# Litianyu141/Gen-FVGN-steady

Hardware: AMD Instinct MI355X
Metric: training iters/sec, 50k-cell cylinder mesh (fwd + loss + bwd + Adam, batch resident in HBM) (higher is better)
Workload: dtype f32

## Files before the change

### gen-fvgn-steady_amd/csrc/cfwd.hip

```cpp
#include <cstdlib>

#include "tchain_kernel.h"

#include "gfv_limits.h"
int* gfv_internal_status_ptr();

namespace {

constexpr float CF_SH = 16.0f;
constexpr float CF_SH_INV = 1.0f / 16.0f;
constexpr float CF_SH_LIMIT = 2048.0f;

__device__ __forceinline__ void cf_barrier() {
  asm volatile("s_waitcnt lgkmcnt(0)\n\ts_barrier" ::: "memory");
}

template <int KT0, int TG, int NW>
struct CfLds {
  static constexpr int KTB = KT0 > 4 ? KT0 : 4;
  static constexpr int B0 = 0;
  static constexpr int B1 = TG * KTB * 2048;
  static constexpr int SINV = B1 + TG * 8192;
  static constexpr int LNP = SINV + TG * 64;
  static constexpr int TOTAL = LNP + TG * 16 * NW * 8;
// ... 132 lines not shown
        if (!LOWP) wl[n][T] = im[T * 1024 + n * 128 + 64];
      }
  };
  auto hidden = [&](int layer, char* xout, float* save) {
#pragma unroll
    for (int q = 0; q < TG; ++q) {
      const int row = row0 + 16 * q + j;
      const bool live = q < ngt && row < A.M;
      const float si = layer == 0 ? sinv[q * 16 + j] : CF_SH_INV;
      float a[4 * NT];
#pragma unroll
      for (int n = 0; n < NT; ++n) {
        const float4 b = bias[layer][n];
        float v[4] = {(acc[q][n][0] * si) * invw + b.x, (acc[q][n][1] * si) * invw + b.y, (acc[q][n][2] * si) * invw + b.z,
                      (acc[q][n][3] * si) * invw + b.w};
        if (PADD && layer == 0) {
          v[0] += ps[PADD ? q : 0][n].x + pr[PADD ? q : 0][n].x; v[1] += ps[PADD ? q : 0][n].y + pr[PADD ? q : 0][n].y;
          v[2] += ps[PADD ? q : 0][n].z + pr[PADD ? q : 0][n].z; v[3] += ps[PADD ? q : 0][n].w + pr[PADD ? q : 0][n].w;
        }
        if (save && live) st4(save + (size_t)row * 128 + c0 + 16 * n, v);
        const gfv_f2 g01 = gfv_gelu2(gfv_f2{v[0], v[1]}), g23 = gfv_gelu2(gfv_f2{v[2], v[3]});
        a[4 * n + 0] = g01.x; a[4 * n + 1] = g01.y; a[4 * n + 2] = g23.x; a[4 * n + 3] = g23.y;
      }
      float m = 0.f;
#pragma unroll
      for (int e = 0; e < 4 * NT; e += 2) m = max3_abs(m, a[e], a[e + 1]);
      mabs = fmaxf(mabs, live ? m : 0.f);
      if constexpr (NT == 2) {
        float e8[8];
#pragma unroll
        for (int e = 0; e < 8; ++e) e8[e] = a[e] * CF_SH;
        gfv_uint4 hi, lo;
        gfv_split8_t<BF>(e8, hi, lo);
        gfv_uint4* dst = reinterpret_cast<gfv_uint4*>(xout + (size_t)(q * 4 + w) * 2048) + lane;
        dst[0] = hi;
        if (!LOWP) dst[64] = lo;
      } else {
        unsigned h0, h1, l0, l1;
        gfv_split_pair_t<BF>(a[0] * CF_SH, a[1] * CF_SH, h0, l0);
        gfv_split_pair_t<BF>(a[2] * CF_SH, a[3] * CF_SH, h1, l1);
        char* dst = xout + (size_t)(q * 4 + (w >> 1)) * 2048 + lane * 16 + (w & 1) * 8;
        *reinterpret_cast<uint2*>(dst) = make_uint2(h0, h1);
        if (!LOWP) *reinterpret_cast<uint2*>(dst + 1024) = make_uint2(l0, l1);
      }
    }
  };

  mma(b0, std::integral_constant<int, KT0>{});
  load_w(A.layer[1].Wh);
  hidden(0, b1, A.layer[0].save);
  cf_barrier();
  mma(b1, std::integral_constant<int, 4>{});
  load_w(A.layer[2].Wh);
  hidden(1, b0, A.layer[1].save);
  float4 gam[NT], bet[NT];
  if constexpr (FINLN) {
#pragma unroll
    for (int n = 0; n < NT; ++n) { gam[n] = ld4(A.fin_gamma + c0 + 16 * n); bet[n] = ld4(A.fin_beta + c0 + 16 * n); }
  }
  float4 rres[TG][NT];
  if (A.res[0]) {
#pragma unroll
    for (int q = 0; q < TG; ++q) {
      const float* rp = A.res[0] + (size_t)min(row0 + 16 * q + j, A.M - 1) * A.res_ld[0] + c0;
#pragma unroll
      for (int n = 0; n < NT; ++n) rres[q][n] = ld4(rp + 16 * n);
    }
  }
  cf_barrier();
  if constexpr (!FINLN) {
    if (w == 0) {
      mma(b0, std::integral_constant<int, 4>{});
      const int ncol = A.layer[2].N;
      const float* bp = A.layer[2].bias;
#pragma unroll
      for (int q = 0; q < TG; ++q) {
        const int row = row0 + 16 * q + j;
        if (q < ngt && row < A.M) {
#pragma unroll
          for (int r = 0; r < 4; ++r) {
            const int col = 4 * g + r;
            if (col < ncol) A.out[0][(size_t)row * A.out_ld[0] + col] = (acc[q][0][r] * CF_SH_INV) * invw + (bp ? bp[col] : 0.f);
          }
        }
      }
    }
    if (mabs > CF_SH_LIMIT) atomicOr(status, 2);
    return;
  }
  mma(b0, std::integral_constant<int, 4>{});
  const int hcols = (A.hidden > 0 && A.hidden < 128) ? A.hidden : 128;
  float y[TG][4 * NT];
#pragma unroll
  for (int q = 0; q < TG; ++q) {
    const int row = row0 + 16 * q + j;
    const bool live = q < ngt && row < A.M;
    float s = 0.f;
#pragma unroll
    for (int n = 0; n < NT; ++n) {
      const float4 b = bias[2][n];
      float v[4] = {(acc[q][n][0] * CF_SH_INV) * invw + b.x, (acc[q][n][1] * CF_SH_INV) * invw + b.y,
                    (acc[q][n][2] * CF_SH_INV) * invw + b.z, (acc[q][n][3] * CF_SH_INV) * invw + b.w};
      if (A.fin_presave && live) st4(A.fin_presave + (size_t)row * 128 + c0 + 16 * n, v);
#pragma unroll
      for (int r = 0; r < 4; ++r) {
        y[q][4 * n + r] = v[r];
        s += v[r];
      }
    }
    const float mw = row_sum(s) * (1.0f / (16.0f * NT));
    float m2 = 0.f;
#pragma unroll
    for (int e = 0; e < 4 * NT; ++e) {
      const float d = y[q][e] - mw;
      m2 += d * d;
    }
    m2 = row_sum(m2);
    if (g == 0) *reinterpret_cast<float2*>(lnp + ((q * 16 + j) * NW + w) * 2) = make_float2(mw, m2);
  }
  cf_barrier();
  {
    const float inv_h = 1.0f / (float)hcols, npad = (float)(128 - hcols);
#pragma unroll
    for (int q = 0; q < TG; ++q) {
      const int row = row0 + 16 * q + j;
      const bool live = q < ngt && row < A.M;
      const float4* pp = reinterpret_cast<const float4*>(lnp + (q * 16 + j) * 2 * NW);
      float m128, m2a;
      if constexpr (NW == 4) {
        const float4 p0 = pp[0], p1 = pp[1];
        m128 = ((p0.x + p0.z) + (p1.x + p1.z)) * 0.25f;
        const float e0 = p0.x - m128, e1 = p0.z - m128, e2 = p1.x - m128, e3 = p1.z - m128;
        m2a = ((p0.y + p0.w) + (p1.y + p1.w)) + 32.0f * ((e0 * e0 + e1 * e1) + (e2 * e2 + e3 * e3));
      } else {
        const float4 p0 = pp[0], p1 = pp[1], p2 = pp[2], p3 = pp[3];
        m128 = (((p0.x + p0.z) + (p1.x + p1.z)) + ((p2.x + p2.z) + (p3.x + p3.z))) * 0.125f;
        const float e0 = p0.x - m128, e1 = p0.z - m128, e2 = p1.x - m128, e3 = p1.z - m128, e4 = p2.x - m128, e5 = p2.z - m128,
                    e6 = p3.x - m128, e7 = p3.z - m128;
        m2a = (((p0.y + p0.w) + (p1.y + p1.w)) + ((p2.y + p2.w) + (p3.y + p3.w))) +
              16.0f * (((e0 * e0 + e1 * e1) + (e2 * e2 + e3 * e3)) + ((e4 * e4 + e5 * e5) + (e6 * e6 + e7 * e7)));
      }
      const float mean = hcols == 128 ? m128 : (m128 * 128.0f) * inv_h;
      const float dm = m128 - mean;
      const float m2 = hcols == 128 ? m2a : (m2a + 128.0f * dm * dm) - npad * (mean * mean);
      const float rstd = rsqrtf(m2 * inv_h + 1e-5f);
      if (A.fin_stats && live && w == 0 && g == 0) *reinterpret_cast<float2*>(A.fin_stats + 2 * (size_t)row) = make_float2(mean, rstd);
#pragma unroll
      for (int n = 0; n < NT; ++n) {
        const float4 ga = gam[n], be = bet[n];
        float o[4] = {(y[q][4 * n + 0] - mean) * rstd * ga.x + be.x, (y[q][4 * n + 1] - mean) * rstd * ga.y + be.y,
                      (y[q][4 * n + 2] - mean) * rstd * ga.z + be.z, (y[q][4 * n + 3] - mean) * rstd * ga.w + be.w};
        if (live) {
          if (A.out_nores) st4(A.out_nores + (size_t)row * 128 + c0 + 16 * n, o);
          if (A.res[0]) { o[0] += rres[q][n].x; o[1] += rres[q][n].y; o[2] += rres[q][n].z; o[3] += rres[q][n].w; }
          st4(A.out[0] + (size_t)row * A.out_ld[0] + c0 + 16 * n, o);
        }
      }
    }
  }
  if (mabs > CF_SH_LIMIT) atomicOr(status, 2);
}

inline bool cf_al16(const void* p) { return (reinterpret_cast<size_t>(p) & 15) == 0; }

template <int KT0, int N0, bool PADD, bool RAGIN, bool FINLN = true>
void cf_launch(const gfv_rowtile_args_t& a, int lowp, hipStream_t stream) {
  int* st = gfv_internal_status_ptr();
  constexpr int tg = 2;
  const int tiles = (a.M + 16 * tg - 1) / (16 * tg);
  const dim3 grid(PADD ? gfv_xcd_grid(tiles) : tiles), blk(512);
  if (lowp == 2) GFV_LAUNCH((cfwd_kernel<KT0, N0, 2, PADD, 2, RAGIN, 8, FINLN>), grid, blk, 0, stream, a, st);
  else if (lowp) GFV_LAUNCH((cfwd_kernel<KT0, N0, 2, PADD, 1, RAGIN, 8, FINLN>), grid, blk, 0, stream, a, st);
  else GFV_LAUNCH((cfwd_kernel<KT0, N0, 2, PADD, 0, RAGIN, 8, FINLN>), grid, blk, 0, stream, a, st);
}

}

int gfv_internal_cfwd_try(const gfv_rowtile_args_t* a, int lowp, hipStream_t stream, int dry) {
  if (!gfv_internal_status_ptr()) return 0;
  const int on = gfv_internal_limit(GFV_LIM_CFWD_ON);
  const int max_m = gfv_internal_limit(GFV_LIM_CFWD_MAX_M);
  if (!on || a->nlayers != 3 || a->M > max_m || a->M < 1 || (a->flags & (GFV_CHAIN_ROW_OWNER | GFV_CHAIN_COLUMN_OWNER))) return 0;
  const bool dec = a->fin_op == GFV_FIN_PLAIN && a->layer[2].N >= 1 && a->layer[2].N <= 16 && !a->res[0] && !a->out_nores && !a->fin_presave &&
                   !a->fin_stats && !a->padd && a->nseg == 1 && a->layer[0].K == 128;
  if (a->in_op != GFV_IN_NONE || !a->wmax) return 0;
  if (!dec && (a->fin_op != GFV_FIN_LN || !a->fin_gamma || !a->fin_beta)) return 0;
  if (a->in_add || a->gadd || a->in_save || a->in_aux || a->ln_partial || a->gscale || a->dw_partial || a->in_stats || a->fin_aux) return 0;
  for (int l = 0; l < 3; ++l) {
    const gfv_layer_t& L = a->layer[l];
    if (!L.Wh || (L.N != 128 && !(dec && l == 2)) || L.aux || L.bias2 || (L.bias && !cf_al16(L.bias) && !(dec && l == 2))) return 0;
    if (L.op != (l < 2 ? GFV_OP_BIAS_GELU : GFV_OP_NONE)) return 0;
    if (l > 0 && L.K != 128) return 0;
    if (L.save && !cf_al16(L.save)) return 0;
  }
  if (a->layer[2].save) return 0;
  if (!a->out[0] || a->out[1] || a->out[2] || (!dec && ((a->out_ld[0] & 3) || !cf_al16(a->out[0]))) || a->res[1] || a->res[2]) return 0;
  if (a->res[0] && ((a->res_ld[0] & 3) || !cf_al16(a->res[0]))) return 0;
  if ((a->out_nores && !cf_al16(a->out_nores)) || (a->fin_presave && !cf_al16(a->fin_presave)) ||
      (!dec && (!cf_al16(a->fin_gamma) || !cf_al16(a->fin_beta))))
    return 0;
  if (a->fin_stats && (reinterpret_cast<size_t>(a->fin_stats) & 7)) return 0;
  for (int i = 0; i < a->nseg; ++i)
    if (a->seg[i].idx || a->seg[i].csr_rowptr || a->seg[i].csr_scale || a->seg[i].save) return 0;
  const int K0 = a->layer[0].K;
  int shape = -1;
  auto plain = [&](int i, int width) {
    const gfv_seg_t& s = a->seg[i];
    return s.width == width && (s.ld & 3) == 0 && cf_al16(s.ptr);
  };
  if (a->padd) {
    if (a->nseg == 1 && K0 == 128 && plain(0, 128) && a->padd_s && a->padd_r && a->padd_ld >= 256 && (a->padd_ld & 3) == 0 && cf_al16(a->padd))
      shape = 1;
  } else if (a->nseg == 2 && K0 == 192 && plain(0, 64) && plain(1, 128)) {
    shape = 0;
  } else if (dec) {
    if (plain(0, 128)) shape = 4;
  } else if (a->nseg == 1 && K0 == 128 && plain(0, 128)) {
    shape = 2;
  } else if (a->nseg == 1 && K0 <= 32 && a->seg[0].width == K0) {
    shape = 3;
  }
  if (shape < 0) return 0;
  if (dry) return 1;
  if (shape == 0) cf_launch<6, 4, false, false>(*a, lowp, stream);
  else if (shape == 1) cf_launch<4, 8, true, false>(*a, lowp, stream);
  else if (shape == 2) cf_launch<4, 8, false, false>(*a, lowp, stream);
  else if (shape == 4) cf_launch<4, 8, false, false, false>(*a, lowp, stream);
  else cf_launch<1, 2, false, true>(*a, lowp, stream);
  return 1;
}
```

### gen-fvgn-steady_amd/csrc/colchain.hip

```cpp
#include "colchain_kernel.h"

int* gfv_internal_status_ptr();

static int cc_env(const char* name, int dflt) {
  const char* e = getenv(name);
  return e ? atoi(e) : dflt;
}
static bool al16(const void* p) { return (reinterpret_cast<size_t>(p) & 15) == 0; }

static int cc_cus() {
  static int n = 0;
  if (!n) {
    int dev = 0;
    hipDeviceProp_t pr;
    if (hipGetDevice(&dev) == hipSuccess && hipGetDeviceProperties(&pr, dev) == hipSuccess) n = pr.multiProcessorCount;
    if (n <= 0) n = 256;
    const int want = cc_env("GFV_COLCHAIN_WGS", 0);
    if (want > 0 && want <= n) n = want;
  }
  return n;
}

static bool cc_bwd_ok(const gfv_rowtile_args_t* a) {
  static const int on = cc_env("GFV_COLCHAIN_BWD", 1);
  static const int min_m = cc_env("GFV_COLCHAIN_BWD_MIN_M", 2048);
  if (a->flags & GFV_CHAIN_ROW_OWNER) return false;
  if (!(a->flags & GFV_CHAIN_COLUMN_OWNER) && (!on || a->M < min_m)) return false;
  if (!a->dw_partial || a->dw_partial_stride < GFV_DW_FUSED_FLOATS || !a->in_stats || !a->wmax) return false;
  if (a->dw_in) return false;
  const bool noout = a->nlayers == 2;
  const bool rc = a->rc_Wh[0] != nullptr;
  if (rc && (!a->rc_Wh[1] || a->dw_in || !al16(a->rc_Wh[0]) || !al16(a->rc_Wh[1]) || (a->rc_bias[0] && !al16(a->rc_bias[0])) ||
             (a->rc_bias[1] && !al16(a->rc_bias[1]))))
    return false;
  if (!rc && a->rc_Wh[1]) return false;
  if ((a->nlayers != 3 && !noout) || a->in_op != GFV_IN_LNBWD || a->fin_op != GFV_FIN_PLAIN || a->nseg != 1) return false;
  if (noout && (a->layer[1].op != GFV_OP_MUL_DGELU || a->layer[1].save || a->res[0] || a->gadd || a->dw_in || !a->out[0])) return false;
  if (a->seg[0].width != 128 || a->seg[0].idx || a->seg[0].csr_rowptr || a->seg[0].save || a->seg[0].ld != 128 || !al16(a->seg[0].ptr)) return false;
  if (a->M > (1 << 22) || a->out_ld[0] != 128 || (a->res[0] && a->res_ld[0] != 128) || (a->dw_in && a->dw_in_ld != 128)) return false;
  if (a->layer[0].op != GFV_OP_MUL_DGELU || a->layer[1].op != GFV_OP_MUL_DGELU || (!noout && a->layer[2].op != GFV_OP_NONE)) return false;
  for (int l = 0; l < a->nlayers; ++l) {
    const gfv_layer_t& L = a->layer[l];
    if (!L.Wh || (L.N != 128 && !(l == 2 && L.N == 192)) || L.K != 128 || L.bias || L.bias2) return false;
    if (l < 2 && !(rc && l == 0) && (!L.aux || !al16(L.aux))) return false;
    if (L.save && !al16(L.save)) return false;
  }
  if ((!rc && (!a->in_aux || !al16(a->in_aux))) || !a->in_gamma || !al16(a->in_gamma) || a->ln_partial || a->padd) return false;
  const bool out2 = !noout && a->layer[2].N == 192;
  if (!a->out[0] || (out2 ? (!a->out[1] || a->out_ld[1] != 64 || !al16(a->out[1]) || a->dw_in) : a->out[1] != nullptr) || a->out[2] ||
      a->res[1] || a->res[2] || a->out_nores)
    return false;
  if ((a->out_ld[0] & 3) || !al16(a->out[0]) || (a->res[0] && ((a->res_ld[0] & 3) || !al16(a->res[0])))) return false;
  if (a->in_add && !al16(a->in_add)) return false;
  if (a->gadd && (!al16(a->gadd) || !a->gadd_s || !a->gadd_r)) return false;
  if (a->in_save && !al16(a->in_save)) return false;
  if ((reinterpret_cast<size_t>(a->in_stats) & 7) || !al16(a->dw_partial) || (a->dw_partial_stride & 3)) return false;
  return true;
}
extern "C" int gfv_hidden_size(void);
extern "C" int gfv_f16split_enabled(void);
extern "C" int gfv_rowtile_dw_partials(void) { return cc_cus(); }
extern "C" int gfv_rowtile_dw_partials_m(int32_t M) {
  const int tiles = (M + 63) / 64;
  return tiles < cc_cus() ? (tiles > 0 ? tiles : 1) : cc_cus();
}
extern "C" int gfv_rowtile_fuses_dw(const gfv_rowtile_args_t* a) {
  if (!a || gfv_hidden_size() != 128 || gfv_f16split_enabled() == 0) return 0;
  gfv_rowtile_args_t t = *a;
  t.hidden = 128;
  return cc_bwd_ok(&t) ? 1 : 0;
}

int gfv_internal_colchain_try(const gfv_rowtile_args_t* a, hipStream_t stream) {
  if (a->hidden == 128 && cc_bwd_ok(a)) {
    int* st = gfv_internal_status_ptr();
    if (!st) return 0;
    const dim3 grid(gfv_rowtile_dw_partials_m(a->M)), blk(64 * CC_W);
#define CB_K(...) GFV_LAUNCH((colchain_bwd_kernel<__VA_ARGS__>), grid, blk, 0, stream, *a, st)
#define CB_LAUNCH(LOWP, RC)                                                                                                      \
  do {                                                                                                                           \
    if (a->nlayers == 2) CB_K(LOWP, false, false, true, RC);                                                                     \
    else if (a->layer[2].N == 192 && a->gadd) CB_K(LOWP, true, true, false, RC);                                                 \
    else if (a->layer[2].N == 192) CB_K(LOWP, false, true, false, RC);                                                           \
    else if (a->gadd) CB_K(LOWP, true, false, false, RC);                                                                        \
    else CB_K(LOWP, false, false, false, RC);                                                                                    \
  } while (0)
    const bool rc = a->rc_Wh[0] != nullptr;
    if (a->product_form == 2) { if (rc) CB_LAUNCH(2, true); else CB_LAUNCH(2, false); }
    else if (a->product_form != 0) { if (rc) CB_LAUNCH(1, true); else CB_LAUNCH(1, false); }
    else { if (rc) CB_LAUNCH(0, true); else CB_LAUNCH(0, false); }
#undef CB_K
#undef CB_LAUNCH
    return 2;
  }
  return 0;
}
```

### gen-fvgn-steady_amd/csrc/colchain_kernel.h

```cpp
#pragma once
#include "tchain_kernel.h"

namespace {

constexpr int CC_W = 8;
constexpr float CC_SH = 16.0f;
constexpr float CC_SH_INV = 1.0f / 16.0f;
constexpr float CC_SH_LIMIT = 2048.0f;
#ifdef GFV_CC_TIMING
#define CT_DECL long long ct_[16] = {0, 0, 0, 0, 0, 0, 0, 0, 0, 0, 0, 0, 0, 0, 0, 0}; long long ct_prev_ = clock64();
#define CT(k) do { __builtin_amdgcn_s_waitcnt(0xc07f); const long long now_ = clock64(); ct_[k] += now_ - ct_prev_; ct_prev_ = now_; } while (0)
#else
#define CT_DECL
#define CT(k)
#endif
__device__ __forceinline__ void cc_barrier() {
  asm volatile("s_waitcnt lgkmcnt(0)\n\ts_barrier" ::: "memory");
}

struct CcCtx {
  int w, lane, j, g, col0;
  int M;
  int row0;
  int ngt;
  float invw;
  float mabs;
};

template <int KT, int LOWP, bool FENCE = false>
__device__ __forceinline__ void cc_mma_pair(const char* xbuf, int pair, const gfv_f16x8 (&wh)[KT], const gfv_f16x8 (&wl)[KT],
                                            int lane, floatx4& a0, floatx4& a1) {
  const gfv_f16x8* f0 = reinterpret_cast<const gfv_f16x8*>(xbuf + (size_t)(2 * pair) * KT * 2048) + lane;
  const gfv_f16x8* f1 = f0 + KT * 128;
  a0 = floatx4{0.f, 0.f, 0.f, 0.f};
  a1 = floatx4{0.f, 0.f, 0.f, 0.f};
#pragma unroll
  for (int T = 0; T < KT; ++T) {
    const gfv_f16x8 xh0 = f0[(2 * T) * 64], xh1 = f1[(2 * T) * 64];
    if (!LOWP) {
      const gfv_f16x8 xl0 = f0[(2 * T + 1) * 64], xl1 = f1[(2 * T + 1) * 64];
      a0 = __builtin_amdgcn_mfma_f32_16x16x32_f16(wl[T], xh0, a0, 0, 0, 0);
      a1 = __builtin_amdgcn_mfma_f32_16x16x32_f16(wl[T], xh1, a1, 0, 0, 0);
      a0 = __builtin_amdgcn_mfma_f32_16x16x32_f16(wh[T], xl0, a0, 0, 0, 0);
      a1 = __builtin_amdgcn_mfma_f32_16x16x32_f16(wh[T], xl1, a1, 0, 0, 0);
    }
    a0 = gfv_mma_hh<LOWP == 2>(wh[T], xh0, a0);
    a1 = gfv_mma_hh<LOWP == 2>(wh[T], xh1, a1);
    if (FENCE) __builtin_amdgcn_sched_barrier(0);
  }
}

template <bool BF>
__device__ __forceinline__ void cc_put_frag(char* xbuf, int q, const CcCtx& c, const float (&a)[4], float scale) {
  unsigned h0, h1, l0, l1;
  const gfv_f2 s01 = gfv_f2{a[0], a[1]} * gfv_splat2(scale), s23 = gfv_f2{a[2], a[3]} * gfv_splat2(scale);
  gfv_split_pair_t<BF>(s01.x, s01.y, h0, l0);
  gfv_split_pair_t<BF>(s23.x, s23.y, h1, l1);
  char* dst = xbuf + (size_t)((q * 4 + (c.w >> 1)) * 2) * 1024 + c.lane * 16 + (c.w & 1) * 8;
  *reinterpret_cast<uint2*>(dst) = make_uint2(h0, h1);
  *reinterpret_cast<uint2*>(dst + 1024) = make_uint2(l0, l1);
}

constexpr int CB_TG = 4;
struct CbLds {
  static constexpr int BUF = CB_TG * 8192;
  static constexpr int B0 = 0, B1 = BUF, B2 = 2 * BUF;
  static constexpr int PART = 3 * BUF;
  static constexpr int SMAX = PART + CB_TG * 16 * 8 * 8;
  static constexpr int TOTAL = SMAX + 64;
};

__device__ __forceinline__ void cb_tr_operand(const char* xbuf, int q0, int ct, int lane, gfv_f16x8& hi, gfv_f16x8& lo) {
  typedef short s4 __attribute__((ext_vector_type(4)));
  typedef __attribute__((address_space(3))) s4* lds_s4;
  const int s = lane & 15, gp = lane >> 4;
  const int off = ((q0 * 4 + (ct >> 1)) * 2) * 1024 + (16 * (s & 3) + 4 * gp + (s >> 2)) * 16 + (ct & 1) * 8;
  const char* p = xbuf + off;
  const s4 h0 = __builtin_amdgcn_ds_read_tr16_b64_v4i16((lds_s4)(p));
  const s4 l0 = __builtin_amdgcn_ds_read_tr16_b64_v4i16((lds_s4)(p + 1024));
  const s4 h1 = __builtin_amdgcn_ds_read_tr16_b64_v4i16((lds_s4)(p + 8192));
  const s4 l1 = __builtin_amdgcn_ds_read_tr16_b64_v4i16((lds_s4)(p + 8192 + 1024));
  typedef short s8 __attribute__((ext_vector_type(8)));
  const s8 h = {h0[0], h0[1], h0[2], h0[3], h1[0], h1[1], h1[2], h1[3]};
  const s8 l = {l0[0], l0[1], l0[2], l0[3], l1[0], l1[1], l1[2], l1[3]};
  hi = __builtin_bit_cast(gfv_f16x8, h);
  lo = __builtin_bit_cast(gfv_f16x8, l);
}

__device__ __forceinline__ int cb_dw_ntile(int w, int i) { return 2 * (w >> 1) + (i >> 2); }
__device__ __forceinline__ int cb_dw_ktile(int w, int i) { return 4 * (w & 1) + (i & 3); }
__device__ __forceinline__ int cb_dw_btile(int w) { return 2 * (w >> 1) + (w & 1); }
template <int LOWP>
__device__ __forceinline__ void cb_dw_tile(const char* gbuf, const char* abuf, int npairs, int w, int lane, floatx4 (&acc)[8],
                                           floatx4& accb) {
  const gfv_f16x8 ones = gfv_frag_ones<LOWP == 2>();
  const int nt0 = 2 * (w >> 1), kt0 = 4 * (w & 1);
  for (int pr = 0; pr < npairs; ++pr) {
    gfv_f16x8 gh[2], gl[2];
    cb_tr_operand(gbuf, 2 * pr, nt0, lane, gh[0], gl[0]);
    cb_tr_operand(gbuf, 2 * pr, nt0 + 1, lane, gh[1], gl[1]);
    {
      const bool odd = (w & 1) != 0;
      const gfv_f16x8 bh = odd ? gh[1] : gh[0], bl = odd ? gl[1] : gl[0];
      if (!LOWP) accb = __builtin_amdgcn_mfma_f32_16x16x32_f16(bl, ones, accb, 0, 0, 0);
      accb = gfv_mma_hh<LOWP == 2>(bh, ones, accb);
    }
#pragma unroll
    for (int kk = 0; kk < 4; ++kk) {
      gfv_f16x8 ah, al;
      cb_tr_operand(abuf, 2 * pr, kt0 + kk, lane, ah, al);
#pragma unroll
      for (int nn = 0; nn < 2; ++nn) {
        if (!LOWP) {
          acc[4 * nn + kk] = __builtin_amdgcn_mfma_f32_16x16x32_f16(gl[nn], ah, acc[4 * nn + kk], 0, 0, 0);
          acc[4 * nn + kk] = __builtin_amdgcn_mfma_f32_16x16x32_f16(gh[nn], al, acc[4 * nn + kk], 0, 0, 0);
        }
        acc[4 * nn + kk] = gfv_mma_hh<LOWP == 2>(gh[nn], ah, acc[4 * nn + kk]);
      }
    }
    __builtin_amdgcn_sched_barrier(0);
  }
}

template <bool BF>
__device__ __forceinline__ void cb_hidden_bwd(CcCtx& c, int q, const floatx4& acc, float inv_in, const float4& z, float sg,
                                              char* gout, char* aout, float (&v)[4]) {
  const gfv_f2 z01 = {z.x, z.y}, z23 = {z.z, z.w};
  gfv_f2 a01, a23, d01, d23;
  gfv_gelu_dgelu2(z01, a01, d01);
  gfv_gelu_dgelu2(z23, a23, d23);
  const gfv_f2 ki = gfv_splat2(inv_in), kw = gfv_splat2(c.invw);
  const gfv_f2 v01 = ((gfv_f2{acc[0], acc[1]} * ki) * kw) * d01, v23 = ((gfv_f2{acc[2], acc[3]} * ki) * kw) * d23;
  v[0] = v01.x; v[1] = v01.y; v[2] = v23.x; v[3] = v23.y;
  const float a[4] = {a01.x, a01.y, a23.x, a23.y};
  const float mq = max3_abs(max3_abs(0.f, v[0], v[1]), v[2], v[3]) * sg;
  const float ma = max3_abs(max3_abs(0.f, a[0], a[1]), a[2], a[3]) * (60000.0f / CC_SH_LIMIT);
  c.mabs = fmaxf(c.mabs, q < c.ngt ? fmaxf(mq, ma) : 0.f);
  cc_put_frag<BF>(gout, q, c, v, sg);
  cc_put_frag<BF>(aout, q, c, a, CC_SH);
}

__device__ __forceinline__ char* cb_own_slot(char* xbuf, int q, const CcCtx& c) {
  return xbuf + (size_t)((q * 4 + (c.w >> 1)) * 2) * 1024 + c.lane * 16 + (c.w & 1) * 8;
}
__device__ __forceinline__ void cb_park4(char* xbuf, int q, const CcCtx& c, const float (&v)[4]) {
  char* d = cb_own_slot(xbuf, q, c);
  *reinterpret_cast<float2*>(d) = make_float2(v[0], v[1]);
  *reinterpret_cast<float2*>(d + 1024) = make_float2(v[2], v[3]);
}
__device__ __forceinline__ void cb_unpark4(char* xbuf, int q, const CcCtx& c, float (&v)[4]) {
  const char* d = cb_own_slot(xbuf, q, c);
  const float2 a = *reinterpret_cast<const float2*>(d), b = *reinterpret_cast<const float2*>(d + 1024);
  v[0] = a.x; v[1] = a.y; v[2] = b.x; v[3] = b.y;
}

template <bool BF>
__device__ __forceinline__ void cb_hidden_bwd_dg(CcCtx& c, int q, const floatx4& acc, float inv_in, const float (&dg)[4], float sg,
                                                 char* gout, float (&v)[4]) {
#pragma unroll
  for (int r = 0; r < 4; ++r) v[r] = ((acc[r] * inv_in) * c.invw) * dg[r];
  const float mq = max3_abs(max3_abs(0.f, v[0], v[1]), v[2], v[3]) * sg;
  c.mabs = fmaxf(c.mabs, q < c.ngt ? mq : 0.f);
  cc_put_frag<BF>(gout, q, c, v, sg);
}

typedef int cb_i32x4 __attribute__((ext_vector_type(4)));
typedef int cb_i32x2 __attribute__((ext_vector_type(2)));
typedef __amdgpu_buffer_rsrc_t cb_rsrc;
constexpr int CB_OFF_DEAD = 0x7ffffff0;
__device__ __forceinline__ cb_rsrc cb_buf(const void* p, size_t bytes) {
  const size_t n = p ? (bytes < 0x7fffffe0ull ? bytes : 0x7fffffe0ull) : 0;
  return __builtin_amdgcn_make_buffer_rsrc(const_cast<void*>(p), 0, (int)n, 0x00020000);
}
typedef float cb_f32x2 __attribute__((ext_vector_type(2)));
__device__ __forceinline__ float4 cb_ld4(cb_rsrc r, int off) {
  const floatx4 f = __builtin_bit_cast(floatx4, __builtin_amdgcn_raw_buffer_load_b128(r, off, 0, 0));
  return make_float4(f[0], f[1], f[2], f[3]);
}
__device__ __forceinline__ float2 cb_ld2(cb_rsrc r, int off) {
  const cb_f32x2 f = __builtin_bit_cast(cb_f32x2, __builtin_amdgcn_raw_buffer_load_b64(r, off, 0, 0));
  return make_float2(f[0], f[1]);
}
__device__ __forceinline__ void cb_st4v(cb_rsrc r, int off, const floatx4& f) {
  __builtin_amdgcn_raw_buffer_store_b128(__builtin_bit_cast(cb_i32x4, f), r, off, 0, 0);
}
__device__ __forceinline__ void cb_st4(cb_rsrc r, int off, const float (&v)[4]) {
  const floatx4 f = {v[0], v[1], v[2], v[3]};
  __builtin_amdgcn_raw_buffer_store_b128(__builtin_bit_cast(cb_i32x4, f), r, off, 0, 0);
}

struct CbIn {
  float4 dy[CB_TG], yv[CB_TG], ga[CB_TG];
  float2 st[CB_TG];
};
struct CbBufs {
  cb_rsrc dy, y3, stats, z2, z1, gadd, gidx, save1, res, out;
};
__device__ __forceinline__ int cb_off(const CcCtx& c, int row0, int q) { return min(row0 + 16 * q + c.j, c.M - 1) * 512 + c.col0 * 4; }

template <bool GADD>
__device__ __forceinline__ void cb_load_gidx(const CbBufs& B, const CcCtx& c, int row0, int (&gidx)[CB_TG]) {
  if (GADD) {
#pragma unroll
    for (int q = 0; q < CB_TG; ++q) gidx[q] = __builtin_amdgcn_raw_buffer_load_b32(B.gidx, min(row0 + 16 * q + c.j, c.M - 1) * 4, 0, 0);
  }
}
__device__ __forceinline__ void cb_load_inputs(const CbBufs& B, const CcCtx& c, int row0, CbIn& in) {
#pragma unroll
  for (int q = 0; q < CB_TG; ++q) {
    const int off = cb_off(c, row0, q);
    in.dy[q] = cb_ld4(B.dy, off);
    in.yv[q] = cb_ld4(B.y3, off);
    in.st[q] = cb_ld2(B.stats, min(row0 + 16 * q + c.j, c.M - 1) * 8);
  }
}
__device__ __forceinline__ void cb_load_dy_stats(const CbBufs& B, const CcCtx& c, int row0, CbIn& in) {
#pragma unroll
  for (int q = 0; q < CB_TG; ++q) {
    in.dy[q] = cb_ld4(B.dy, cb_off(c, row0, q));
    in.st[q] = cb_ld2(B.stats, min(row0 + 16 * q + c.j, c.M - 1) * 8);
  }
}
__device__ __forceinline__ void cb_load_rows(cb_rsrc r, const CcCtx& c, int row0, float4 (&v)[CB_TG]) {
#pragma unroll
  for (int q = 0; q < CB_TG; ++q) v[q] = cb_ld4(r, cb_off(c, row0, q));
}
template <bool GADD>
__device__ __forceinline__ void cb_load_gathers(const CbBufs& B, const CcCtx& c, const int (&gidx)[CB_TG], CbIn& in) {
  if (GADD) {
#pragma unroll
    for (int q = 0; q < CB_TG; ++q) in.ga[q] = cb_ld4(B.gadd, gidx[q] * 256 + (c.col0 & 63) * 4);
  }
}

template <int LOWP, bool GADD, bool OUT2 = false, bool NOOUT = false, bool RC = false>
__global__ __launch_bounds__(64 * CC_W, 2) void colchain_bwd_kernel(const gfv_rowtile_args_t A, int* status) {
  constexpr int TG = CB_TG;
  __shared__ __attribute__((aligned(16))) char lds[CbLds::TOTAL + (RC ? CbLds::BUF : 0)];
  char* b0 = lds + CbLds::B0;
  char* b1 = lds + CbLds::B1;
  char* b2 = lds + CbLds::B2;
  char* b3 = lds + CbLds::TOTAL;
  float* part = reinterpret_cast<float*>(lds + CbLds::PART);
  float* smax = reinterpret_cast<float*>(lds + CbLds::SMAX);

  CcCtx c;
  c.w = __builtin_amdgcn_readfirstlane(threadIdx.x >> 6);
  c.lane = threadIdx.x & 63;
  c.j = c.lane & 15;
  c.g = c.lane >> 4;
  c.col0 = 16 * c.w + 4 * c.g;
  c.M = A.M;
  c.mabs = 0.f;
  c.invw = 1.0f / gfv_pow2_scale(*A.wmax);

  const int nwg = gridDim.x;
  const int wg = (nwg & 7) == 0 ? (int)(blockIdx.x & 7) * (nwg >> 3) + (int)(blockIdx.x >> 3) : (int)blockIdx.x;
  const int NG = (A.M + 15) >> 4;
  const int g_beg = (int)((long)NG * wg / nwg), g_end = (int)((long)NG * (wg + 1) / nwg);

  const size_t rows128 = (size_t)A.M * 512;
  CbBufs B;
  B.dy = cb_buf(A.seg[0].ptr, rows128);
  B.y3 = cb_buf(RC ? nullptr : A.in_aux, rows128);
  B.stats = cb_buf(A.in_stats, (size_t)A.M * 8);
  B.z2 = cb_buf(RC ? nullptr : A.layer[0].aux, rows128);
  B.z1 = cb_buf(A.layer[1].aux, rows128);
  B.gadd = cb_buf(A.gadd, 0x7fffffe0ull);
  B.gidx = cb_buf(c.w < 4 ? A.gadd_s : A.gadd_r, (size_t)A.M * 4);
  B.save1 = cb_buf(NOOUT ? A.out[0] : A.layer[1].save, rows128);
  B.res = cb_buf(NOOUT ? nullptr : A.res[0], rows128);
  B.out = cb_buf(NOOUT ? nullptr : A.out[0], rows128);
  const cb_rsrc out2 = cb_buf(OUT2 ? A.out[1] : nullptr, (size_t)A.M * 256);

  const cb_rsrc w0 = cb_buf(A.layer[0].Wh, 65536), w1 = cb_buf(A.layer[1].Wh, 65536),
                w2 = cb_buf(NOOUT ? nullptr : A.layer[2].Wh, OUT2 ? 131072 : 65536);
  const cb_rsrc rw2 = cb_buf(RC ? A.rc_Wh[0] : nullptr, 65536), rw3 = cb_buf(RC ? A.rc_Wh[1] : nullptr, 65536);
  const int woff = (c.w * 128 + c.lane) * 16;
  floatx4 dw3[8], dw2[8], db3 = floatx4{0.f, 0.f, 0.f, 0.f}, db2 = db3;
#pragma unroll
  for (int kt = 0; kt < 8; ++kt) dw3[kt] = dw2[kt] = floatx4{0.f, 0.f, 0.f, 0.f};
  float dgam[4] = {0.f, 0.f, 0.f, 0.f}, dbet[4] = {0.f, 0.f, 0.f, 0.f};
  float sacc = 0.f;
  float scap = 3.0e38f;

  float step1, step2;
  {
    float l1[2];
#pragma unroll
    for (int l = 0; l < 2; ++l) {
      const cb_rsrc wb = l == 0 ? w0 : w1;
      float acc = 0.f;
#pragma unroll
      for (int T = 0; T < 4; ++T) {
        const gfv_f16x8 h = __builtin_bit_cast(gfv_f16x8, __builtin_amdgcn_raw_buffer_load_b128(wb, woff + T * 16384, 0, 0));
        const gfv_f16x8 lo = __builtin_bit_cast(gfv_f16x8, __builtin_amdgcn_raw_buffer_load_b128(wb, woff + T * 16384 + 1024, 0, 0));
        if (LOWP == 2) {
          const gfv_bf16x8 hb = __builtin_bit_cast(gfv_bf16x8, h);
#pragma unroll
          for (int e = 0; e < 8; ++e) acc += fabsf((float)hb[e]);
        } else {
#pragma unroll
          for (int e = 0; e < 8; ++e) acc += fabsf((float)h[e] + (float)lo[e]);
        }
      }
      l1[l] = gfv_wave_max(row_sum(acc));
    }
    if (c.lane == 0) { smax[c.w] = l1[0]; part[c.w] = l1[1]; }
    cc_barrier();
    float m0 = 0.f, m1 = 0.f;
#pragma unroll
    for (int k = 0; k < 8; ++k) { m0 = fmaxf(m0, smax[k]); m1 = fmaxf(m1, part[k]); }
    cc_barrier();
    const float g0 = 1.13f * m0 * c.invw, g1 = 1.13f * m1 * c.invw;
    step1 = 1.0f / gfv_pow2_ceil(g0);
    step2 = 1.0f / gfv_pow2_ceil(g1);
  }

  constexpr bool PRE = true;
  int gidx[TG] = {0, 0, 0, 0};
  CbIn in;
  float4 zn[RC ? TG : 1];
  if (g_beg < g_end) {
    cb_load_gidx<GADD>(B, c, 16 * g_beg, gidx);
    if constexpr (RC) {
      cb_load_rows(B.z1, c, 16 * g_beg, zn);
      cb_load_dy_stats(B, c, 16 * g_beg, in);
      cb_load_gathers<GADD>(B, c, gidx, in);
    } else if (PRE) {
      cb_load_inputs(B, c, 16 * g_beg, in);
      cb_load_gathers<GADD>(B, c, gidx, in);
    }
  }
  const bool CB_LATE = c.w >= 4;
  CT_DECL
  for (int t0 = g_beg; t0 < g_end; t0 += TG) {
    c.row0 = 16 * t0;
    c.ngt = min(TG, g_end - t0);
    const int np = (c.ngt + 1) >> 1;
    const int next_row0 = t0 + TG < g_end ? 16 * (t0 + TG) : c.M;
    int offL[TG], offS[TG];
#pragma unroll
    for (int q = 0; q < TG; ++q) {
      const int row = c.row0 + 16 * q + c.j;
      offL[q] = cb_off(c, c.row0, q);
      offS[q] = (q < c.ngt && row < c.M) ? row * 512 + c.col0 * 4 : CB_OFF_DEAD;
    }
    if constexpr (RC) {
      gfv_f16x8 rh[4], rl[4];
#pragma unroll
      for (int T = 0; T < 4; ++T) {
        rh[T] = __builtin_bit_cast(gfv_f16x8, __builtin_amdgcn_raw_buffer_load_b128(rw2, woff + T * 16384, 0, 0));
        rl[T] = __builtin_bit_cast(gfv_f16x8, __builtin_amdgcn_raw_buffer_load_b128(rw2, woff + T * 16384 + 1024, 0, 0));
      }
      const float4 zero4 = make_float4(0.f, 0.f, 0.f, 0.f);
#pragma unroll
      for (int q = 0; q < TG; ++q) {
        const float z4[4] = {zn[q].x, zn[q].y, zn[q].z, zn[q].w};
        float a[4];
#pragma unroll
        for (int r = 0; r < 4; ++r) a[r] = gfv_gelu(z4[r]);
        const float ma = max3_abs(max3_abs(0.f, a[0], a[1]), a[2], a[3]) * (60000.0f / CC_SH_LIMIT);
        c.mabs = fmaxf(c.mabs, q < c.ngt ? ma : 0.f);
        cc_put_frag<LOWP == 2>(b3, q, c, a, CC_SH);
      }
      CT(12);
      cc_barrier();
      CT(13);
#pragma unroll
      for (int q = 0; q < TG; ++q) in.yv[q] = zero4;
      {
        int tvar = 0;
        asm volatile("" : "+v"(tvar));
        const float4 bi2 = cb_ld4(cb_buf(A.rc_bias[0], 512), c.col0 * 4 + tvar);
        floatx4 a0, a1;
        cc_mma_pair<4, LOWP, true>(b3, 0, rh, rl, c.lane, a0, a1);
#pragma unroll
        for (int p = 0; p < TG / 2; ++p) {
          if (p >= np) break;
          floatx4 n0 = a0, n1 = a1;
          if (p + 1 < TG / 2) cc_mma_pair<4, LOWP, true>(b3, p + 1, rh, rl, c.lane, n0, n1);
#pragma unroll
          for (int h = 0; h < 2; ++h) {
            const int q = 2 * p + h;
            const floatx4& acc = h ? a1 : a0;
            const float bb[4] = {bi2.x, bi2.y, bi2.z, bi2.w};
            float a[4], dg[4];
#pragma unroll
            for (int r = 0; r < 4; ++r) {
              const float z = (acc[r] * CC_SH_INV) * c.invw + bb[r];
              const gfv_erfc_t e = gfv_erfc_half(z);
              const float cdf = z >= 0.0f ? 1.0f - e.y : e.y;
              dg[r] = fmaf(z * 0.39894228040143267794f, e.e, cdf);
              a[r] = fmaf(-fabsf(z), e.y, fmaxf(z, 0.0f));
            }
            cb_park4(b1, q, c, dg);
            const float ma = max3_abs(max3_abs(0.f, a[0], a[1]), a[2], a[3]) * (60000.0f / CC_SH_LIMIT);
            c.mabs = fmaxf(c.mabs, q < c.ngt ? ma : 0.f);
            cc_put_frag<LOWP == 2>(b2, q, c, a, CC_SH);
          }
          a0 = n0; a1 = n1;
        }
      }
#pragma unroll
      for (int T = 0; T < 4; ++T) {
        rh[T] = __builtin_bit_cast(gfv_f16x8, __builtin_amdgcn_raw_buffer_load_b128(rw3, woff + T * 16384, 0, 0));
        rl[T] = __builtin_bit_cast(gfv_f16x8, __builtin_amdgcn_raw_buffer_load_b128(rw3, woff + T * 16384 + 1024, 0, 0));
      }
      CT(14);
      cc_barrier();
      CT(15);
      {
        int tvar = 0;
        asm volatile("" : "+v"(tvar));
        const float4 bi3 = cb_ld4(cb_buf(A.rc_bias[1], 512), c.col0 * 4 + tvar);
        floatx4 a0, a1;
        cc_mma_pair<4, LOWP, true>(b2, 0, rh, rl, c.lane, a0, a1);
#pragma unroll
        for (int p = 0; p < TG / 2; ++p) {
          if (p >= np) break;
          floatx4 n0 = a0, n1 = a1;
          if (p + 1 < TG / 2) cc_mma_pair<4, LOWP, true>(b2, p + 1, rh, rl, c.lane, n0, n1);
          in.yv[2 * p] = make_float4((a0[0] * CC_SH_INV) * c.invw + bi3.x, (a0[1] * CC_SH_INV) * c.invw + bi3.y,
                                     (a0[2] * CC_SH_INV) * c.invw + bi3.z, (a0[3] * CC_SH_INV) * c.invw + bi3.w);
          in.yv[2 * p + 1] = make_float4((a1[0] * CC_SH_INV) * c.invw + bi3.x, (a1[1] * CC_SH_INV) * c.invw + bi3.y,
                                         (a1[2] * CC_SH_INV) * c.invw + bi3.z, (a1[3] * CC_SH_INV) * c.invw + bi3.w);
          a0 = n0; a1 = n1;
        }
      }
    }
    float gg[TG][4], xh[TG][4], rs[TG];
    {
      float bmax = 0.f;
      if (!PRE) {
        cb_load_inputs(B, c, c.row0, in);
        cb_load_gathers<GADD>(B, c, gidx, in);
      }
      if (A.in_add) {
        const cb_rsrc ia = cb_buf(A.in_add, rows128);
#pragma unroll
        for (int q = 0; q < TG; ++q) {
          const float4 t = cb_ld4(ia, offL[q]);
          in.dy[q].x += t.x; in.dy[q].y += t.y; in.dy[q].z += t.z; in.dy[q].w += t.w;
        }
      }
      float* part_j = part + (c.j * 8 + c.w) * 2;
      const float4 gam = RC ? cb_ld4(cb_buf(A.in_gamma, 512), c.col0 * 4) : ld4(A.in_gamma + c.col0);
#pragma unroll
      for (int q = 0; q < TG; ++q) {
        const float lf = offS[q] != CB_OFF_DEAD ? 1.0f : 0.0f;
        float d[4] = {in.dy[q].x, in.dy[q].y, in.dy[q].z, in.dy[q].w};
        if (GADD) { d[0] += in.ga[q].x; d[1] += in.ga[q].y; d[2] += in.ga[q].z; d[3] += in.ga[q].w; }
        const float y[4] = {in.yv[q].x, in.yv[q].y, in.yv[q].z, in.yv[q].w};
        const float gm[4] = {gam.x, gam.y, gam.z, gam.w};
        const float mean = in.st[q].x, rstd = in.st[q].y;
        rs[q] = rstd;
        float s1 = 0.f, s2 = 0.f, am = 0.f;
#pragma unroll
        for (int h = 0; h < 2; ++h) {
          const int r = 2 * h;
          const gfv_f2 dd = gfv_f2{d[r], d[r + 1]} * gfv_splat2(lf);
          const gfv_f2 xx = (gfv_f2{y[r], y[r + 1]} - gfv_splat2(mean)) * gfv_splat2(rstd);
          const gfv_f2 dx = dd * xx;
          const gfv_f2 g2 = dd * gfv_f2{gm[r], gm[r + 1]};
          const gfv_f2 gx = g2 * xx;
          const gfv_f2 ng = gfv_f2{dgam[r], dgam[r + 1]} + dx, nb = gfv_f2{dbet[r], dbet[r + 1]} + dd;
          dgam[r] = ng.x; dgam[r + 1] = ng.y;
          dbet[r] = nb.x; dbet[r + 1] = nb.y;
          xh[q][r] = xx.x; xh[q][r + 1] = xx.y;
          gg[q][r] = g2.x; gg[q][r + 1] = g2.y;
          s1 += g2.x; s1 += g2.y;
          s2 += gx.x; s2 += gx.y;
          am = max3_abs(am, g2.x, g2.y);
        }
        s1 = row_sum(s1);
        s2 = row_sum(s2);
        if (c.g == 0) *reinterpret_cast<float2*>(part_j + q * 256) = make_float2(s1, s2);
        bmax = fmaxf(bmax, am * fabsf(rstd) * lf);
      }
      bmax = gfv_wave_max(bmax);
      if (c.lane == 0) smax[c.w] = bmax;
    }
    gfv_f16x8 wh[4], wl[4];
#pragma unroll
    for (int T = 0; T < 4; ++T) {
      wh[T] = __builtin_bit_cast(gfv_f16x8, __builtin_amdgcn_raw_buffer_load_b128(w0, woff + T * 16384, 0, 0));
      wl[T] = __builtin_bit_cast(gfv_f16x8, __builtin_amdgcn_raw_buffer_load_b128(w0, woff + T * 16384 + 1024, 0, 0));
    }
    float4 zq[TG];
    if constexpr (!RC) {
#pragma unroll
      for (int q = 0; q < TG; ++q) zq[q] = cb_ld4(B.z2, offL[q]);
    }
    CT(0);
    cc_barrier();
    CT(1);
    float s3;
    {
      const float4 ma = *reinterpret_cast<const float4*>(smax), mb = *reinterpret_cast<const float4*>(smax + 4);
      const float mx = fmaxf(fmaxf(fmaxf(ma.x, ma.y), fmaxf(ma.z, ma.w)), fmaxf(fmaxf(mb.x, mb.y), fmaxf(mb.z, mb.w)));
      s3 = fminf(gfv_pow2_scale(mx * 13.5f) * 2.0f, scap);
      scap = fminf(scap, s3 * 1048576.0f);
#pragma unroll
      for (int q = 0; q < TG; ++q) {
        const float4* pp = reinterpret_cast<const float4*>(part + (q * 16 + c.j) * 16);
        const float4 p0 = pp[0], p1 = pp[1], p2 = pp[2], p3 = pp[3];
        const float m1 = (((p0.x + p0.z) + (p1.x + p1.z)) + ((p2.x + p2.z) + (p3.x + p3.z))) * 0.0078125f;
        const float m2 = (((p0.y + p0.w) + (p1.y + p1.w)) + ((p2.y + p2.w) + (p3.y + p3.w))) * 0.0078125f;
        float g3[4];
#pragma unroll
        for (int h = 0; h < 2; ++h) {
          const int r = 2 * h;
          const gfv_f2 t = gfv_splat2(rs[q]) * ((gfv_f2{gg[q][r], gg[q][r + 1]} - gfv_splat2(m1)) - gfv_f2{xh[q][r], xh[q][r + 1]} * gfv_splat2(m2));
          g3[r] = t.x; g3[r + 1] = t.y;
        }
        if (A.in_save) cb_st4(cb_buf(A.in_save, rows128), offS[q], g3);
        cc_put_frag<LOWP == 2>(b0, q, c, g3, s3);
      }
    }
    if (sacc != 0.f && sacc != s3) {
      const float ratio = s3 / sacc;
#pragma unroll
      for (int kt = 0; kt < 8; ++kt) { dw3[kt] *= ratio; dw2[kt] *= ratio; }
      db3 *= ratio;
      db2 *= ratio;
    }
    sacc = s3;
    const float s2s = s3 * step1, s1s = s2s * step2;
    if (A.gscale && c.w == 0 && c.lane < c.ngt) {
      const size_t grp = (size_t)(c.row0 >> 4) + c.lane;
      A.gscale[grp] = s3 * 0.25f;
      A.gscale[(size_t)A.gscale_ld + grp] = s2s * 0.25f;
      A.gscale[2 * (size_t)A.gscale_ld + grp] = s1s * 0.25f;
    }
    CT(2);
    cc_barrier();
    CT(3);
    cb_load_gidx<GADD>(B, c, next_row0, gidx);
    {
      const float inv_in = 1.0f / s3;
      floatx4 a0, a1;
      cc_mma_pair<4, LOWP, true>(b0, 0, wh, wl, c.lane, a0, a1);
#pragma unroll
      for (int p = 0; p < TG / 2; ++p) {
        if (p >= np) break;
        floatx4 n0 = a0, n1 = a1;
        float v0[4], v1[4];
        if (!CB_LATE && p + 1 < TG / 2) cc_mma_pair<4, LOWP, true>(b0, p + 1, wh, wl, c.lane, n0, n1);
        if constexpr (RC) {
          float d0[4], d1[4];
          cb_unpark4(b1, 2 * p, c, d0);
          cb_unpark4(b1, 2 * p + 1, c, d1);
          cb_hidden_bwd_dg<LOWP == 2>(c, 2 * p, a0, inv_in, d0, s2s, b1, v0);
          cb_hidden_bwd_dg<LOWP == 2>(c, 2 * p + 1, a1, inv_in, d1, s2s, b1, v1);
        } else {
          cb_hidden_bwd<LOWP == 2>(c, 2 * p, a0, inv_in, zq[2 * p], s2s, b1, b2, v0);
          cb_hidden_bwd<LOWP == 2>(c, 2 * p + 1, a1, inv_in, zq[2 * p + 1], s2s, b1, b2, v1);
        }
        if (A.layer[0].save) {
          const cb_rsrc s0 = cb_buf(A.layer[0].save, rows128);
          cb_st4(s0, offS[2 * p], v0);
          cb_st4(s0, offS[2 * p + 1], v1);
        }
        if (CB_LATE && p + 1 < TG / 2) cc_mma_pair<4, LOWP, true>(b0, p + 1, wh, wl, c.lane, n0, n1);
        a0 = n0; a1 = n1;
      }
    }
#pragma unroll
    for (int T = 0; T < 4; ++T) {
      wh[T] = __builtin_bit_cast(gfv_f16x8, __builtin_amdgcn_raw_buffer_load_b128(w1, woff + T * 16384, 0, 0));
      wl[T] = __builtin_bit_cast(gfv_f16x8, __builtin_amdgcn_raw_buffer_load_b128(w1, woff + T * 16384 + 1024, 0, 0));
    }
#pragma unroll
    for (int q = 0; q < TG; ++q) zq[q] = cb_ld4(B.z1, offL[q]);
    CT(4);
    cc_barrier();
    CT(5);
    if constexpr (RC) cb_load_rows(B.z1, c, next_row0, zn);
    cb_dw_tile<LOWP>(b0, b2, np, c.w, c.lane, dw3, db3);
    if constexpr (RC) cb_dw_tile<LOWP>(b1, b3, np, c.w, c.lane, dw2, db2);
    CT(6);
    cc_barrier();
    CT(7);
    {
      const float inv_in = 1.0f / s2s;
      floatx4 a0, a1;
      cc_mma_pair<4, LOWP, true>(b1, 0, wh, wl, c.lane, a0, a1);
#pragma unroll
      for (int p = 0; p < TG / 2; ++p) {
        if (p >= np) break;
        floatx4 n0 = a0, n1 = a1;
        float v0[4], v1[4];
        if (!CB_LATE && p + 1 < TG / 2) cc_mma_pair<4, LOWP, true>(b1, p + 1, wh, wl, c.lane, n0, n1);
        if constexpr (RC) {
          const float d0[4] = {gfv_dgelu(zq[2 * p].x), gfv_dgelu(zq[2 * p].y), gfv_dgelu(zq[2 * p].z), gfv_dgelu(zq[2 * p].w)};
          const float d1[4] = {gfv_dgelu(zq[2 * p + 1].x), gfv_dgelu(zq[2 * p + 1].y), gfv_dgelu(zq[2 * p + 1].z),
                               gfv_dgelu(zq[2 * p + 1].w)};
          cb_hidden_bwd_dg<LOWP == 2>(c, 2 * p, a0, inv_in, d0, s1s, b0, v0);
          cb_hidden_bwd_dg<LOWP == 2>(c, 2 * p + 1, a1, inv_in, d1, s1s, b0, v1);
        } else {
          cb_hidden_bwd<LOWP == 2>(c, 2 * p, a0, inv_in, zq[2 * p], s1s, b0, b2, v0);
          cb_hidden_bwd<LOWP == 2>(c, 2 * p + 1, a1, inv_in, zq[2 * p + 1], s1s, b0, b2, v1);
        }
        cb_st4(B.save1, offS[2 * p], v0);
        cb_st4(B.save1, offS[2 * p + 1], v1);
        if (CB_LATE && p + 1 < TG / 2) cc_mma_pair<4, LOWP, true>(b1, p + 1, wh, wl, c.lane, n0, n1);
        a0 = n0; a1 = n1;
      }
    }
    if constexpr (!NOOUT) {
#pragma unroll
      for (int T = 0; T < 4; ++T) {
        wh[T] = __builtin_bit_cast(gfv_f16x8, __builtin_amdgcn_raw_buffer_load_b128(w2, woff + T * 16384, 0, 0));
        wl[T] = __builtin_bit_cast(gfv_f16x8, __builtin_amdgcn_raw_buffer_load_b128(w2, woff + T * 16384 + 1024, 0, 0));
      }
    }
    float4 rr[NOOUT ? 1 : TG];
    if constexpr (!NOOUT) {
#pragma unroll
      for (int q = 0; q < TG; ++q) rr[q] = cb_ld4(B.res, offL[q]);
    }
    CT(8);
    cc_barrier();
    CT(9);
    if constexpr (!NOOUT) {
      const float inv_in = 1.0f / s1s;
      floatx4 a0, a1;
      cc_mma_pair<4, LOWP, true>(b0, 0, wh, wl, c.lane, a0, a1);
#pragma unroll
      for (int p = 0; p < TG / 2; ++p) {
        if (p >= np) break;
        floatx4 n0 = a0, n1 = a1;
        if (!CB_LATE && p + 1 < TG / 2) cc_mma_pair<4, LOWP, true>(b0, p + 1, wh, wl, c.lane, n0, n1);
        const floatx4 o0 = (a0 * inv_in) * c.invw + floatx4{rr[2 * p].x, rr[2 * p].y, rr[2 * p].z, rr[2 * p].w};
        const floatx4 o1 = (a1 * inv_in) * c.invw + floatx4{rr[2 * p + 1].x, rr[2 * p + 1].y, rr[2 * p + 1].z, rr[2 * p + 1].w};
        cb_st4v(B.out, offS[2 * p], o0);
        cb_st4v(B.out, offS[2 * p + 1], o1);
        if (CB_LATE && p + 1 < TG / 2) cc_mma_pair<4, LOWP, true>(b0, p + 1, wh, wl, c.lane, n0, n1);
        a0 = n0; a1 = n1;
      }
      if constexpr (OUT2) {
        if (c.w < 4) {
          gfv_f16x8 xh2[4], xl2[4];
#pragma unroll
          for (int T = 0; T < 4; ++T) {
            xh2[T] = __builtin_bit_cast(gfv_f16x8, __builtin_amdgcn_raw_buffer_load_b128(w2, 65536 + woff + T * 16384, 0, 0));
            xl2[T] = __builtin_bit_cast(gfv_f16x8, __builtin_amdgcn_raw_buffer_load_b128(w2, 65536 + woff + T * 16384 + 1024, 0, 0));
          }
#pragma unroll
          for (int p = 0; p < TG / 2; ++p) {
            if (p >= np) break;
            floatx4 e0, e1;
            cc_mma_pair<4, LOWP, true>(b0, p, xh2, xl2, c.lane, e0, e1);
            const floatx4 o0 = (e0 * inv_in) * c.invw, o1 = (e1 * inv_in) * c.invw;
            const int ra = c.row0 + 32 * p + c.j, rb = ra + 16;
            cb_st4v(out2, (2 * p < c.ngt && ra < c.M) ? ra * 256 + c.col0 * 4 : CB_OFF_DEAD, o0);
            cb_st4v(out2, (2 * p + 1 < c.ngt && rb < c.M) ? rb * 256 + c.col0 * 4 : CB_OFF_DEAD, o1);
          }
        }
      }
    }
    CT(10);
    if constexpr (RC) {
      cb_load_dy_stats(B, c, next_row0, in);
      cb_load_gathers<GADD>(B, c, gidx, in);
    } else {
      if (PRE) {
        cb_load_inputs(B, c, next_row0, in);
        cb_load_gathers<GADD>(B, c, gidx, in);
      }
      cb_dw_tile<LOWP>(b1, b2, np, c.w, c.lane, dw2, db2);
    }
    CT(11);
  }

#ifdef GFV_CC_TIMING
  if (c.lane == 0 && A.fin_aux) {
    long long* dbg = reinterpret_cast<long long*>(const_cast<float*>(A.fin_aux)) + ((size_t)blockIdx.x * CC_W + c.w) * 16;
    for (int kk = 0; kk < 16; ++kk) dbg[kk] = ct_[kk];
  }
#endif
  if (A.dw_partial) {
    float* blk = A.dw_partial + (size_t)blockIdx.x * A.dw_partial_stride;
    const float is = sacc != 0.f ? 1.0f / sacc : 0.f;
    const float r2 = 1.0f / step1, r1 = r2 / step2;
    const float u3 = is * CC_SH_INV, u2 = (is * r2) * CC_SH_INV;
#pragma unroll
    for (int kt = 0; kt < 8; ++kt)
#pragma unroll
      for (int r = 0; r < 4; ++r) {
        const int n = 16 * cb_dw_ntile(c.w, kt) + 4 * c.g + r, k = 16 * cb_dw_ktile(c.w, kt) + c.j;
        blk[n * 128 + k] = dw3[kt][r] * u3;
        blk[16384 + 128 + n * 128 + k] = dw2[kt][r] * u2;
      }
    if (c.j == 0) {
#pragma unroll
      for (int r = 0; r < 4; ++r) {
        const int nb = 16 * cb_dw_btile(c.w) + 4 * c.g + r;
        blk[16384 + nb] = db3[r] * is;
        blk[2 * 16384 + 128 + nb] = db2[r] * (is * r2);
      }
    }
#pragma unroll
    for (int r = 0; r < 4; ++r) {
      const float dg = gfv_row16_sum(dgam[r]), db = gfv_row16_sum(dbet[r]);
      if (c.j == 0) {
        blk[2 * 16384 + 256 + c.col0 + r] = dg;
        blk[2 * 16384 + 384 + c.col0 + r] = db;
      }
    }
  }
  if (c.mabs > 60000.0f) atomicOr(status, 2);
}


}
```

### gen-fvgn-steady_amd/csrc/gfv_limits.h

```cpp
#pragma once
enum {
  GFV_LIM_CBWD_ON = 0,
  GFV_LIM_CBWD_MAX_M,
  GFV_LIM_CFWD_ON,
  GFV_LIM_CFWD_MAX_M,
  GFV_LIM_CTRANS_ON,
  GFV_LIM_CTRANS_MAX_M,
  GFV_LIM_LIN1S_ON,
  GFV_LIM_LIN1S_MAX_M,
  GFV_LIM_COUNT
};
int gfv_internal_limit(int which);
```

### gen-fvgn-steady_amd/csrc/rowtile.hip

```cpp
#include <atomic>
#include <stdio.h>
#include <stdlib.h>
#include <mutex>
#include "gfv_common.h"
#include "gfv_limits.h"
#include "gfv_prof.h"
#include "../../include/gfv.h"

namespace {
constexpr int BM = 64;
}

int gfv_internal_tchain_launch(const gfv_rowtile_args_t* args, int ragged, int f16, hipStream_t stream);

static std::atomic<int> g_f16_default{-1};
static thread_local int g_f16split = -1;
static int f16_default() {
  int d = g_f16_default.load(std::memory_order_relaxed);
  if (d < 0) {
    const char* e = getenv("GFV_F16SPLIT");
    d = e ? ((atoi(e) == 2 || atoi(e) == 3) ? atoi(e) : (atoi(e) != 0)) : 1;
    int expect = -1;
    if (!g_f16_default.compare_exchange_strong(expect, d)) d = expect;
  }
  return d;
}
extern "C" int gfv_f16split_enabled(void) { return g_f16split >= 0 ? g_f16split : f16_default(); }
extern "C" int gfv_set_f16split(int32_t on) {
  g_f16_default.store((on == 2 || on == 3) ? on : (on ? 1 : 0));
  g_f16split = -1;
  return GFV_OK;
}
extern "C" int gfv_set_f16split_thread(int32_t on) {
  if (on < -1 || on > 3) return GFV_ERR_ARG;
  g_f16split = on;
  return GFV_OK;
}
static int f16_mode() { return gfv_f16split_enabled(); }

static thread_local int g_hidden = 128;
extern "C" int gfv_hidden_size(void) { return g_hidden; }
extern "C" int gfv_set_hidden_size(int32_t h) {
  if (h < 16 || h > 128 || (h & 15)) return GFV_ERR_ARG;
  g_hidden = h;
  return GFV_OK;
}

static thread_local int g_last_path = -1;
extern "C" int gfv_rowtile_last_path(void) { return g_last_path; }
namespace {
struct LimitDef { const char* env; int dflt; };
const LimitDef k_limits[GFV_LIM_COUNT] = {
    {"GFV_CBWD", 1},        {"GFV_CBWD_MAX_M", 25000},      {"GFV_CFWD", 1},          {"GFV_CFWD_MAX_M", 250000},
    {"GFV_CTRANS", 1},         {"GFV_CTRANS_MAX_M", 16384},
    {"GFV_LIN1S", 1},       {"GFV_LIN1S_MAX_M", 16384}};
int g_limit[GFV_LIM_COUNT];
bool g_limit_set[GFV_LIM_COUNT];
std::once_flag g_limit_once;
void limits_init() {
  for (int i = 0; i < GFV_LIM_COUNT; ++i) {
    const char* e = getenv(k_limits[i].env);
    g_limit[i] = e ? atoi(e) : k_limits[i].dflt;
    g_limit_set[i] = false;
  }
}
}
int gfv_internal_limit(int which) {
  std::call_once(g_limit_once, limits_init);
  return (which >= 0 && which < GFV_LIM_COUNT) ? g_limit[which] : 0;
}
extern "C" int gfv_get_limit(int32_t which) { return (which >= 0 && which < GFV_LIM_COUNT) ? gfv_internal_limit(which) : -1; }
extern "C" int gfv_set_limit(int32_t which, int32_t value) {
  if (which < 0 || which >= GFV_LIM_COUNT) return GFV_ERR_ARG;
  std::call_once(g_limit_once, limits_init);
  if (value < 0) {
    const char* e = getenv(k_limits[which].env);
    g_limit[which] = e ? atoi(e) : k_limits[which].dflt;
  } else {
    g_limit[which] = value;
  }
  return GFV_OK;
}
extern "C" const char* gfv_limit_name(int32_t which) { return (which >= 0 && which < GFV_LIM_COUNT) ? k_limits[which].env : nullptr; }

static thread_local int g_last_ln_rows = 0;
extern "C" int gfv_rowtile_last_ln_rows(void) { return g_last_ln_rows; }

extern "C" int gfv_rowtile_tiles(int32_t M) { return (M + BM - 1) / BM; }

static int rowtile_chain_impl(const gfv_rowtile_args_t* args, void* stream);
extern "C" int gfv_rowtile_chain(const gfv_rowtile_args_t* args, void* stream) {
  if (!args) return GFV_ERR_ARG;
  if (args->product_form < 0 || args->product_form > 4 || (args->hidden != 0 && (args->hidden < 16 || args->hidden > 128 || (args->hidden & 15))))
    return GFV_ERR_ARG;
  if (args->product_form == 0 && args->hidden == 0) return rowtile_chain_impl(args, stream);
  const int f0 = g_f16split, h0 = g_hidden;
  if (args->product_form) g_f16split = args->product_form - 1;
  if (args->hidden) g_hidden = args->hidden;
  const int rc = rowtile_chain_impl(args, stream);
  g_f16split = f0;
  g_hidden = h0;
  return rc;
}
int gfv_internal_lin1_try(const gfv_rowtile_args_t* a, int lowp, hipStream_t stream, int dry);
int gfv_internal_cfwd_try(const gfv_rowtile_args_t* a, int lowp, hipStream_t stream, int dry);
bool gfv_internal_wimg_form_ok(const float* wmax);
int gfv_internal_cbwd_try(const gfv_rowtile_args_t* a, int lowp, hipStream_t stream, int dry);
static int cfwd_try(const gfv_rowtile_args_t* args, int lowp, hipStream_t stream, int dry) {
  if (args->nlayers != 3 || (args->fin_op != GFV_FIN_LN && args->fin_op != GFV_FIN_PLAIN)) return 0;
  gfv_rowtile_args_t local = *args;
  local.hidden = g_hidden;
  return gfv_internal_cfwd_try(&local, lowp, stream, dry);
}
static int cbwd_try(const gfv_rowtile_args_t* args, int lowp, hipStream_t stream, int dry) {
  if (args->in_op != GFV_IN_LNBWD || args->dw_partial || !args->in_stats) return 0;
  gfv_rowtile_args_t local = *args;
  local.hidden = g_hidden;
  return gfv_internal_cbwd_try(&local, lowp, stream, dry);
}
static int rowtile_chain_impl(const gfv_rowtile_args_t* args, void* stream) {
  if (!args || args->M < 0 || args->nlayers < 1 || args->nlayers > 3 || args->nseg < 1 || args->nseg > 3) return GFV_ERR_ARG;
  if (args->M == 0) {
    g_last_ln_rows = 0;
    return GFV_OK;
  }
  for (int i = 0; i < args->nseg; ++i)
    if (args->seg[i].width < 1 || args->seg[i].width > 128) return GFV_ERR_ARG;
  for (int l = 0; l + 1 < args->nlayers; ++l)
    if (args->layer[l].N != 128 || args->layer[l + 1].K != 128) return GFV_ERR_ARG;
  int k0 = 0;
  for (int i = 0; i < args->nseg; ++i) k0 += args->seg[i].width;
  if (k0 != args->layer[0].K) return GFV_ERR_ARG;
  const gfv_layer_t& last = args->layer[args->nlayers - 1];
  if (last.N > 384 || last.N < 1) return GFV_ERR_ARG;
  if ((args->rc_Wh[0] || args->rc_Wh[1]) && !args->dw_partial) return GFV_ERR_ARG;
  if (args->padd && (args->nlayers < 2 || args->padd_ld < 256 || (args->padd_ld & 3) || !args->padd_s || !args->padd_r)) return GFV_ERR_ARG;
  for (int l = 0; l < args->nlayers; ++l)
    if (args->layer[l].ldw != 0 && args->layer[l].ldw < args->layer[l].K) return GFV_ERR_ARG;
  if (last.N > 128 && (last.N & 15)) return GFV_ERR_ARG;
  if ((args->fin_op != GFV_FIN_PLAIN || args->in_op == GFV_IN_LN || args->in_op == GFV_IN_LNBWD) &&
      (args->fin_op != GFV_FIN_PLAIN ? last.N != 128 : false))
    return GFV_ERR_ARG;
  if ((args->in_op == GFV_IN_LN || args->in_op == GFV_IN_LNBWD) && (args->nseg != 1 || args->seg[0].width != 128))
    return GFV_ERR_ARG;
  bool fast_t = true;
  for (int i = 0; i < args->nseg; ++i) fast_t = fast_t && (args->seg[i].width % 32 == 0) && (args->seg[i].ld % 4 == 0);
  for (int l = 0; l < args->nlayers; ++l) {
    const bool lastl = (l == args->nlayers - 1);
    fast_t = fast_t && (args->layer[l].K % 4 == 0) && (args->layer[l].ldw % 4 == 0) && (args->layer[l].N % (lastl ? 64 : 128) == 0);
  }
  if (args->fin_op != GFV_FIN_PLAIN) fast_t = fast_t && last.N == 128;
  for (int c = 0; c < 3; ++c) {
    if (args->out[c]) fast_t = fast_t && (args->out_ld[c] % 4 == 0);
    if (args->res[c]) fast_t = fast_t && (args->res_ld[c] % 4 == 0);
  }
  bool rag_t = !fast_t && args->in_op != GFV_IN_LNBWD && args->fin_op != GFV_FIN_LNBWD;
  for (int l = 0; l + 1 < args->nlayers; ++l) rag_t = rag_t && args->layer[l].N == 128;
  if (last.N > 128) rag_t = rag_t && (last.N % 64 == 0);
  if (last.N % 16) rag_t = rag_t && last.op != GFV_OP_MUL_DGELU && args->fin_op == GFV_FIN_PLAIN && !args->out_nores;
  if (args->in_op == GFV_IN_LN) rag_t = rag_t && args->seg[0].width == 128 && (args->seg[0].ld % 4 == 0);
  if (args->gadd) rag_t = rag_t && args->seg[0].width == 128 && (args->seg[0].ld % 4 == 0);
  for (int l = 1; l < args->nlayers; ++l) rag_t = rag_t && (args->layer[l].K == 128);
  {
    bool csr = false;
    for (int i = 0; i < args->nseg; ++i) {
      const gfv_seg_t& sg = args->seg[i];
      csr = csr || sg.csr_rowptr != nullptr || sg.save != nullptr;
      if (sg.csr_rowptr && (!sg.idx || (i == 0 && args->in_add))) return GFV_ERR_ARG;
    }
    if (csr && (!fast_t || args->in_op == GFV_IN_LNBWD || args->fin_op == GFV_FIN_LNBWD))
      return GFV_ERR_ARG;
  }
  bool f16 = (fast_t || rag_t) && f16_mode() != 0 && args->wmax != nullptr;
  for (int l = 0; l < args->nlayers; ++l) f16 = f16 && args->layer[l].Wh != nullptr;
  for (int i = 0; i + 1 < args->nseg; ++i) f16 = f16 && (args->seg[i].width % 32 == 0);
  if (f16 && !gfv_internal_wimg_form_ok(args->wmax)) return GFV_ERR_ARG;
  for (int l = 0; l < args->nlayers; ++l)
    if ((!args->layer[l].W || args->layer[l].bias2) && !f16) return GFV_ERR_ARG;
  if (!fast_t && !rag_t) {
    static const bool dbg = getenv("GFV_ROWTILE_DEBUG") != nullptr;
    if (dbg)
      fprintf(stderr, "[gfv] gfv_rowtile_chain: unsupported shape M=%d nseg=%d widths=%d,%d,%d ld0=%d nlayers=%d K0=%d Nlast=%d out_ld=%d in_op=%d fin_op=%d\n",
              args->M, args->nseg, args->seg[0].width, args->nseg > 1 ? args->seg[1].width : 0,
              args->nseg > 2 ? args->seg[2].width : 0, args->seg[0].ld, args->nlayers, args->layer[0].K, last.N,
              args->out_ld[0], args->in_op, args->fin_op);
    return GFV_ERR_ARG;
  }
  void* tok = nullptr;
  if (gfv_prof_enabled()) {
    double fl = 0, by = 0;
    for (int l = 0; l < args->nlayers; ++l) {
      fl += 2.0 * args->M * (double)args->layer[l].K * args->layer[l].N;
      by += 4.0 * ((double)args->layer[l].K * args->layer[l].N + args->layer[l].N);
      if (args->layer[l].save) by += 4.0 * args->M * args->layer[l].N;
      if (args->layer[l].aux) by += 4.0 * args->M * args->layer[l].N;
    }
    by += 4.0 * args->M * (double)args->layer[0].K + 4.0 * args->M * (double)last.N;
    for (int i = 0; i < args->nseg; ++i) if (args->seg[i].idx) by += 4.0 * args->M;
    if (args->in_aux || args->fin_aux) by += 4.0 * args->M * 128.0;
    if (args->in_save) by += 4.0 * args->M * 128.0;
    if (args->fin_presave) by += 4.0 * args->M * 128.0;
    if (args->out_nores) by += 4.0 * args->M * 128.0;
    if (args->padd) by += 4.0 * args->M * 258.0;
    for (int c = 0; c < 3; ++c) if (args->res[c]) by += 4.0 * args->M * 128.0;
    const int lnm = args->in_op == GFV_IN_LNBWD ? 1 : (args->fin_op == GFV_FIN_LNBWD ? 2 : 0);
    int kind = fast_t ? GFV_K_TCHAIN0 + lnm : GFV_K_TCHAIN_RAG;
    for (int i = 0; i < args->nseg; ++i)
      if (args->seg[i].csr_rowptr || args->seg[i].save) kind = GFV_K_TCHAIN_CSR;
    if (fast_t && f16 && args->nlayers == 1 && gfv_internal_lin1_try(args, f16_mode() >= 2 ? f16_mode() - 1 : 0, (hipStream_t)stream, 1))
      kind = GFV_K_LIN1;
    if (f16 && cfwd_try(args, f16_mode() >= 2 ? f16_mode() - 1 : 0, (hipStream_t)stream, 1))
      kind = GFV_K_COLCHAIN_FWD;
    if (args->dw_partial) {
      kind = GFV_K_COLCHAIN_BWD;
      const int nfused = 2 + (args->rc_Wh[0] ? 2 : 0);
      fl += nfused * 2.0 * args->M * 128.0 * 128.0;
      by += 8.0 * args->M + 4.0 * (double)gfv_rowtile_dw_partials_m(args->M) * (double)args->dw_partial_stride;
    }
    tok = gfv_prof_begin(kind, fl, by, (hipStream_t)stream);
  }
  g_last_path = (fast_t ? 1 : 2) + (f16 ? 4 : 0);
  g_last_ln_rows = (args->M + BM - 1) / BM;
  if (args->dw_partial && !(fast_t && f16)) return GFV_ERR_ARG;
  if (fast_t && f16 && args->nlayers == 1 && gfv_internal_lin1_try(args, f16_mode() >= 2 ? f16_mode() - 1 : 0, (hipStream_t)stream, 0)) {
    g_last_path += 32;
  } else if (f16 && !args->dw_partial && cfwd_try(args, f16_mode() >= 2 ? f16_mode() - 1 : 0, (hipStream_t)stream, 0)) {
    g_last_path += 64;
  } else if (fast_t && f16 && cbwd_try(args, f16_mode() >= 2 ? f16_mode() - 1 : 0, (hipStream_t)stream, 0)) {
    g_last_path += 128;
    g_last_ln_rows = (args->M + 31) / 32;
  } else if (fast_t) {
    const int took = gfv_internal_tchain_launch(args, 0, f16 ? 1 : 0, (hipStream_t)stream);
    if (args->dw_partial && took != 2) return GFV_ERR_ARG;
    g_last_path += 8 * took;
  }
  else
    gfv_internal_tchain_launch(args, 1, f16 ? 1 : 0, (hipStream_t)stream);
  gfv_prof_end(tok, (hipStream_t)stream);
  GFV_CHECK_LAUNCH();
  return GFV_OK;
}
```

### gen-fvgn-steady_amd/gfv/cmdlist.py

```python
from __future__ import annotations

import torch

import os

NATIVE = os.environ.get("GFV_CMDLIST_NATIVE", "1") != "0"

_QUERIES = frozenset((
    "gfv_abi_version", "gfv_struct_size", "gfv_rowtile_tiles", "gfv_rowtile_last_path", "gfv_dw_chunks", "gfv_dw_slabs",
    "gfv_linear_dw_workspace_floats", "gfv_dw_multi_workspace_floats", "gfv_f16split_enabled", "gfv_set_f16split", "gfv_set_f16split_thread", "gfv_hidden_size",
    "gfv_weight_image_bytes", "gfv_normalizer_blocks", "gfv_slice_softmax_bwd_blocks", "gfv_profile_enable",
    "gfv_profile_collect", "gfv_profile_reset", "gfv_profile_set_sizes", "gfv_status_flags", "gfv_status_mirror", "gfv_prep_workspace_bytes", "gfv_get_limit", "gfv_set_limit", "gfv_limit_name", "gfv_rowtile_dw_partials", "gfv_rowtile_dw_partials_m",
    "gfv_rowtile_fuses_dw", "gfv_graph_norm_workspace_bytes", "gfv_plan_create", "gfv_plan_destroy", "gfv_plan_table", "gfv_plan_sizes",
    "gfv_record_begin", "gfv_record_count", "gfv_record_end", "gfv_record_length", "gfv_record_replay", "gfv_record_free",
    "gfv_record_delay_side", "gfv_pool_args_bytes", "gfv_pool_table_bytes", "gfv_pool_table_check"))


class CommandList:
    def __init__(self):
        self.cmds = []
        self.pool = None
        self.main = None
        self.keep = []
        self.native = 0
        self.n_native = 0

    def __len__(self):
        return len(self.cmds) + self.n_native

    def __del__(self):
        if self.native:
            try:
                from . import lib as L
                L.load(raw=True).gfv_record_free(self.native)
            except Exception:
                pass

    def replay(self):
        cur = torch.cuda.current_stream()
        if cur != self.main:
            raise RuntimeError("a command list replays on the stream it was recorded on")
        if self.native:
            from . import lib as L
            lib, h, pos = L.load(raw=True), self.native, 0
            for fn, args, st, idx in self.cmds:
                if idx > pos:
                    L.check(lib.gfv_record_replay(h, pos, idx), "gfv_record_replay")
                    pos = idx
                if st is None or st == cur:
                    fn(*args)
                else:
                    with torch.cuda.stream(st):
                        fn(*args)
            if self.n_native > pos:
                L.check(lib.gfv_record_replay(h, pos, self.n_native), "gfv_record_replay")
            return
        for fn, args, st in self.cmds:
            if st is None or st == cur:
                fn(*args)
            else:
                with torch.cuda.stream(st):
                    fn(*args)


_ACTIVE = None


def active():
    return _ACTIVE


_IN_CALL = 0


def call(fn, *args):
    global _IN_CALL
    _IN_CALL += 1
    try:
        r = fn(*args)
    finally:
        _IN_CALL -= 1
    if _ACTIVE is not None:
        if _ACTIVE.native:
            from . import lib as L
            _ACTIVE.cmds.append((fn, args, torch.cuda.current_stream(), L.load(raw=True).gfv_record_count()))
        else:
            _ACTIVE.cmds.append((fn, args, torch.cuda.current_stream()))
    return r


_NO_KERNEL = frozenset((
    "aten::empty.memory_format", "aten::empty_strided", "aten::empty_like", "aten::new_empty", "aten::new_empty_strided",
    "aten::detach", "aten::alias", "aten::lift_fresh", "aten::_unsafe_view", "aten::is_pinned", "aten::resize_",
    "aten::set_.source_Storage", "aten::set_.source_Storage_storage_offset", "aten::set_.source_Tensor", "aten::_local_scalar_dense",
    "aten::is_same_size", "aten::stride", "aten::sym_size", "aten::sym_stride", "aten::sym_numel", "aten::sym_storage_offset"))


def _guard_mode():
    from torch.utils._python_dispatch import TorchDispatchMode
    from torch.utils._pytree import tree_leaves

    class Guard(TorchDispatchMode):
        def __torch_dispatch__(self, func, types, args=(), kwargs=None):
            out = func(*args, **(kwargs or {}))
            if _IN_CALL == 0:
                name = func._schema.name + ("." + func._overloadname if func._overloadname and func._overloadname != "default" else "")
                if name not in _NO_KERNEL and not getattr(func, "is_view", False):
                    leaves = tree_leaves((args, kwargs, out))
                    if any(isinstance(t, torch.Tensor) and t.is_cuda for t in leaves):
                        raise RuntimeError(
                            f"cmdlist: torch op {name} enqueued device work outside cmdlist.call while a step was being "
                            "recorded; it would be dropped on replay (wrap it in cmdlist.call, move it to set-up, or run the "
                            "step with use_graph=False)")
            return out
    return Guard()


class _RecordingLib:

    def __init__(self, cdll, target):
        self._cdll, self._target, self._cache = cdll, target, {}

    def __getattr__(self, name):
        hit = self._cache.get(name)
        if hit is not None:
            return hit
        f = getattr(self._cdll, name)
        if name in _QUERIES:
            self._cache[name] = f
            return f
        cmds = self._target.cmds
        if self._target.native:
            self._cache[name] = f
            return f

        def launch(*args):
            rc = f(*args)
            cmds.append((f, args, None))
            return rc
        self._cache[name] = launch
        return launch


class record:

    def __init__(self):
        self.cl = CommandList()

    def __enter__(self):
        global _ACTIVE
        from . import lib as L
        if _ACTIVE is not None:
            raise RuntimeError("nested recording")
        self.cl.main = torch.cuda.current_stream()
        self.cl.pool = torch.cuda.MemPool()
        self._ctx = torch.cuda.use_mem_pool(self.cl.pool)
        self._ctx.__enter__()
        _ACTIVE = self.cl
        if NATIVE:
            rc = L.load(raw=True).gfv_record_begin()
            if rc != 0:
                _ACTIVE = None
                self._ctx.__exit__(None, None, None)
                L.check(rc, "gfv_record_begin")
            self.cl.native = -1
        L._recording = _RecordingLib(L.load(raw=True), self.cl)
# ... 26 lines not shown
```

### gen-fvgn-steady_amd/gfv/engine.py

```python
from __future__ import annotations

import contextlib
import os

import torch

from . import cmdlist
from . import lib as L
from . import ops
from .ops import LayerSpec, Seg

_MODE = {"explicit": 0, "implicit": 1, "imex": 2}


def _empty(dev, *shape):
    return torch.empty(shape, dtype=torch.float32, device=dev)


def pick_concurrent_stream(priority=0, candidates=8):
    if torch.cuda.is_current_stream_capturing():
        return torch.cuda.Stream(priority=priority)
    main = torch.cuda.current_stream()
    cycles = 400_000

# ... 169 lines not shown
            return
        pend, self._pending = self._pending, []
        if split and len(pend) > 1:
            k = 1 if split == 1 else len(pend) - 1
            main_part, side_part = (pend[:k], pend[k:]) if split == 1 else (pend[k:], pend[:k])
            self._pending = side_part
            self.flush()
            self._pending = main_part
            self.flush(on_main=True)
            return
        if on_main:
            ws, self._dw_ws = self._dw_ws, self._dw_ws_main
            try:
                for fn, _ in pend:
                    fn()
            finally:
                self._dw_ws_main, self._dw_ws = self._dw_ws, ws
            return
        with self.fork(*[t for _, keep in pend for t in keep]):
            for fn, _ in pend:
                fn()

    def join(self):
        self.flush()
        if self.overlap and self._side is not None:
            for sd in self._sides:
                L.stream_wait(torch.cuda.current_stream(), sd)
        self._keep.clear()

    def _pkey(self, P, fresh=False):
        hit = self._pkey_cache
        if fresh or hit is None or hit[0] is not P:
            self._pkey_cache = hit = (P, tuple(t.data_ptr() for t in P.values()))
        return hit[1]

    def _wi_enter(self, phase, P):
        if not self.f16split:
            return None
        key = self._pkey(P, fresh=(phase == "fwd"))
        if self._wi_key != key:
            dev = next(iter(P.values())).device
            self._retired.append((self._wi, self._wmax, self._wi_abs))
            self._wmax = torch.zeros((1,), dtype=torch.float32, device=dev)
            self._wi = {ph: ops.WeightImages(dev, self._wmax) for ph in ("fwd", "bwd")}
            self._wi["fwd"].add_static(P.values())
            mats = [t for t in P.values() if t.dim() == 2 and t.stride(1) == 1]
            self._wi_abs = ops.WeightImages._upload([((t.data_ptr(), t.stride(0), t.shape[0], t.shape[1]), t) for t in mats], dev)
            self._wi_key = key
        wi = self._wi[phase]
        if phase == "fwd":
            L.check(L.load().gfv_weight_absmax(self._wi_abs[0].data_ptr(), self._wi_abs[1], self._wmax.data_ptr(),
                                               L.stream_ptr()), "gfv_weight_absmax")
        elif not wi.static and self._wt:
            wi.add_static(self._wt.values())
            if self.recompute:
                wi.add_static(P.values())
        wi.build()
        return ops.set_weight_images(wi)

    def build_static_images(self, P):
        if not self.f16split:
            return
        prev = self._wi_enter("fwd", P)
        ops.set_weight_images(prev)

    def _wi_static_enter(self, P):
        if not self.f16split:
            return None
        if self._wi is None or self._wi_key != self._pkey(P, fresh=True):
            raise RuntimeError("static weight images belong to another parameter set: call build_static_images(P) first")
        wi = self._wi["fwd"]
        if len(wi.valid) != len(wi.images) and cmdlist.active() is None:
            L.check(L.load().gfv_weight_absmax(self._wi_abs[0].data_ptr(), self._wi_abs[1], self._wmax.data_ptr(),
                                               L.stream_ptr()), "gfv_weight_absmax")
            wi.build()
        return ops.set_weight_images(wi)

    def capture_signature(self):
        wi = self._wi or {}
        return (self._wi_key, self._wt_key, L.load().gfv_f16split_enabled(),
                tuple((ph, len(w.images), None if w._desc is None else w._desc.data_ptr()) for ph, w in sorted(wi.items())))

    def _wi_exit(self, phase, prev):
        if not self.f16split:
            return
        self._wi[phase].invalidate()
        ops.set_weight_images(prev)

    def _T(self, W, perm=False):
        hit = self._wt.get((W.data_ptr(), perm)) if self._wt_live else None
        if hit is not None:
            return hit
        if not perm:
            return ops.transpose(W)
        if perm == "c":
            return ops.transpose(W, col0=256, ncols=128)
        if perm == "ab":
            return torch.cat((ops.transpose(W, col0=0, ncols=128), ops.transpose(W, col0=128, ncols=128)), 1).contiguous()
        out = _empty(W.device, 192, 128)
        ops.transpose(W, out=out[0:128], col0=64, ncols=128)
        ops.transpose(W, out=out[128:192], col0=0, ncols=64)
        return out

    def prepare_transposes(self, P):
        lib = L.load()
        key = self._pkey(P)
        if self._wt_key != key:
            import ctypes as C
            rows = []
            self._retired.append((self._wt, getattr(self, "_wt_desc", None)))
            self._wt = {}
            dev = next(iter(P.values())).device
            for n, W in P.items():
                if not n.endswith(".weight") or W.dim() != 2:
                    continue
                if any(t in n for t in (".to_q.", ".to_k.", ".to_v.", ".in_project_slice.")):
                    continue
                if ".encoder." in n and n.endswith(".0.0.weight"):
                    continue
                r, c = W.shape
                if ".nb_module.net.0.0.weight" in n:
                    out = _empty(dev, 192, 128)
                    rows.append((W.data_ptr() + 4 * 64, out.data_ptr(), r, 128, c, 0))
                    rows.append((W.data_ptr(), out.data_ptr() + 4 * 128 * 128, r, 64, c, 0))
                    self._wt[(W.data_ptr(), True)] = out
                elif self.factor and ".eb_module.net.0.0.weight" in n:
                    oc, oab = _empty(dev, 128, 128), _empty(dev, 128, 256)
                    rows.append((W.data_ptr() + 4 * 256, oc.data_ptr(), r, 128, c, 0))
                    rows.append((W.data_ptr(), oab.data_ptr(), r, 128, c, 256))
                    rows.append((W.data_ptr() + 4 * 128, oab.data_ptr() + 4 * 128, r, 128, c, 256))
                    self._wt[(W.data_ptr(), "c")] = oc
                    self._wt[(W.data_ptr(), "ab")] = oab
                else:
                    out = _empty(dev, c, r)
                    rows.append((W.data_ptr(), out.data_ptr(), r, c, c, 0))
                    self._wt[(W.data_ptr(), False)] = out
            import struct
            blob = b"".join(struct.pack("<QQiiii", a, b, r, c, ld, ldo) for a, b, r, c, ld, ldo in rows)
            self._wt_desc = torch.frombuffer(bytearray(blob), dtype=torch.uint8).to(dev)
            self._wt_n = len(rows)
            self._wt_max = (max(r[2] for r in rows), max(r[3] for r in rows))
            self._wt_key = key
        L.check(lib.gfv_transpose_batch(self._wt_desc.data_ptr(), self._wt_n, self._wt_max[0], self._wt_max[1],
                                        L.stream_ptr()), "gfv_transpose_batch")
        self._wt_live = True

    @staticmethod
    def _mlp_names(prefix, ln):
        lin = prefix + ".0" if ln else prefix
        return [f"{lin}.0.weight", f"{lin}.0.bias", f"{lin}.2.weight", f"{lin}.2.bias", f"{lin}.4.weight",
                f"{lin}.4.bias"] + ([f"{prefix}.1.weight", f"{prefix}.1.bias"] if ln else [])

    def mlp3_fwd(self, P, prefix, M, segs, *, ln=True, res=None, in_add=None, want_nores=False, keep=True, w1=None,
                 padd=None, saved_segs=None, nores_from_saved=False):
        names = self._mlp_names(prefix, ln)
        W1, b1, W2, b2, W3, b3 = (P[n] for n in names[:6])
        if w1 is not None:
            W1 = w1
        dev = W1.device
        nout = W3.shape[0]
        would_fuse = (ln and self.fuse_dw and self.f16split and self.hidden == 128 and nout == 128
                      and M >= self._fuse_dw_min and M > self._cbwd_max
                      and (self._fuse_noout or all(sg.width % 32 == 0 for sg in segs)))
        fused_bwd = keep and would_fuse
        would_stats = would_fuse or (ln and self.f16split and nout == 128 and M <= self._cbwd_max)
        lean = fused_bwd and self.recompute
        if keep:
            stats = _empty(dev, M, 2) if would_stats else None
            z1 = _empty(dev, M, 128)
            z2 = _empty(dev, M, 128) if not lean else None
            y3 = _empty(dev, M, 128) if (ln and not lean) else None
        else:
            from_saved = (want_nores and nores_from_saved and would_stats and ln and nout == 128
                          and not (would_fuse and self.recompute))
            z1 = z2 = None
            y3 = _empty(dev, M, 128) if from_saved else None
            stats = _empty(dev, M, 2) if from_saved else None
        out = _empty(dev, M, nout)
        if want_nores and nores_from_saved and y3 is not None and stats is not None and nout == 128:
            want_nores = False
        nores = _empty(dev, M, 128) if want_nores else None
        ops.rowtile_chain(
            M, segs,
            [LayerSpec(W1, b1, L.OP_BIAS_GELU, save=z1), LayerSpec(W2, b2, L.OP_BIAS_GELU, save=z2), LayerSpec(W3, b3)],
            [out], in_add=in_add, fin_op=L.FIN_LN if ln else L.FIN_PLAIN,
            fin_gamma=P[names[6]] if ln else None, fin_beta=P[names[7]] if ln else None, fin_presave=y3,
            res=[res] if res is not None else None, out_nores=nores, fin_stats=stats,
            **(dict(padd=padd[0], padd_s=padd[1], padd_r=padd[2]) if padd is not None else {}))
        if not keep:
            return out, nores, dict(y3=y3, stats=stats)
        saved = dict(z1=z1, z2=z2, y3=y3, segs=segs if saved_segs is None else saved_segs, in_add=in_add, M=M, ln=ln,
                     prefix=prefix, stats=stats, lean=lean, fused=fused_bwd)
        return out, nores, saved

    def _rematerialize(self, P, sv):
        if not sv.get("lean") or sv["z2"] is not None:
            return
        names = self._mlp_names(sv["prefix"], sv["ln"])
        M, dev = sv["M"], sv["z1"].device
        sv["z2"], sv["y3"] = _empty(dev, M, 128), _empty(dev, M, 128)
        ops.rowtile_chain(M, [Seg(sv["z1"])], [LayerSpec(P[names[2]], P[names[3]], L.OP_BIAS_GELU, save=sv["z2"]),
                                              LayerSpec(P[names[4]], P[names[5]])], [sv["y3"]], in_op=L.IN_GELU)

    def mlp3_bwd(self, P, sv, G, grads, *, outs=None, res=None, gadd=None, W1t=None, g_ld=None, g_add=None):
        prefix, M, ln = sv["prefix"], sv["M"], sv["ln"]
        names = self._mlp_names(prefix, ln)
        W1, W2, W3 = P[names[0]], P[names[2]], P[names[4]]
        dev = W1.device
        nout = W3.shape[0]
        W3t, W2t = self._T(W3), self._T(W2)
        if (self.fuse_dw and ln and sv.get("fused", sv.get("stats") is not None) and G.stride(0) == 128 and g_ld is None and gadd is None
                and (outs is not None or (res is None and self._fuse_noout))
                and self._mlp3_bwd_fused(P, sv, G, grads, names, W3t, W2t,
                                         None if outs is None else (W1t if W1t is not None else self._T(W1)), outs, res, g_add)):
            return
        self._rematerialize(P, sv)
        gz2, gz1 = _empty(dev, M, 128), _empty(dev, M, 128)
        part = _empty(dev, ops.ln_rows(M), 2, 128) if ln else None
        g3 = _empty(dev, M, 128) if ln else G
        gseg = Seg(G, width=nout, ld=G.stride(0) if g_ld is None else g_ld)
        kw = dict(in_op=L.IN_LNBWD, in_gamma=P[names[6]], in_aux=sv["y3"], in_save=g3, ln_partial=part,
                  in_stats=sv.get("stats")) if ln else {}
        if gadd is not None:
            kw.update(gadd=gadd[0], gadd_s=gadd[1], gadd_r=gadd[2])
        if g_add is not None:
            assert ln, "the addend is folded into the LayerNorm-backward prologue"
            kw.update(in_add=g_add)
        gs = _empty(dev, 3, ops.gscale_ld(M))
        if outs is not None:
            if W1t is None:
                W1t = self._T(W1)
            have = ops.rowtile_chain(M, [gseg],
                                     [LayerSpec(W3t, None, L.OP_MUL_DGELU, save=gz2, aux=sv["z2"]),
                                      LayerSpec(W2t, None, L.OP_MUL_DGELU, save=gz1, aux=sv["z1"]), LayerSpec(W1t)],
                                     outs, res=res, gscale=gs, **kw)
        else:
            have = ops.rowtile_chain(M, [gseg],
                                     [LayerSpec(W3t, None, L.OP_MUL_DGELU, save=gz2, aux=sv["z2"]),
                                      LayerSpec(W2t, None, L.OP_MUL_DGELU, aux=sv["z1"])], [gz1], gscale=gs, **kw)
        tiles_n = ops.last_ln_rows()
        s0, s1, s2 = (gs[0], gs[1], gs[2]) if have else (None, None, None)
        if not ln and (gadd is not None or g_add is not None):
            s0 = None
        tiles = [self._tile(gz1, 128, sg, in_add=sv["in_add"] if i == 0 else None, gscale=s2,
                            a_op=L.DW_COLSCALE if sg.width <= 16 else 0) for i, sg in enumerate(sv["segs"])]
        tiles.append(self._tile(gz2, 128, Seg(sv["z1"]), a_op=1, gscale=s1))
        tiles.append(self._tile(g3, nout, Seg(sv["z2"]), a_op=1, ldg=(G.stride(0) if g_ld is None else g_ld) if not ln else None,
                                gscale=s0))
        def side():
            wptr, slabs, blen, _ = self._dw_block(
                grads, [(names[0], names[1], len(sv["segs"])), (names[2], names[3], 1), (names[4], names[5], 1)], tiles, M,
                reduce=False)
            off0, _ = grads.block(names[0], names[5])
            pieces = [dict(partial=wptr, out=grads.flat.data_ptr() + 4 * off0, n_chunks=slabs, chunk_stride=blen, rows=1, cols=blen)]
            if ln:
                pieces.append(dict(partial=part, out=self._gview2(grads, names[6], names[7]), n_chunks=tiles_n, chunk_stride=256,
                                   rows=1, cols=256))
            ops.reduce_multi(pieces)
        self.defer(side, gz1, gz2, g3, G, part, gs, sv["z1"], sv["z2"], sv["in_add"], *[sg.t for sg in sv["segs"]],
                   *[sg.idx for sg in sv["segs"]])

    def _mlp3_bwd_fused(self, P, sv, G, grads, names, W3t, W2t, W1t, outs, res, g_add):
        M = sv["M"]
        dev = G.device
        lib = L.load()
        nwg = lib.gfv_rowtile_dw_partials_m(M)
        FL = L.DW_FUSED_FLOATS
        dwp = _empty(dev, nwg, FL)
        gz1 = _empty(dev, M, 128)
        gs = _empty(dev, 3, ops.gscale_ld(M))
        if outs is None:
            layers = [LayerSpec(W3t, None, L.OP_MUL_DGELU, aux=sv["z2"]), LayerSpec(W2t, None, L.OP_MUL_DGELU, aux=sv["z1"])]
            outs = [gz1]
        else:
            layers = [LayerSpec(W3t, None, L.OP_MUL_DGELU, aux=sv["z2"]),
                      LayerSpec(W2t, None, L.OP_MUL_DGELU, save=gz1, aux=sv["z1"]), LayerSpec(W1t)]
        kw = dict(res=res, in_op=L.IN_LNBWD, in_gamma=P[names[6]], in_aux=sv["y3"], in_stats=sv["stats"], dw_partial=dwp, gscale=gs,
                  in_add=g_add, rc=(P[names[2]], P[names[3]], P[names[4]], P[names[5]]) if sv["z2"] is None else None)
        if not ops.rowtile_chain(M, [Seg(G)], layers, outs, query_fused=True, **kw):
            return False
        ops.rowtile_chain(M, [Seg(G)], layers, outs, **kw)
        segs = sv["segs"]

        base = dwp.data_ptr()
        piece = lambda off, out, cols: dict(partial=base + 4 * off, out=out, n_chunks=nwg, chunk_stride=FL, rows=1, cols=cols)
        fused_pieces = [piece(16384 + 128, self._gview2(grads, names[2], names[3]), 16384 + 128),
                        piece(0, self._gview2(grads, names[4], names[5]), 16384 + 128),
                        piece(2 * 16384 + 256, self._gview2(grads, names[6], names[7]), 256)]
        keep = (dwp, gz1, gs, sv["in_add"], *[sg.t for sg in segs], *[sg.idx for sg in segs])

        def side():
            lay = [(names[0], names[1], len(segs))]
            tiles = [self._tile(gz1, 128, sg, in_add=sv["in_add"] if i == 0 else None, gscale=gs[2],
                                a_op=L.DW_COLSCALE if sg.width <= 16 else 0) for i, sg in enumerate(segs)]
            w1, slabs1, blen1, _ = self._dw_block(grads, lay, tiles, M, reduce=False)
            off0, _ = grads.block(names[0], names[1])
            ops.reduce_multi([dict(partial=w1, out=grads.flat.data_ptr() + 4 * off0, n_chunks=slabs1, chunk_stride=blen1, rows=1,
                                   cols=blen1)] + fused_pieces)
        self.defer(side, *keep)
        return True

    @staticmethod
    def _gview2(grads, n0, n1):
        off, length = grads.block(n0, n1)
        return grads.flat[off:off + length]

    @staticmethod
    def _tile(G, n_out, seg, *, a_op=0, a_gamma=None, a_beta=None, in_add=None, ldg=None, g_offset=0, gscale=None):
        return dict(G=G, n_out=n_out, seg=seg, a_op=a_op, a_gamma=a_gamma, a_beta=a_beta, in_add=in_add,
                    ldg=G.stride(0) if ldg is None else ldg, g_offset=g_offset, gscale=gscale)

    def _workspace(self, n_floats, dev):
        if self._dw_ws is None or self._dw_ws.numel() < n_floats or self._dw_ws.device != dev:
            self._dw_ws = torch.zeros(int(n_floats * 1.25) + 1024, dtype=torch.float32, device=dev)
        return self._dw_ws

    def _dw_block(self, grads, layers, tiles, M, row0s=None, reduce=True, ws_offset=0):
        lib = L.load()
        first = layers[0][0]
        last = layers[-1][1] if layers[-1][1] is not None else layers[-1][0]
        off0, blen = grads.block(first, last)
        ct = (L.DwTile * 6)()
        ti = 0
        for li, (wname, bname, nt) in enumerate(layers):
            K = grads.shape[wname][1]
            koff = 0
            for j in range(nt):
                t, c = tiles[ti], ct[ti]
                sg = t["seg"]
                row0 = 0 if row0s is None else row0s[ti]
                c.G = t["G"].data_ptr() + 4 * t["g_offset"]
                c.A = sg.t.data_ptr() + 4 * sg.offset
                c.idx = None if sg.idx is None else sg.idx.data_ptr()
                c.in_add = None if t["in_add"] is None else t["in_add"].data_ptr()
                c.a_gamma = None if t["a_gamma"] is None else t["a_gamma"].data_ptr()
                c.a_beta = None if t["a_beta"] is None else t["a_beta"].data_ptr()
                c.gscale = None if t.get("gscale") is None else t["gscale"].data_ptr()
                c.ldg, c.n_out, c.width, c.ld = t["ldg"], t["n_out"], sg.width, sg.ld
                c.a_op, c.ld_out = t["a_op"], K
                if row0s is None:
                    c.out_off = grads.off[wname] - off0 + koff
                    c.db_off = (grads.off[bname] - off0) if (bname is not None and j == 0) else -1
                    koff += sg.width
                else:
                    c.out_off = grads.off[wname] - off0 + row0 * K
                    c.db_off = (grads.off[bname] - off0 + row0) if bname is not None else -1
                ti += 1
        need = lib.gfv_dw_multi_workspace_floats(M, ti, blen)
        dev = grads.flat.device
        ws = self._workspace(ws_offset + need, dev)
        wptr = ws.data_ptr() + 4 * ws_offset
        L.check(lib.gfv_dw_multi(ct, ti, M, blen, wptr, (grads.flat.data_ptr() + 4 * off0) if reduce else None, 0,
                                 L.stream_ptr()), "gfv_dw_multi")
        if not reduce:
            return wptr, lib.gfv_dw_slabs(M, ti, None), blen, (need + 3) // 4 * 4

    def _dw_jobs(self, grads, jobs, pieces=()):
        lib = L.load()
        dev = grads.flat.device
        needs = []
        for j in jobs:
            first = j["layers"][0][0]
            last = j["layers"][-1][1] if j["layers"][-1][1] is not None else j["layers"][-1][0]
            blen = grads.block(first, last)[1]
            needs.append((lib.gfv_dw_multi_workspace_floats(j["M"], len(j["tiles"]), blen) + 3) // 4 * 4)
        self._workspace(sum(needs) + 8, dev)
        out, off = [], 0
        for j, need in zip(jobs, needs):
            first = j["layers"][0][0]
            last = j["layers"][-1][1] if j["layers"][-1][1] is not None else j["layers"][-1][0]
            wptr, slabs, blen, used = self._dw_block(grads, j["layers"], j["tiles"], j["M"], row0s=j.get("row0s"), reduce=False,
                                                     ws_offset=off)
            assert used <= need
            off0, _ = grads.block(first, last)
            out.append(dict(partial=wptr, out=grads.flat.data_ptr() + 4 * off0, n_chunks=slabs, chunk_stride=blen, rows=1, cols=blen))
            off += need
        out += list(pieces)
        for k in range(0, len(out), 12):
            ops.reduce_multi(out[k:k + 12])

    @staticmethod
    def _put(grads, name, value):
        cmdlist.call(grads.view(name).copy_, value.reshape(grads.shape[name]))

    def gn_fwd(self, P, prefix, x, e, pl, keep=True):
        N, E = pl.N, pl.E
        fuse = self.csr_fuse
        if self.factor:
            W1 = P[f"{prefix}.eb_module.net.0.0.weight"]
            pab = _empty(x.device, N, 256)
            if fuse and ((self._fuse_mask & 1) or N <= self._csr1_max) and ops.stack_ready(W1[:, 0:128], W1[:, 128:256], rows=True):
                nb = _empty(x.device, N, 128) if keep else None
                ops.rowtile_chain(N, [Seg(x, csr=(pl.n_rowptr, pl.n_col_node), save=nb)],
                                  [LayerSpec(W1[:, 0:128], stack=W1[:, 128:256])], [(pab, 256), (pab.data_ptr() + 512, 256)])
            else:
                nb = ops.seg_gather_sum(x, pl.n_rowptr, pl.n_col_node, N)
                ops.rowtile_chain(N, [Seg(nb)], [LayerSpec(W1[:, 0:128], stack=W1[:, 128:256])],
                                  [(pab, 256), (pab.data_ptr() + 512, 256)])
            e_out, e_new, sv_e = self.mlp3_fwd(P, f"{prefix}.eb_module.net", E, [Seg(e)], res=e, want_nores=True,
                                               w1=W1[:, 256:384], padd=(pab, pl.es, pl.er), nores_from_saved=self._agg_ln, keep=keep)
            sv_e["nb"] = nb
        else:
            nb = ops.seg_gather_sum(x, pl.n_rowptr, pl.n_col_node, N)
            e_out, e_new, sv_e = self.mlp3_fwd(P, f"{prefix}.eb_module.net", E, [Seg(nb, pl.es), Seg(nb, pl.er), Seg(e)],
                                               res=e, want_nores=True, nores_from_saved=self._agg_ln, keep=keep)
        if e_new is None:
            ln_names = self._mlp_names(f"{prefix}.eb_module.net", True)
            agg = ops.seg_gather_sum_ln(sv_e["y3"], sv_e["stats"], P[ln_names[6]], P[ln_names[7]], pl.n_rowptr, pl.n_col_edge2, N)
        else:
            agg = ops.seg_gather_sum(e_new.view(2 * E, 64), pl.n_rowptr, pl.n_col_edge2, N)
        if fuse and (self._fuse_mask & 2):
            nbm = _empty(x.device, N, 128) if keep else None
            x_out, _, sv_n = self.mlp3_fwd(P, f"{prefix}.nb_module.net", N,
                                           [Seg(agg, csr=(pl.n_rowptr, pl.n_col_node), scale=pl.inv_deg, save=nbm), Seg(x)],
                                           res=x, saved_segs=[Seg(nbm, width=64, ld=128), Seg(x)] if keep else None, keep=keep)
        else:
            nbm = ops.seg_gather_sum(agg, pl.n_rowptr, pl.n_col_node, N, scale=pl.inv_deg)
            x_out, _, sv_n = self.mlp3_fwd(P, f"{prefix}.nb_module.net", N, [Seg(nbm), Seg(x)], res=x, keep=keep)
        if not keep:
            return x_out, e_out, None
        return x_out, e_out, dict(sv_e=sv_e, sv_n=sv_n, prefix=prefix)

    def _edge_tmp(self, dev):
        if self._etmp is None or self._etmp[0].flat.device != dev:
            e = GradStore(["W1c", "b1", "W2", "b2", "W3", "b3"], [(128, 128), (128,), (128, 128), (128,), (128, 128), (128,)], dev)
            n = GradStore(["W1ab"], [(128, 256)], dev)
            self._etmp = (e, n)
        return self._etmp

    def edge_bwd_factored(self, P, sv, G, grads, pl, gadd):
        prefix, M, N = sv["prefix"], sv["M"], pl.N
        names = self._mlp_names(prefix, True)
        W1, W2, W3 = P[names[0]], P[names[2]], P[names[4]]
        dev = W1.device
        W3t, W2t, W1ct, Wabt = self._T(W3), self._T(W2), self._T(W1, perm="c"), self._T(W1, perm="ab")
        e = sv["segs"][0].t
        if self.fuse_dw and sv.get("fused", sv.get("stats") is not None) and e.stride(0) == 128 and G.stride(0) == 128:
            fused = self._edge_bwd_fused(P, sv, G, grads, pl, gadd, names, (W3t, W2t, W1ct, Wabt))
            if fused is not None:
                return fused
        self._rematerialize(P, sv)
        gz2, gz1, g3, g_e_in = (_empty(dev, M, 128) for _ in range(4))
        part = _empty(dev, ops.ln_rows(M), 2, 128)
        gs = _empty(dev, 3, ops.gscale_ld(M))
        have = ops.rowtile_chain(M, [Seg(G)],
                                 [LayerSpec(W3t, None, L.OP_MUL_DGELU, save=gz2, aux=sv["z2"]),
                                  LayerSpec(W2t, None, L.OP_MUL_DGELU, save=gz1, aux=sv["z1"]), LayerSpec(W1ct)],
                                 [g_e_in], res=[G], in_op=L.IN_LNBWD, in_gamma=P[names[6]], in_aux=sv["y3"], in_save=g3,
                                 ln_partial=part, gadd=gadd[0], gadd_s=gadd[1], gadd_r=gadd[2], gscale=gs, in_stats=sv.get("stats"))
        tiles_n = ops.last_ln_rows()
        s0, s1, s2 = (gs[0], gs[1], gs[2]) if have else (None, None, None)
        g_nb = _empty(dev, N, 128)
        if self.csr_fuse and (self._fuse_mask & 4):
            G_s, G_r = _empty(dev, N, 128), _empty(dev, N, 128)
            ops.rowtile_chain(N, [Seg(gz1, csr=(pl.s_rowptr, pl.s_col), save=G_s), Seg(gz1, csr=(pl.r_rowptr, pl.r_col), save=G_r)],
                              [LayerSpec(Wabt)], [g_nb])
        else:
            G_s = ops.seg_gather_sum(gz1, pl.s_rowptr, pl.s_col, N)
            G_r = ops.seg_gather_sum(gz1, pl.r_rowptr, pl.r_col, N)
            ops.rowtile_chain(N, [Seg(G_s), Seg(G_r)], [LayerSpec(Wabt)], [g_nb])
        nb = sv["nb"]
        def side():
            tmpE, tmpN = self._edge_tmp(dev)
            gW1 = grads.view(names[0])
            lib = L.load()
            self._workspace(lib.gfv_dw_multi_workspace_floats(M, 3, tmpE.block("W1c", "b3")[1])
                            + lib.gfv_dw_multi_workspace_floats(N, 2, tmpN.block("W1ab", "W1ab")[1]) + 8, dev)
            w1, slabs1, blen1, used = self._dw_block(tmpE, [("W1c", "b1", 1), ("W2", "b2", 1), ("W3", "b3", 1)],
                                                     [self._tile(gz1, 128, Seg(e), gscale=s2),
                                                      self._tile(gz2, 128, Seg(sv["z1"]), a_op=1, gscale=s1),
                                                      self._tile(g3, 128, Seg(sv["z2"]), a_op=1, gscale=s0)], M, reduce=False)
            w2, slabs2, blen2, _ = self._dw_block(tmpN, [("W1ab", None, 2)],
                                                  [self._tile(G_s, 128, Seg(nb)), self._tile(G_r, 128, Seg(nb))], N,
                                                  reduce=False, ws_offset=used)
            assert w2 == w1 + 4 * used
            off, length = grads.block(names[1], names[5])
            o2, l2 = tmpE.block("b1", "b3")
            assert l2 == length
            ops.reduce_multi([
                dict(partial=w1, out=gW1.data_ptr() + 4 * 256, n_chunks=slabs1, chunk_stride=blen1, rows=128, cols=128, ld_out=384),
                dict(partial=w1 + 4 * o2, out=grads.flat.data_ptr() + 4 * off, n_chunks=slabs1, chunk_stride=blen1, rows=1, cols=l2),
                dict(partial=w2, out=gW1.data_ptr(), n_chunks=slabs2, chunk_stride=blen2, rows=128, cols=256, ld_out=384),
                dict(partial=part, out=self._gview2(grads, names[6], names[7]), n_chunks=tiles_n, chunk_stride=256, rows=1,
                     cols=256)])
        self.defer(side, gz1, gz2, g3, G_s, G_r, nb, e, part, gs, sv["z1"], sv["z2"])
        return g_nb, g_e_in

    def _edge_bwd_fused(self, P, sv, G, grads, pl, gadd, names, Wt):
        M, N = sv["M"], pl.N
        W3t, W2t, W1ct, Wabt = Wt
        dev = G.device
        e = sv["segs"][0].t
        lib = L.load()
        nwg = lib.gfv_rowtile_dw_partials_m(M)
        lean = sv["z2"] is None
        FL = L.DW_FUSED_FLOATS
        dwp = _empty(dev, nwg, FL)
        gz1, g_e_in = _empty(dev, M, 128), _empty(dev, M, 128)
        layers = [LayerSpec(W3t, None, L.OP_MUL_DGELU, aux=sv["z2"]), LayerSpec(W2t, None, L.OP_MUL_DGELU, save=gz1, aux=sv["z1"]),
                  LayerSpec(W1ct)]
        gs = _empty(dev, 3, ops.gscale_ld(M))
        kw = dict(res=[G], in_op=L.IN_LNBWD, in_gamma=P[names[6]], in_aux=sv["y3"], in_stats=sv["stats"], gadd=gadd[0], gadd_s=gadd[1],
                  gadd_r=gadd[2], dw_partial=dwp, gscale=gs,
                  rc=(P[names[2]], P[names[3]], P[names[4]], P[names[5]]) if lean else None)
        if not ops.rowtile_chain(M, [Seg(G)], layers, [g_e_in], query_fused=True, **kw):
            return None
        ops.rowtile_chain(M, [Seg(G)], layers, [g_e_in], **kw)
        g_nb = _empty(dev, N, 128)
        if self.csr_fuse and (self._fuse_mask & 4):
            G_s, G_r = _empty(dev, N, 128), _empty(dev, N, 128)
            ops.rowtile_chain(N, [Seg(gz1, csr=(pl.s_rowptr, pl.s_col), save=G_s), Seg(gz1, csr=(pl.r_rowptr, pl.r_col), save=G_r)],
                              [LayerSpec(Wabt)], [g_nb])
        else:
            G_s = ops.seg_gather_sum(gz1, pl.s_rowptr, pl.s_col, N)
            G_r = ops.seg_gather_sum(gz1, pl.r_rowptr, pl.r_col, N)
            ops.rowtile_chain(N, [Seg(G_s), Seg(G_r)], [LayerSpec(Wabt)], [g_nb])
        nb = sv["nb"]

        def side():
            tmpE, tmpN = self._edge_tmp(dev)
            gW1 = grads.view(names[0])
            base = dwp.data_ptr()
            piece = lambda off, out, rows, cols, ld_out=None: dict(partial=base + 4 * off, out=out, n_chunks=nwg, chunk_stride=FL,
                                                                   rows=rows, cols=cols, ld_in=cols, ld_out=cols if ld_out is None else ld_out)
            pieces = [piece(16384 + 128, self._gview2(grads, names[2], names[3]), 1, 16384 + 128),
                      piece(0, self._gview2(grads, names[4], names[5]), 1, 16384 + 128),
                      piece(2 * 16384 + 256, self._gview2(grads, names[6], names[7]), 1, 256)]
            lay = [("W1c", "b1", 1)]
            self._workspace(lib.gfv_dw_multi_workspace_floats(M, 1, tmpE.block("W1c", "b1")[1])
                            + lib.gfv_dw_multi_workspace_floats(N, 2, tmpN.block("W1ab", "W1ab")[1]) + 8, dev)
            w1, slabs1, blen1, used = self._dw_block(tmpE, lay, [self._tile(gz1, 128, Seg(e), gscale=gs[2])], M, reduce=False)
            ob1, lb1 = tmpE.block("b1", "b1")
            pieces += [dict(partial=w1, out=gW1.data_ptr() + 4 * 256, n_chunks=slabs1, chunk_stride=blen1, rows=128, cols=128, ld_out=384),
                       dict(partial=w1 + 4 * ob1, out=grads.view(names[1]), n_chunks=slabs1, chunk_stride=blen1, rows=1, cols=128)]
            w2, slabs2, blen2, _ = self._dw_block(tmpN, [("W1ab", None, 2)],
                                                  [self._tile(G_s, 128, Seg(nb)), self._tile(G_r, 128, Seg(nb))], N, reduce=False,
                                                  ws_offset=used)
            pieces.append(dict(partial=w2, out=gW1.data_ptr(), n_chunks=slabs2, chunk_stride=blen2, rows=128, cols=256, ld_out=384))
            ops.reduce_multi(pieces)
        self.defer(side, dwp, gz1, e, G_s, G_r, nb, gs)
        return g_nb, g_e_in

    def gn_bwd(self, P, sv, g_x_out, g_e_out, grads, pl):
        N, E = pl.N, pl.E
        dev = g_x_out.device
        prefix = sv["prefix"]
        W1n = P[f"{prefix}.nb_module.net.0.0.weight"]
        W1t = self._T(W1n, perm=True)
        g_x_in, g_nbm = _empty(dev, N, 128), _empty(dev, N, 64)
        self.mlp3_bwd(P, sv["sv_n"], g_x_out, grads, outs=[g_x_in, (g_nbm, 64)], res=[g_x_out, None], W1t=W1t)
        g_agg = ops.seg_gather_sum(g_nbm, pl.n_rowptr, pl.n_col_node, N, src_scale=pl.inv_deg)
        if "nb" in sv["sv_e"]:
            g_nb, g_e_in = self.edge_bwd_factored(P, sv["sv_e"], g_e_out, grads, pl, (g_agg, pl.es, pl.er))
        else:
            gnb2, g_e_in = _empty(dev, E, 256), _empty(dev, E, 128)
            self.mlp3_bwd(P, sv["sv_e"], g_e_out, grads, outs=[(gnb2, 256), (gnb2.data_ptr() + 512, 256), g_e_in],
                          res=[None, None, g_e_out], gadd=(g_agg, pl.es, pl.er))
            g_nb = ops.seg_gather_sum(gnb2.view(2 * E, 128), pl.n_rowptr, pl.n_col_edge2, N)
        ops.seg_gather_sum(g_nb, pl.n_rowptr, pl.n_col_node, N, out=g_x_in, accumulate=True)
        last = self._defer_mode and getattr(self, "_last_gn", False)
        tail_main, tail_split = self._tail_cfg(pl)
        self.flush(on_main=last and tail_main >= 3, split=tail_split if last else 0)
        return g_x_in, g_e_in

    def trans_fwd(self, P, prefix, xg, emb, pl, keep=True):
        lib = L.load()
        st = L.stream_ptr()
        N, B = pl.N, pl.B
        dev = xg.device
        a = f"{prefix}.Attn"
        fx_in, fx_mid, x_mid = _empty(dev, N, 128), _empty(dev, N, 128), _empty(dev, N, 128)
        ops.rowtile_chain(N, [Seg(xg)],
                          [LayerSpec(P[f"{a}.in_project_fx.weight"], P[f"{a}.in_project_fx.bias"],
                                     stack=P[f"{a}.in_project_x.weight"], bias2=P[f"{a}.in_project_x.bias"])],
                          [fx_mid, x_mid], in_add=emb, in_save=fx_in)
        w = _empty(dev, N, 256)
        temp = P[f"{a}.graph_temperature"]
        partial = _empty(dev, pl.n_chunks, 256, 17)
        if self._slice_fuse:
            L.check(lib.gfv_slice_softmax_token(x_mid.data_ptr(), P[f"{a}.in_project_slice.weight"].data_ptr(),
                                                P[f"{a}.in_project_slice.bias"].data_ptr(), temp.data_ptr(), fx_mid.data_ptr(),
                                                pl.chunk_beg.data_ptr(), pl.chunk_end.data_ptr(), pl.n_chunks, w.data_ptr(),
                                                partial.data_ptr(), st), "slice_softmax_token")
        else:
            L.check(lib.gfv_slice_softmax_fwd(x_mid.data_ptr(), P[f"{a}.in_project_slice.weight"].data_ptr(),
                                              P[f"{a}.in_project_slice.bias"].data_ptr(), temp.data_ptr(), w.data_ptr(), N,
                                              st), "slice_softmax_fwd")
            L.check(lib.gfv_slice_token_partial(w.data_ptr(), fx_mid.data_ptr(), pl.chunk_beg.data_ptr(),
                                                pl.chunk_end.data_ptr(), pl.n_chunks, partial.data_ptr(), st), "token_partial")
        partial, gptr = self._graph_partials(partial, pl)
        token, norm = (_empty(dev, B, 8, 32, 16), _empty(dev, B, 8, 32)) if keep else (None, None)
        attn, out_token = _empty(dev, B, 8, 32, 32) if keep else None, _empty(dev, B, 8, 32, 16)
        L.check(lib.gfv_slice_attention_fwd(partial.data_ptr(), gptr.data_ptr(), B, P[f"{a}.to_q.weight"].data_ptr(),
                                            P[f"{a}.to_k.weight"].data_ptr(), P[f"{a}.to_v.weight"].data_ptr(),
                                            L.ptr(token), L.ptr(norm), L.ptr(attn), out_token.data_ptr(), st),
                "slice_attention_fwd")
        if not keep:
            del partial, fx_mid, x_mid
        out_x = _empty(dev, N, 128)
        L.check(lib.gfv_deslice(w.data_ptr(), out_token.data_ptr(), pl.batch.data_ptr(), out_x.data_ptr(), N,
                                4 if B == 1 else 0, st), "deslice")
        if not keep:
            del w
        fx1, z = (_empty(dev, N, 128), _empty(dev, N, 256)) if keep else (None, None)
        out = _empty(dev, N, 128)
        if not (self._trans_fuse and (N >= self._trans_fuse_min or self._trans_fuse_fwd_small) and ops.trans_mlp_fwd(
                out_x, fx_in, P[f"{a}.to_out.0.weight"], P[f"{a}.to_out.0.bias"], P[f"{prefix}.ln_2.weight"], P[f"{prefix}.ln_2.bias"],
                P[f"{prefix}.mlp.linear_pre.0.weight"], P[f"{prefix}.mlp.linear_pre.0.bias"], P[f"{prefix}.mlp.linear_post.weight"],
                P[f"{prefix}.mlp.linear_post.bias"], fx1, z, out)):
            if not keep:
                fx1, z = _empty(dev, N, 128), _empty(dev, N, 256)
            ops.rowtile_chain(N, [Seg(out_x)], [LayerSpec(P[f"{a}.to_out.0.weight"], P[f"{a}.to_out.0.bias"])], [fx1],
                              res=[fx_in])
            ops.rowtile_chain(N, [Seg(fx1)],
                              [LayerSpec(P[f"{prefix}.mlp.linear_pre.0.weight"], P[f"{prefix}.mlp.linear_pre.0.bias"])],
                              [(z, 256), (z.data_ptr() + 512, 256)], in_op=L.IN_LN, in_gamma=P[f"{prefix}.ln_2.weight"],
                              in_beta=P[f"{prefix}.ln_2.bias"])
            ops.rowtile_chain(N, [Seg(z, width=128, ld=256), Seg(z, width=128, ld=256, offset=128)],
                              [LayerSpec(P[f"{prefix}.mlp.linear_post.weight"], P[f"{prefix}.mlp.linear_post.bias"])], [out],
                              in_op=L.IN_GELU, res=[fx1])
        if not keep:
            return out, None
        sv = dict(prefix=prefix, fx_in=fx_in, fx_mid=fx_mid, x_mid=x_mid, w=w, token=token, norm=norm, attn=attn,
                  out_token=out_token, out_x=out_x, fx1=fx1, z=z)
        return out, sv

    def _graph_partials(self, partial, pl):
        out = _empty(partial.device, pl.B, 256, 17)
        L.check(L.load().gfv_reduce_partials_seg(partial.data_ptr(), pl.gchunk_ptr.data_ptr(), pl.B, 256 * 17,
                                                 out.data_ptr(), L.stream_ptr()), "reduce_partials_seg")
        return out, pl.gunit_ptr

    def trans_bwd(self, P, sv, g_out, grads, pl, g_add=None):
        lib = L.load()
        st = L.stream_ptr()
        N, B = pl.N, pl.B
        dev = g_out.device
        prefix = sv["prefix"]
        a = f"{prefix}.Attn"
        z, fx1, fx_in = sv["z"], sv["fx1"], sv["fx_in"]
        zsegs = [Seg(z, width=128, ld=256), Seg(z, width=128, ld=256, offset=128)]
        Wpost, Wpre = P[f"{prefix}.mlp.linear_post.weight"], P[f"{prefix}.mlp.linear_pre.0.weight"]
        g_z = _empty(dev, N, 256)
        g_sum = _empty(dev, N, 128) if g_add is not None else None
        gs = _empty(dev, 3, ops.gscale_ld(N))
        tiles = ops.rowtile_tiles(N)
        part = _empty(dev, ops.ln_rows(N), 2, 128)
        g_fx1, g_out_x = _empty(dev, N, 128), _empty(dev, N, 128)
        gam2, bet2 = P[f"{prefix}.ln_2.weight"], P[f"{prefix}.ln_2.bias"]
        fused = (self._trans_fuse and (N >= self._trans_fuse_min or self._trans_fuse_fwd_small) and
                 ops.trans_mlp_bwd(g_out, g_add, g_sum, z, fx1, self._T(Wpost), self._T(Wpre), self._T(P[f"{a}.to_out.0.weight"]),
                                   gam2, g_z, g_fx1, g_out_x, part, gs[0]))
        if fused:
            have = True
            tiles = lib.gfv_trans_mlp_ln_rows(N)
        else:
            have = ops.rowtile_chain(N, [Seg(g_out)], [LayerSpec(self._T(Wpost), None, L.OP_MUL_DGELU, aux=z)],
                                     [(g_z, 256), (g_z.data_ptr() + 512, 256)], in_add=g_add, in_save=g_sum, gscale=gs)
        s_post = gs[0] if have else None
        if g_add is not None:
# ... 190 lines not shown
                                       sums.data_ptr(), losses.data_ptr(), B, st), "graph_loss")
            if want_outputs:
                L.check(lib.gfv_cell_to_node(phic.data_ptr(), pl.nrow.data_ptr(), pl.ncell.data_ptr(), pl.pos.data_ptr(),
                                             pl.centroid.data_ptr(), pl.node_type.data_ptr(), pl.y.data_ptr(),
                                             pl.batch.data_ptr(), pl.uvp_dim.data_ptr(), pl.sigma.data_ptr(), phi.data_ptr(),
                                             self.smooth | (2 if raw_outputs else 0), uvp_node.data_ptr(), N, st), "cell_to_node")
            if train_loss is not None:
                L.check(lib.gfv_train_loss_dev(losses.data_ptr(), B, train_loss[0].data_ptr(), train_loss[1].data_ptr(),
                                               train_loss[2].data_ptr(), st), "train_loss")
        if want_outputs and raw_outputs:
            uvp_cell = phic[:, 0:3].clone()
        if not keep:
            return losses, uvp_node, uvp_cell, None
        sv = dict(Ff=Ff, cres=cres, sums=sums, phi=phi, grad=grad, phic=phic, gradc=gradc)
        return losses, uvp_node, uvp_cell, sv

    def fvm_bwd(self, sv, gloss, pl):
        lib = L.load()
        if self._fvm_fuse and not self.nc:
            dev = gloss.device
            gFf, gphi, grhs = _empty(dev, pl.E, 16), _empty(dev, pl.N, 8), _empty(dev, pl.N, 8, pl.M)
            gdec = _empty(dev, pl.N, 3)
            L.check(lib.gfv_fvm_bwd_fused(self._fvm_mesh(pl), sv["cres"].data_ptr(), sv["sums"].data_ptr(), gloss.data_ptr(),
                                          sv["Ff"].data_ptr(), sv["dec"].data_ptr(), gFf.data_ptr(), gphi.data_ptr(), grhs.data_ptr(),
                                          gdec.data_ptr(), L.stream_ptr()), "fvm_bwd_fused")
            return gdec
        gphi = self.fvm_core_bwd(sv, gloss, pl)
        gdec = _empty(gloss.device, pl.N, 3)
        L.check(lib.gfv_phi_bwd(gphi.data_ptr(), sv["dec"].data_ptr(), pl.node_type.data_ptr(), gdec.data_ptr(), pl.N,
                                self.mode, L.stream_ptr()), "phi_bwd")
        return gdec

    def fvm_core_bwd(self, sv, gloss, pl):
        lib = L.load()
        st = L.stream_ptr()
        N, E, C = pl.N, pl.E, pl.C
        dev = gloss.device
        gc, gFf = _empty(dev, C, 4), _empty(dev, E, 16)
        gphi, ggrad = _empty(dev, N, 8), _empty(dev, N, 16)
        L.check(lib.gfv_fvm_bwd_ex(sv["cres"].data_ptr(), sv["sums"].data_ptr(), gloss.data_ptr(), sv["Ff"].data_ptr(),
                                pl.cbatch.data_ptr(), pl.theta.data_ptr(), pl.sigma.data_ptr(), pl.dt.data_ptr(),
                                pl.frow.data_ptr(), pl.fk.data_ptr(), pl.kcell.data_ptr(), pl.kS.data_ptr(),
                                pl.ftype.data_ptr(), pl.n_rowptr.data_ptr(), pl.n_col_edge2.data_ptr(), pl.nrow.data_ptr(),
                                pl.ncell.data_ptr(), pl.crow.data_ptr(), pl.pos.data_ptr(), pl.fpos.data_ptr(),
                                pl.centroid.data_ptr(), pl.area.data_ptr(), gc.data_ptr(), gFf.data_ptr(), gphi.data_ptr(),
                                ggrad.data_ptr(), N, E, C, self.nc, None if not self.nc else sv["gradc"].data_ptr(),
                                None if not self.nc else sv["phic"].data_ptr(), st), "fvm_bwd")
        grhs = _empty(dev, N, 8, pl.M)
        L.check(lib.gfv_wlsq_bwd_ex(ggrad.data_ptr(), None, pl.An.data_ptr(), pl.rn.data_ptr(), pl.xo_rowptr.data_ptr(),
                                    pl.xo_in.data_ptr(), pl.xo_B.data_ptr(), pl.sumB.data_ptr(), grhs.data_ptr(),
                                    gphi.data_ptr(), N, pl.M, st), "wlsq_bwd")
        return gphi

    def prep_fwd(self, x, buffers, pl, norm_global, accumulate, want_edge_attr15=True, x_raw=None):
        lib = L.load()
        st = L.stream_ptr()
        N, E, B = pl.N, pl.E, pl.B
        dev = x.device
        assert x.is_contiguous() and x.shape[1] == 12
        if os.environ.get("GFV_PREP_FUSE", "1") == "0" or B > 1024:
            return self._prep_fwd_unfused(x, buffers, pl, norm_global, accumulate, want_edge_attr15, x_raw)
        stats = _empty(dev, B, 6)
        ws = self._prep_ws
        need = lib.gfv_prep_workspace_bytes(B) // 4
        if ws is None or ws.numel() < need or ws.device != dev:
            ws = self._prep_ws = torch.zeros(need, dtype=torch.float32, device=dev)
        mean_std = _empty(dev, 18)
        fused_norm = False
        if norm_global:
            sync = accumulate and (self.dist_world > 1 or self.dist_force)
            if accumulate:
                nb = lib.gfv_normalizer_blocks(N)
                pws = _empty(dev, nb, 18)
                src = x if x_raw is None else x_raw
                if sync:
                    from . import parallel
                    before = parallel.snapshot_normalizer(buffers)

                def update(acc):
                    L.check(lib.gfv_normalizer_update(src.data_ptr(), 12, N, 1 if acc else 0, buffers["acc_count"].data_ptr(),
                                                      buffers["num_accumulations"].data_ptr(), buffers["acc_sum"].data_ptr(),
                                                      buffers["acc_sum_squared"].data_ptr(), pws.data_ptr(),
                                                      mean_std.data_ptr(), L.stream_ptr()), "normalizer_update")
                update(True)
                if sync:
                    parallel.allreduce_normalizer(buffers, before, self.dist_world, self.dist_group, force=self.dist_force)
                    update(False)
            else:
                fused_norm = True
        own_raw = x_raw is None
        if own_raw:
            x_raw = _empty(dev, N, 12)
        L.check(lib.gfv_prep_stats((x if own_raw else x_raw).data_ptr(), 12, pl.gnode_ptr.data_ptr(), B, stats.data_ptr(), ws.data_ptr(),
                                   x_raw.data_ptr() if own_raw else None,
                                   buffers["acc_count"].data_ptr() if fused_norm else None,
                                   buffers["acc_sum"].data_ptr() if fused_norm else None,
                                   buffers["acc_sum_squared"].data_ptr() if fused_norm else None,
                                   mean_std.data_ptr() if fused_norm else None, st), "prep_stats")
        uv_old = _empty(dev, N, 2)
        ea16 = _empty(dev, E, 16)
        ea15 = _empty(dev, E, 15) if want_edge_attr15 else None
        L.check(lib.gfv_prep_apply(x_raw.data_ptr(), x.data_ptr(), pl.batch.data_ptr(), stats.data_ptr(), pl.uvp_dim.data_ptr(),
                                   mean_std.data_ptr(), 1 if norm_global else 0, uv_old.data_ptr(), N, pl.pos.data_ptr(),
                                   pl.es.data_ptr(), pl.er.data_ptr(), ea16.data_ptr(),
                                   None if ea15 is None else ea15.data_ptr(), E, st), "prep_apply")
        return uv_old, ea16, ea15

    def _prep_fwd_unfused(self, x, buffers, pl, norm_global, accumulate, want_edge_attr15=True, x_raw=None):
        lib = L.load()
        st = L.stream_ptr()
        N, E, B = pl.N, pl.E, pl.B
        dev = x.device
        if x_raw is not None:
            cmdlist.call(x.copy_, x_raw)
        stats = _empty(dev, B, 6)
        nws = _empty(dev, B, 64 * 12)
        L.check(lib.gfv_graph_norm_stats_ws(x.data_ptr(), 12, pl.gnode_ptr.data_ptr(), B, stats.data_ptr(), nws.data_ptr(), st),
                "norm_stats")
        mean_std = _empty(dev, 18)
        if norm_global:
            nb = lib.gfv_normalizer_blocks(N)
            pws = _empty(dev, nb, 18)
            sync = accumulate and (self.dist_world > 1 or self.dist_force)
            if sync:
                from . import parallel
                before = parallel.snapshot_normalizer(buffers)

            def update(acc):
                L.check(lib.gfv_normalizer_update(x.data_ptr(), 12, N, 1 if acc else 0, buffers["acc_count"].data_ptr(),
                                                  buffers["num_accumulations"].data_ptr(), buffers["acc_sum"].data_ptr(),
                                                  buffers["acc_sum_squared"].data_ptr(), pws.data_ptr(),
                                                  mean_std.data_ptr(), L.stream_ptr()), "normalizer_update")
            update(accumulate)
            if sync:
                parallel.allreduce_normalizer(buffers, before, self.dist_world, self.dist_group, force=self.dist_force)
                update(False)
        uv_old = _empty(dev, N, 2)
        L.check(lib.gfv_node_prep(x.data_ptr(), 12, pl.batch.data_ptr(), stats.data_ptr(), pl.uvp_dim.data_ptr(),
                                  mean_std.data_ptr(), 1 if norm_global else 0, uv_old.data_ptr(), N, st), "node_prep")
        ea16 = _empty(dev, E, 16)
        ea15 = _empty(dev, E, 15) if want_edge_attr15 else None
        L.check(lib.gfv_edge_attr(x.data_ptr(), 12, pl.pos.data_ptr(), pl.es.data_ptr(), pl.er.data_ptr(), ea16.data_ptr(),
                                  None if ea15 is None else ea15.data_ptr(), E, st), "edge_attr")
        return uv_old, ea16, ea15

    def simulator_fwd(self, P, x, ea16, pl, prefix="simulator", keep=True):
        N, E = pl.N, pl.E
        xn, _, sv_nenc = self.mlp3_fwd(P, f"{prefix}.encoder.nb_encoder", N, [Seg(x, width=12, ld=12)], keep=keep)
        en, _, sv_eenc = self.mlp3_fwd(P, f"{prefix}.encoder.eb_encoder", E, [Seg(ea16, width=15, ld=16)], keep=keep)
        procs = []
        if self.net == "EPD":
            blocks = []
            for ig in range(self.mp):
                xn, en, sv = self.gn_fwd(P, f"{prefix}.GN_block_list.{ig}", xn, en, pl, keep=keep)
                blocks.append(sv)
            procs.append(dict(blocks=blocks, trans=None))
        else:
            pps = [prefix] if self.net == "TransFVGN_v1" else [f"{prefix}.processpr_list.{ip}" for ip in range(self.n_proc)]
            for pp in pps:
                emb = xn
                blocks = []
                for ig in range(self.mp):
                    xn, en, sv = self.gn_fwd(P, f"{pp}.GN_block_list.{ig}", xn, en, pl, keep=keep)
                    blocks.append(sv)
                xn, svt = self.trans_fwd(P, f"{pp}.TransBlock", xn, emb, pl, keep=keep)
                procs.append(dict(blocks=blocks, trans=svt))
        dec, _, sv_dec = self.mlp3_fwd(P, f"{prefix}.decoder.node_decode_module", N, [Seg(xn)], ln=False, keep=keep)
        if not keep:
            return dec, None
        return dec, dict(sv_nenc=sv_nenc, sv_eenc=sv_eenc, procs=procs, sv_dec=sv_dec)

    def simulator_bwd(self, P, sv, g_dec, grads, pl):
        N, E = pl.N, pl.E
        dev = g_dec.device
        g_x = _empty(dev, N, 128)
        self.mlp3_bwd(P, sv["sv_dec"], g_dec, grads, outs=[g_x])
        self.flush()
        g_e = None
        pending = None
        for proc in reversed(sv["procs"]):
            g_emb = None
            if proc["trans"] is not None:
                g_x = self.trans_bwd(P, proc["trans"], g_x, grads, pl, g_add=pending)
                pending = None
                g_emb = g_x
            elif pending is not None:
                g_x, pending = g_x + pending, None
            for blk in reversed(proc["blocks"]):
                if g_e is None:
                    if self._zero_e is None or self._zero_e.shape[0] != E or self._zero_e.device != dev:
                        self._zero_e = torch.zeros((E, 128), dtype=torch.float32, device=dev)
                    g_e = self._zero_e
                self._last_gn = proc is sv["procs"][0] and blk is proc["blocks"][0]
                g_x, g_e = self.gn_bwd(P, blk, g_x, g_e, grads, pl)
            if g_emb is not None:
                pending = g_emb
            if self.bucket_hook is not None and proc is sv["procs"][-1] and len(sv["procs"]) > 1:
                self.flush()
                self.bucket_hook()
        tail = self._tail_cfg(pl)[0] if self._defer_mode else 0
        self.mlp3_bwd(P, sv["sv_eenc"], g_e, grads)
        self.flush(on_main=tail >= 2)
        self.mlp3_bwd(P, sv["sv_nenc"], g_x, grads, g_add=pending)
        self.flush(on_main=tail >= 1)

    def forward(self, P, buffers, x, pl, *, norm_global=True, accumulate=True, want_outputs=True, want_edge_attr15=True,
                before_prep=None, x_raw=None, train_loss=None, keep=True, static_weights=False):
        if static_weights:
            prev = self._wi_static_enter(P)
        else:
            with self.fork():
                prev = self._wi_enter("fwd", P)
        try:
            if before_prep is not None:
                before_prep()
            uv_old, ea16, ea15 = self.prep_fwd(x, buffers, pl, norm_global, accumulate, want_edge_attr15, x_raw=x_raw)
            if not static_weights:
                self.join()
            dec, sv_sim = self.simulator_fwd(P, x, ea16, pl, keep=keep)
        finally:
            if not static_weights:
                self._wi_exit("fwd", prev)
            elif self.f16split:
                ops.set_weight_images(prev)
        if not keep:
            del ea16
        losses, uvp_node, uvp_cell, sv_fvm = self.fvm_fwd(dec, uv_old, pl, want_outputs, train_loss=train_loss, keep=keep)
        return losses, uvp_node, uvp_cell, ea15, (dict(sim=sv_sim, fvm=sv_fvm) if keep else None)

    def backward(self, P, ctx, gloss, grads, pl):
        with self.fork():
            self.prepare_transposes(P)
            prev = self._wi_enter("bwd", P)
        try:
            g_dec = self.fvm_bwd(ctx["fvm"], gloss, pl)
            self.join()
            self.simulator_bwd(P, ctx["sim"], g_dec, grads, pl)
            self.join()
        finally:
            self._wt_live = False
            self._wi_exit("bwd", prev)
        return grads
```

### gen-fvgn-steady_amd/gfv/lib.py

```python
from __future__ import annotations

import ctypes as C
import os

import torch

HERE = os.path.dirname(os.path.abspath(__file__))
LIB_PATH = os.environ.get("GFV_LIB", os.path.join(HERE, "libgfv.so"))

c_float_p = C.c_void_p
c_int_p = C.c_void_p

OP_NONE, OP_BIAS_GELU, OP_MUL_DGELU = 0, 1, 2
IN_NONE, IN_GELU, IN_LN, IN_LNBWD = 0, 1, 2, 3
FIN_PLAIN, FIN_LN, FIN_LNBWD = 0, 1, 2
CHAIN_ROW_OWNER, CHAIN_COLUMN_OWNER = 1, 2
DW_COLSCALE = 8


class Seg(C.Structure):
    _fields_ = [("ptr", C.c_void_p), ("idx", C.c_void_p), ("width", C.c_int32), ("ld", C.c_int32),
                ("csr_rowptr", C.c_void_p), ("csr_scale", C.c_void_p), ("save", C.c_void_p)]


class Layer(C.Structure):
    _fields_ = [("W", C.c_void_p), ("bias", C.c_void_p), ("K", C.c_int32), ("N", C.c_int32), ("op", C.c_int32),
                ("ldw", C.c_int32), ("save", C.c_void_p), ("aux", C.c_void_p), ("Wh", C.c_void_p),
                ("bias2", C.c_void_p)]


class RowtileArgs(C.Structure):
    _fields_ = [
        ("M", C.c_int32), ("nseg", C.c_int32), ("seg", Seg * 3), ("in_add", C.c_void_p), ("in_op", C.c_int32),
        ("nlayers", C.c_int32), ("in_gamma", C.c_void_p), ("in_beta", C.c_void_p), ("in_aux", C.c_void_p),
        ("gadd", C.c_void_p), ("gadd_s", C.c_void_p), ("gadd_r", C.c_void_p), ("in_save", C.c_void_p),
        ("ln_partial", C.c_void_p), ("layer", Layer * 3), ("fin_op", C.c_int32), ("hidden", C.c_int32),
        ("fin_gamma", C.c_void_p), ("fin_beta", C.c_void_p), ("fin_aux", C.c_void_p), ("fin_presave", C.c_void_p),
        ("res", C.c_void_p * 3), ("res_ld", C.c_int32 * 3), ("out_ld", C.c_int32 * 3), ("out", C.c_void_p * 3),
        ("out_nores", C.c_void_p), ("padd", C.c_void_p), ("padd_s", C.c_void_p), ("padd_r", C.c_void_p),
        ("padd_ld", C.c_int32), ("flags", C.c_int32), ("wmax", C.c_void_p),
        ("gscale", C.c_void_p), ("gscale_ld", C.c_int32), ("product_form", C.c_int32),
        ("fin_stats", C.c_void_p), ("in_stats", C.c_void_p), ("dw_partial", C.c_void_p), ("dw_partial_stride", C.c_int64),
        ("dw_in", C.c_void_p), ("dw_in_ld", C.c_int32), ("reserved2_", C.c_int32),
        ("rc_Wh", C.c_void_p * 2), ("rc_bias", C.c_void_p * 2),
    ]


ABI_VERSION = 3

DW_FUSED_FLOATS = 2 * 128 * 128 + 4 * 128


class WimgDesc(C.Structure):
    _fields_ = [("W", C.c_void_p), ("img", C.c_void_p), ("ldw", C.c_int32), ("N", C.c_int32), ("K", C.c_int32),
                ("reserved", C.c_int32)]


class DwTile(C.Structure):
    _fields_ = [("G", C.c_void_p), ("A", C.c_void_p), ("idx", C.c_void_p), ("in_add", C.c_void_p),
                ("a_gamma", C.c_void_p), ("a_beta", C.c_void_p), ("ldg", C.c_int32), ("n_out", C.c_int32),
                ("width", C.c_int32), ("ld", C.c_int32), ("a_op", C.c_int32), ("ld_out", C.c_int32),
                ("out_off", C.c_int64), ("db_off", C.c_int64), ("gscale", C.c_void_p)]


class ReducePiece(C.Structure):
    _fields_ = [("partial", C.c_void_p), ("out", C.c_void_p), ("chunk_stride", C.c_int64), ("n_chunks", C.c_int32),
                ("rows", C.c_int32), ("cols", C.c_int32), ("ld_in", C.c_int32), ("ld_out", C.c_int32), ("reserved", C.c_int32)]


class TransMlp(C.Structure):
    _fields_ = [("x", C.c_void_p), ("res", C.c_void_p), ("img_out", C.c_void_p), ("img_pre", C.c_void_p), ("img_post", C.c_void_p),
                ("b_out", C.c_void_p), ("b_pre", C.c_void_p), ("b_post", C.c_void_p), ("gamma", C.c_void_p), ("beta", C.c_void_p),
                ("wmax", C.c_void_p), ("fx1", C.c_void_p), ("z", C.c_void_p), ("out", C.c_void_p), ("M", C.c_int32),
                ("reserved", C.c_int32)]


class TransMlpBwd(C.Structure):
    _fields_ = [("g", C.c_void_p), ("g_add", C.c_void_p), ("g_sum", C.c_void_p), ("z", C.c_void_p), ("fx1", C.c_void_p),
                ("img_post_t", C.c_void_p), ("img_pre_t", C.c_void_p), ("img_out_t", C.c_void_p), ("gamma", C.c_void_p),
                ("wmax", C.c_void_p), ("g_z", C.c_void_p), ("g_fx1", C.c_void_p), ("g_out_x", C.c_void_p),
                ("ln_partial", C.c_void_p), ("gscale", C.c_void_p), ("M", C.c_int32), ("reserved", C.c_int32)]


class FvmMesh(C.Structure):
    _fields_ = ([("N", C.c_int32), ("E", C.c_int32), ("C", C.c_int32), ("B", C.c_int32), ("terms", C.c_int32), ("mode", C.c_int32),
                 ("smooth", C.c_int32), ("reserved", C.c_int32)]
                + [(n, C.c_void_p) for n in (
                    "node_type", "batch", "ftype", "cbatch", "gcell_ptr", "pos", "fpos", "y", "centroid", "area", "theta", "sigma",
                    "uvp_dim", "dt", "crow", "kcell", "kS", "frow", "fk", "nfrow", "nfcol2", "nrow", "ncell", "An", "rn",
                    "xo_rowptr", "xo_in", "xo_B", "sumB")])


POOL_MAX_GRAPHS, POOL_MAX_ATTRS, POOL_ROW_HEAD = 64, 56, 8
POOL_COPY, POOL_ADD, POOL_ROWPTR, POOL_FILL = 0, 1, 2, 3


class PoolArgs(C.Structure):
    _fields_ = [("table_host", C.c_void_p), ("table_dev", C.c_void_p), ("n_entries", C.c_int32), ("n_attrs", C.c_int32),
                ("max_graphs", C.c_int32), ("slice_chunk", C.c_int32), ("max_chunks", C.c_int64),
                ("attr_info", C.c_int32 * POOL_MAX_ATTRS), ("dst", C.c_void_p * POOL_MAX_ATTRS),
                ("dst_cap_words", C.c_int64 * POOL_MAX_ATTRS), ("small", C.c_void_p * 6), ("B", C.c_int32),
                ("reserved", C.c_int32), ("idx", C.c_int32 * POOL_MAX_GRAPHS)]


_lib = None

_SIGNATURES = {
    "gfv_pool_args_bytes": (C.c_size_t, []),
    "gfv_pool_table_bytes": (C.c_size_t, [C.c_int32, C.c_int32]),
    "gfv_pool_table_check": (C.c_int, [C.c_void_p, C.c_int32, C.c_int32, C.c_void_p]),
    "gfv_pool_assemble": (C.c_int, [C.POINTER(PoolArgs), C.c_void_p]),
    "gfv_pool_payback": (C.c_int, [C.c_void_p, C.c_void_p, C.c_int32, C.c_int32, C.c_int32, C.c_void_p, C.c_int32, C.c_void_p,
                                   C.c_int64, C.c_void_p, C.c_void_p]),
    "gfv_abi_version": (C.c_int, []),
    "gfv_struct_size": (C.c_int, [C.c_int32]),
    "gfv_seg_gather_sum": (C.c_int, [C.c_void_p, C.c_void_p, C.c_void_p, C.c_void_p, C.c_void_p, C.c_void_p, C.c_int32,
                                     C.c_int32, C.c_int32, C.c_void_p]),
    "gfv_seg_gather_sum_nnz": (C.c_int, [C.c_void_p, C.c_void_p, C.c_void_p, C.c_void_p, C.c_void_p, C.c_void_p, C.c_int32,
                                         C.c_int32, C.c_int32, C.c_int64, C.c_void_p]),
    "gfv_seg_gather_sum_ex": (C.c_int, [C.c_void_p, C.c_void_p, C.c_void_p, C.c_void_p, C.c_void_p, C.c_void_p, C.c_int32,
                                        C.c_int32, C.c_int32, C.c_int64, C.c_int64, C.c_void_p]),
    "gfv_seg_gather_sum_ln": (C.c_int, [C.c_void_p, C.c_void_p, C.c_void_p, C.c_void_p, C.c_void_p, C.c_void_p, C.c_void_p, C.c_int32,
                                        C.c_int64, C.c_int64, C.c_void_p]),
    "gfv_transpose_batch": (C.c_int, [C.c_void_p, C.c_int32, C.c_int32, C.c_int32, C.c_void_p]),
    "gfv_status_flags": (C.c_int, [C.POINTER(C.c_int32)]),
    "gfv_status_mirror": (C.c_int, [C.POINTER(C.POINTER(C.c_int32))]),
    "gfv_status_publish": (C.c_int, [C.c_void_p]),
    "gfv_profile_enable": (C.c_int, [C.c_int]),
    "gfv_profile_collect": (C.c_int, [C.c_int, C.POINTER(C.c_double)]),
    "gfv_profile_reset": (C.c_int, []),
    "gfv_profile_set_sizes": (C.c_int, [C.c_double, C.c_double]),
    "gfv_gather_pair": (C.c_int, [C.c_void_p, C.c_void_p, C.c_void_p, C.c_void_p, C.c_void_p, C.c_int32, C.c_int32,
                                  C.c_void_p]),
    "gfv_get_limit": (C.c_int, [C.c_int32]),
    "gfv_set_limit": (C.c_int, [C.c_int32, C.c_int32]),
    "gfv_limit_name": (C.c_char_p, [C.c_int32]),
    "gfv_rowtile_tiles": (C.c_int, [C.c_int32]),
    "gfv_rowtile_chain": (C.c_int, [C.POINTER(RowtileArgs), C.c_void_p]),
    "gfv_rowtile_last_path": (C.c_int, []),
    "gfv_rowtile_ln_rows": (C.c_int, [C.c_int32]),
    "gfv_rowtile_last_ln_rows": (C.c_int, []),
    "gfv_rowtile_dw_partials": (C.c_int, []),
    "gfv_rowtile_dw_partials_m": (C.c_int, [C.c_int32]),
    "gfv_rowtile_fuses_dw": (C.c_int, [C.POINTER(RowtileArgs)]),
    "gfv_dw_chunks": (C.c_int, [C.c_int32]),
    "gfv_linear_dw_workspace_floats": (C.c_size_t, [C.c_int32, C.c_int32, C.c_int32]),
    "gfv_linear_dw": (C.c_int, [C.c_void_p, C.c_int32, C.c_int32, C.POINTER(Seg), C.c_int32, C.c_void_p, C.c_int32,
                                C.c_int32, C.c_void_p, C.c_void_p, C.c_void_p, C.c_int32, C.c_void_p]),
    "gfv_linear_dw_ex": (C.c_int, [C.c_void_p, C.c_int32, C.c_int32, C.POINTER(Seg), C.c_int32, C.c_void_p, C.c_int32,
                                   C.c_void_p, C.c_void_p, C.c_int32, C.c_void_p, C.c_int32, C.c_void_p, C.c_void_p,
                                   C.c_int32, C.c_void_p]),
    "gfv_linear_dw_gs": (C.c_int, [C.c_void_p, C.c_int32, C.c_int32, C.POINTER(Seg), C.c_int32, C.c_void_p, C.c_int32,
                                   C.c_void_p, C.c_void_p, C.c_int32, C.c_void_p, C.c_void_p, C.c_void_p, C.c_void_p,
                                   C.c_int32, C.c_void_p]),
    "gfv_dw_slabs": (C.c_int, [C.c_int32, C.c_int32, C.c_void_p]),
    "gfv_dw_multi_workspace_floats": (C.c_size_t, [C.c_int32, C.c_int32, C.c_int64]),
    "gfv_dw_multi": (C.c_int, [C.POINTER(DwTile), C.c_int32, C.c_int32, C.c_int64, C.c_void_p, C.c_void_p, C.c_int32,
                               C.c_void_p]),
    "gfv_reduce_partials": (C.c_int, [C.c_void_p, C.c_int32, C.c_int32, C.c_void_p, C.c_int32, C.c_void_p]),
    "gfv_concat_offsets": (C.c_int, [C.c_void_p, C.c_int32, C.c_int32, C.c_void_p]),
    "gfv_f16split_enabled": (C.c_int, []),
    "gfv_set_f16split": (C.c_int, [C.c_int32]),
    "gfv_set_f16split_thread": (C.c_int, [C.c_int32]),
    "gfv_hidden_size": (C.c_int, []),
    "gfv_set_hidden_size": (C.c_int, [C.c_int32]),
    "gfv_weight_image_bytes": (C.c_size_t, [C.c_int32, C.c_int32]),
    "gfv_weight_absmax": (C.c_int, [C.c_void_p, C.c_int32, C.c_void_p, C.c_void_p]),
    "gfv_weight_images": (C.c_int, [C.c_void_p, C.c_int32, C.c_int64, C.c_void_p, C.c_void_p]),
    "gfv_weight_images_form": (C.c_int, [C.c_void_p]),
    "gfv_reduce_partials_2d": (C.c_int, [C.c_void_p, C.c_int32, C.c_int64, C.c_int32, C.c_int32, C.c_int32, C.c_void_p, C.c_void_p]),
    "gfv_reduce_multi": (C.c_int, [C.POINTER(ReducePiece), C.c_int32, C.c_void_p]),
    "gfv_reduce_partials_seg": (C.c_int, [C.c_void_p, C.c_void_p, C.c_int32, C.c_int32, C.c_void_p, C.c_void_p]),
    "gfv_transpose": (C.c_int, [C.c_void_p, C.c_int32, C.c_void_p, C.c_int32, C.c_int32, C.c_void_p]),
    "gfv_slice_softmax_fwd": (C.c_int, [C.c_void_p, C.c_void_p, C.c_void_p, C.c_void_p, C.c_void_p, C.c_int32, C.c_void_p]),
    "gfv_slice_softmax_bwd_blocks": (C.c_int, [C.c_int32]),
    "gfv_slice_softmax_bwd": (C.c_int, [C.c_void_p, C.c_void_p, C.c_void_p, C.c_void_p, C.c_void_p, C.c_void_p, C.c_void_p, C.c_void_p, C.c_int32, C.c_void_p]),
    "gfv_slice_token_partial": (C.c_int, [C.c_void_p, C.c_void_p, C.c_void_p, C.c_void_p, C.c_int32, C.c_void_p, C.c_void_p]),
    "gfv_slice_attention_fwd": (C.c_int, [C.c_void_p, C.c_void_p, C.c_int32, C.c_void_p, C.c_void_p, C.c_void_p, C.c_void_p, C.c_void_p, C.c_void_p, C.c_void_p, C.c_void_p]),
    "gfv_slice_attention_bwd": (C.c_int, [C.c_void_p, C.c_void_p, C.c_int32, C.c_void_p, C.c_void_p, C.c_void_p, C.c_void_p, C.c_void_p, C.c_void_p, C.c_void_p, C.c_void_p, C.c_void_p, C.c_void_p]),
    "gfv_deslice": (C.c_int, [C.c_void_p, C.c_void_p, C.c_void_p, C.c_void_p, C.c_int32, C.c_int32, C.c_void_p]),
    "gfv_slice_gw": (C.c_int, [C.c_void_p, C.c_void_p, C.c_void_p, C.c_void_p, C.c_void_p, C.c_int32, C.c_int32, C.c_void_p]),
    "gfv_slice_softmax_token": (C.c_int, [C.c_void_p] * 7 + [C.c_int32, C.c_void_p, C.c_void_p, C.c_void_p]),
    "gfv_slice_post_bwd": (C.c_int, [C.c_void_p] * 14 + [C.c_int32, C.c_int32, C.c_void_p]),
    "gfv_phi_fwd": (C.c_int, [C.c_void_p, C.c_void_p, C.c_void_p, C.c_void_p, C.c_void_p, C.c_int32, C.c_int32, C.c_void_p]),
    "gfv_phi_bwd": (C.c_int, [C.c_void_p, C.c_void_p, C.c_void_p, C.c_void_p, C.c_int32, C.c_int32, C.c_void_p]),
    "gfv_wlsq_fwd": (C.c_int, [C.c_void_p, C.c_void_p, C.c_void_p, C.c_void_p, C.c_void_p, C.c_void_p, C.c_void_p, C.c_int32, C.c_void_p]),
    "gfv_wlsq_bwd": (C.c_int, [C.c_void_p, C.c_void_p, C.c_void_p, C.c_void_p, C.c_void_p, C.c_void_p, C.c_void_p, C.c_void_p, C.c_void_p, C.c_int32, C.c_void_p]),
    "gfv_wlsq_fwd_ex": (C.c_int, [C.c_void_p] * 8 + [C.c_int32, C.c_int32, C.c_void_p]),
    "gfv_wlsq_bwd_ex": (C.c_int, [C.c_void_p] * 10 + [C.c_int32, C.c_int32, C.c_void_p]),
    "gfv_wlsq_fwd_full": (C.c_int, [C.c_void_p, C.c_void_p, C.c_void_p, C.c_void_p, C.c_void_p, C.c_void_p, C.c_void_p, C.c_void_p, C.c_int32, C.c_void_p]),
    "gfv_wlsq_bwd_full": (C.c_int, [C.c_void_p, C.c_void_p, C.c_void_p, C.c_void_p, C.c_void_p, C.c_void_p, C.c_void_p, C.c_void_p, C.c_void_p, C.c_int32, C.c_void_p]),
    "gfv_face_fwd": (C.c_int, [C.c_void_p, C.c_void_p, C.c_void_p, C.c_void_p, C.c_void_p, C.c_void_p, C.c_void_p, C.c_void_p, C.c_void_p, C.c_int32, C.c_void_p]),
    "gfv_cell_fwd": (C.c_int, [C.c_void_p, C.c_void_p, C.c_void_p, C.c_void_p, C.c_void_p, C.c_void_p, C.c_void_p, C.c_void_p, C.c_void_p, C.c_void_p, C.c_void_p, C.c_void_p, C.c_void_p, C.c_void_p, C.c_void_p, C.c_void_p, C.c_void_p, C.c_void_p, C.c_void_p, C.c_int32, C.c_void_p]),
    "gfv_cell_fwd_ex": (C.c_int, [C.c_void_p] * 19 + [C.c_int32, C.c_int32, C.c_void_p, C.c_void_p]),
    "gfv_graph_loss": (C.c_int, [C.c_void_p, C.c_void_p, C.c_void_p, C.c_void_p, C.c_void_p, C.c_void_p, C.c_int32, C.c_void_p]),
    "gfv_cell_to_node": (C.c_int, [C.c_void_p, C.c_void_p, C.c_void_p, C.c_void_p, C.c_void_p, C.c_void_p, C.c_void_p, C.c_void_p, C.c_void_p, C.c_void_p, C.c_void_p, C.c_int32, C.c_void_p, C.c_int32, C.c_void_p]),
    "gfv_fvm_bwd": (C.c_int, [C.c_void_p, C.c_void_p, C.c_void_p, C.c_void_p, C.c_void_p, C.c_void_p, C.c_void_p, C.c_void_p, C.c_void_p, C.c_void_p, C.c_void_p, C.c_void_p, C.c_void_p, C.c_void_p, C.c_void_p, C.c_void_p, C.c_void_p, C.c_void_p, C.c_void_p, C.c_void_p, C.c_void_p, C.c_void_p, C.c_void_p, C.c_void_p, C.c_void_p, C.c_void_p, C.c_int32, C.c_int32, C.c_int32, C.c_void_p]),
    "gfv_fvm_bwd_ex": (C.c_int, [C.c_void_p] * 26 + [C.c_int32] * 4 + [C.c_void_p] * 3),
    "gfv_khop_workspace_ints": (C.c_size_t, [C.c_int32, C.c_int32]),
    "gfv_khop_count": (C.c_int, [C.c_void_p, C.c_void_p, C.c_int32, C.c_int32, C.c_int32, C.c_void_p, C.c_void_p]),
    "gfv_khop_fill": (C.c_int, [C.c_int32, C.c_int32, C.c_void_p, C.c_void_p, C.c_void_p, C.c_void_p]),
    "gfv_wlsq_moments": (C.c_int, [C.c_void_p] * 6 + [C.c_int32, C.c_int32, C.c_void_p]),
    "gfv_interp2_fwd": (C.c_int, [C.c_void_p] * 6 + [C.c_int32, C.c_void_p, C.c_void_p, C.c_int32, C.c_int32, C.c_void_p]),
    "gfv_interp2_bwd": (C.c_int, [C.c_void_p] * 6 + [C.c_int32, C.c_void_p, C.c_void_p, C.c_int32, C.c_int32, C.c_void_p]),
    "gfv_graph_norm_stats": (C.c_int, [C.c_void_p, C.c_int32, C.c_void_p, C.c_int32, C.c_void_p, C.c_void_p]),
    "gfv_graph_norm_workspace_bytes": (C.c_size_t, [C.c_int32]),
    "gfv_graph_norm_stats_ws": (C.c_int, [C.c_void_p, C.c_int32, C.c_void_p, C.c_int32, C.c_void_p, C.c_void_p, C.c_void_p]),
    "gfv_normalizer_blocks": (C.c_int, [C.c_int32]),
    "gfv_normalizer_update": (C.c_int, [C.c_void_p, C.c_int32, C.c_int32, C.c_int32, C.c_void_p, C.c_void_p, C.c_void_p, C.c_void_p, C.c_void_p, C.c_void_p, C.c_void_p]),
    "gfv_node_prep": (C.c_int, [C.c_void_p, C.c_int32, C.c_void_p, C.c_void_p, C.c_void_p, C.c_void_p, C.c_int32, C.c_void_p, C.c_int32, C.c_void_p]),
    "gfv_edge_attr": (C.c_int, [C.c_void_p, C.c_int32, C.c_void_p, C.c_void_p, C.c_void_p, C.c_void_p, C.c_void_p, C.c_int32, C.c_void_p]),
    "gfv_adam_step_dev": (C.c_int, [C.c_void_p, C.c_void_p, C.c_void_p, C.c_void_p, C.c_int64, C.c_void_p, C.c_void_p, C.c_void_p]),
    "gfv_prep_workspace_bytes": (C.c_size_t, [C.c_int32]),
    "gfv_prep_stats": (C.c_int, [C.c_void_p, C.c_int32, C.c_void_p, C.c_int32, C.c_void_p, C.c_void_p, C.c_void_p, C.c_void_p,
                                 C.c_void_p, C.c_void_p, C.c_void_p, C.c_void_p]),
    "gfv_prep_apply": (C.c_int, [C.c_void_p, C.c_void_p, C.c_void_p, C.c_void_p, C.c_void_p, C.c_void_p, C.c_int32, C.c_void_p,
                                 C.c_int32, C.c_void_p, C.c_void_p, C.c_void_p, C.c_void_p, C.c_void_p, C.c_int32, C.c_void_p]),
    "gfv_fvm_fwd_tail": (C.c_int, [C.POINTER(FvmMesh)] + [C.c_void_p] * 11),
    "gfv_fvm_bwd_fused": (C.c_int, [C.POINTER(FvmMesh)] + [C.c_void_p] * 10),
    "gfv_adam_state_init": (C.c_int, [C.c_void_p, C.c_double, C.c_double, C.c_float, C.c_void_p]),
    "gfv_train_loss_dev": (C.c_int, [C.c_void_p, C.c_int32, C.c_void_p, C.c_void_p, C.c_void_p, C.c_void_p]),
    "gfv_train_loss": (C.c_int, [C.c_void_p, C.c_int32, C.c_float, C.c_float, C.c_float, C.c_void_p, C.c_void_p, C.c_void_p]),
    "gfv_plan_create": (C.c_int, [C.c_void_p, C.POINTER(C.c_void_p), C.c_void_p]),
    "gfv_plan_destroy": (C.c_int, [C.c_void_p]),
    "gfv_plan_table": (C.c_int, [C.c_void_p, C.c_int32, C.POINTER(C.c_void_p), C.POINTER(C.c_int64)]),
    "gfv_plan_sizes": (C.c_int, [C.c_void_p, C.POINTER(C.c_int64)]),
    "gfv_rollout_advance": (C.c_int, [C.c_void_p, C.c_void_p, C.c_void_p, C.c_int32, C.c_void_p, C.c_void_p, C.c_void_p, C.c_int32,
                                      C.c_int32, C.c_void_p, C.c_void_p, C.c_void_p, C.c_int32, C.c_void_p, C.c_void_p]),
    "gfv_trans_mlp_fwd": (C.c_int, [C.POINTER(TransMlp), C.c_void_p]),
    "gfv_trans_mlp_bwd": (C.c_int, [C.POINTER(TransMlpBwd), C.c_void_p]),
    "gfv_trans_mlp_ln_rows": (C.c_int, [C.c_int32]),
    "gfv_record_begin": (C.c_int, []),
    "gfv_record_count": (C.c_int, []),
    "gfv_record_end": (C.c_int64, []),
    "gfv_record_length": (C.c_int, [C.c_int64]),
    "gfv_record_replay": (C.c_int, [C.c_int64, C.c_int32, C.c_int32]),
    "gfv_record_free": (C.c_int, [C.c_int64]),
    "gfv_stream_wait": (C.c_int, [C.c_void_p, C.c_void_p]),
    "gfv_record_delay_side": (C.c_int, [C.c_int64, C.c_void_p, C.c_int32]),
}


class PlanDesc(C.Structure):
    _fields_ = [("n_nodes", C.c_int64), ("n_faces", C.c_int64), ("n_cells", C.c_int64), ("n_incidences", C.c_int64),
                ("n_stencil_pairs", C.c_int64), ("n_support_pairs", C.c_int64),
                ("edge_index", C.c_void_p), ("cells_node", C.c_void_p), ("cells_face", C.c_void_p),
                ("cells_index", C.c_void_p), ("face_node_x", C.c_void_p), ("support_edge", C.c_void_p)]


PLAN_TABLES = ("ES", "ER", "N_ROWPTR", "N_COL_NODE", "N_COL_EDGE2", "INV_DEG", "S_ROWPTR", "S_COL", "R_ROWPTR", "R_COL",
               "X_ROWPTR", "X_OUT", "X_ORDER", "XO_ROWPTR", "XO_IN", "XO_ORDER", "CROW", "K_ORDER", "KFACE", "KNODE", "KCELL",
               "FROW", "FK", "NROW", "NCELL")


def declared_symbols():
    return list(_SIGNATURES)


def register(name, restype, argtypes):
    _SIGNATURES[name] = (restype, argtypes)
    if _lib is not None:
        fn = getattr(_lib, name)
        fn.restype, fn.argtypes = restype, argtypes


_recording = None


def load(raw=False):
    global _lib
    if _lib is not None:
        return _lib if (_recording is None or raw) else _recording
    if not os.path.exists(LIB_PATH):
        raise RuntimeError(
            f"libgfv.so not found at {LIB_PATH}: build it with `python gen-fvgn-steady_amd/gfv/build.py` "
            "(hipcc --offload-arch=gfx950). The HIP extension is mandatory; there is no fallback path.")
    lib = C.CDLL(LIB_PATH)
    for name, (restype, argtypes) in _SIGNATURES.items():
        fn = getattr(lib, name)
        fn.restype, fn.argtypes = restype, argtypes
    if lib.gfv_abi_version() != ABI_VERSION:
        raise RuntimeError(f"libgfv.so has ABI {lib.gfv_abi_version()}, this binding is written for {ABI_VERSION}: rebuild it "
                           "(python gen-fvgn-steady_amd/gfv/build.py)")
    for which, st in enumerate((Seg, Layer, RowtileArgs, WimgDesc, DwTile, ReducePiece, PlanDesc, TransMlp, TransMlpBwd, FvmMesh)):
        if lib.gfv_struct_size(which) != C.sizeof(st):
            raise RuntimeError(f"libgfv.so: struct {st.__name__} is {lib.gfv_struct_size(which)} bytes in the library, "
                               f"{C.sizeof(st)} in the binding")
    if lib.gfv_pool_args_bytes() != C.sizeof(PoolArgs):
        raise RuntimeError(f"libgfv.so: gfv_pool_args_t is {lib.gfv_pool_args_bytes()} bytes in the library, "
                           f"{C.sizeof(PoolArgs)} in the binding")
    _lib = lib
    return lib if (_recording is None or raw) else _recording


def stream_ptr():
    return C.c_void_p(torch.cuda.current_stream().cuda_stream)

# ... 99 lines not shown
```

### gen-fvgn-steady_amd/gfv/ops.py

```python
from __future__ import annotations

import ctypes as C

import torch

from . import lib as L


def _p(t):
    return None if t is None else t.data_ptr()


def seg_gather_sum(src, rowptr, col, n_rows, scale=None, src_scale=None, out=None, accumulate=False):
    lib = L.load()
    F = src.shape[-1]
    L.f32c(src)
    if out is None:
        assert not accumulate
        out = torch.empty((n_rows, F), dtype=torch.float32, device=src.device)
    rc = lib.gfv_seg_gather_sum_ex(_p(src), _p(L.i32c(rowptr)), _p(L.i32c(col)), _p(scale), _p(src_scale), _p(out),
                                   n_rows, F, 1 if accumulate else 0, col.shape[0], src.shape[0], L.stream_ptr())
    L.check(rc, "gfv_seg_gather_sum")
    return out


def seg_gather_sum_ln(y, stats, gamma, beta, rowptr, col, n_rows, out=None):
    lib = L.load()
    assert y.dim() == 2 and y.shape[1] == 128 and y.is_contiguous() and stats.shape == (y.shape[0], 2) and stats.is_contiguous()
    if out is None:
        out = torch.empty((n_rows, 64), dtype=torch.float32, device=y.device)
    rc = lib.gfv_seg_gather_sum_ln(_p(L.f32c(y)), _p(L.f32c(stats)), _p(L.f32c(gamma)), _p(L.f32c(beta)), _p(L.i32c(rowptr)),
                                   _p(L.i32c(col)), _p(out), n_rows, col.shape[0], 2 * y.shape[0], L.stream_ptr())
    L.check(rc, "gfv_seg_gather_sum_ln")
    return out


def gather_pair(a, s, r, base=None, out=None):
    lib = L.load()
    F = a.shape[-1]
    E = s.shape[0]
    if out is None:
        out = torch.empty((E, 2 * F), dtype=torch.float32, device=a.device)
    rc = lib.gfv_gather_pair(_p(L.f32c(a)), _p(L.i32c(s)), _p(L.i32c(r)), _p(base), _p(out), E, F, L.stream_ptr())
    L.check(rc, "gfv_gather_pair")
    return out


def transpose(w, out=None, col0=0, ncols=None):
    lib = L.load()
    rows, cols = w.shape
    ncols = cols - col0 if ncols is None else ncols
    if out is None:
        out = torch.empty((ncols, rows), dtype=torch.float32, device=w.device)
    rc = lib.gfv_transpose(L.f32c(w).data_ptr() + 4 * col0, cols, _p(out), rows, ncols, L.stream_ptr())
    L.check(rc, "gfv_transpose")
    return out


def reduce_partials(partial, n_chunks, n, out=None, accumulate=False):
    lib = L.load()
    if out is None:
        out = torch.empty((n,), dtype=torch.float32, device=partial.device)
    rc = lib.gfv_reduce_partials(_p(partial), n_chunks, n, _p(out), 1 if accumulate else 0, L.stream_ptr())
    L.check(rc, "gfv_reduce_partials")
    return out


def reduce_multi(pieces):
    lib = L.load()
    arr = (L.ReducePiece * len(pieces))()
    for a, p in zip(arr, pieces):
        a.partial = p["partial"].data_ptr() if torch.is_tensor(p["partial"]) else p["partial"]
        a.out = p["out"].data_ptr() if torch.is_tensor(p["out"]) else p["out"]
        a.n_chunks, a.chunk_stride, a.rows, a.cols = p["n_chunks"], p["chunk_stride"], p["rows"], p["cols"]
        a.ld_in = p.get("ld_in", p["cols"])
        a.ld_out = p.get("ld_out", p["cols"])
    L.check(lib.gfv_reduce_multi(arr, len(pieces), L.stream_ptr()), "gfv_reduce_multi")


def csr_prologue_enabled():
    import os
    return os.environ.get("GFV_CSR_FUSE", "1") != "0"


def rowtile_tiles(M):
    return (M + 63) // 64


def ln_rows(M):
    return (M + 31) // 32


def last_ln_rows():
    return L.load().gfv_rowtile_last_ln_rows()


def gscale_ld(M):
    return (M + 127) // 128 * 8


class Seg:

    def __init__(self, t, idx=None, width=None, ld=None, offset=0, csr=None, scale=None, save=None):
        self.t, self.idx = t, idx
        self.width = t.shape[-1] if width is None else width
        self.ld = t.stride(0) if ld is None else ld
        self.offset = offset
        self.csr, self.scale, self.save = csr, scale, save
        assert csr is None or idx is None

    def fill(self, cs):
        cs.ptr = self.t.data_ptr() + 4 * self.offset
        cs.idx = _p(self.idx) if self.csr is None else self.csr[1].data_ptr()
        cs.width = self.width
        cs.ld = self.ld
        cs.csr_rowptr = None if self.csr is None else self.csr[0].data_ptr()
        cs.csr_scale = _p(self.scale)
        cs.save = _p(self.save)


class LayerSpec:
    def __init__(self, W, bias=None, op=L.OP_NONE, save=None, aux=None, stack=None, bias2=None, stack_cols=None):
        self.W, self.bias, self.op, self.save, self.aux = W, bias, op, save, aux
        self.stack, self.bias2, self.stack_cols = stack, bias2, stack_cols


class WeightImages:

    def __init__(self, device, wmax):
        self.device, self.wmax = device, wmax
        self.images = {}
        self.valid = set()
        self.static = []
        self._desc, self._desc_keys, self._max_frags = None, (), 0
        self._retired = []
        self._bf = None

    def add_static(self, tensors):
        for t in tensors:
            st = t.untyped_storage()
            self.static.append((st.data_ptr(), st.data_ptr() + st.nbytes()))
        self.static.sort()

    def _is_static(self, ptr):
        import bisect
        i = bisect.bisect_right(self.static, (ptr, 1 << 62)) - 1
        return i >= 0 and self.static[i][0] <= ptr < self.static[i][1]

    @staticmethod
    def _parts(key, img):
        if key[0] != "stack":
            return [(key, img.data_ptr())]
        per = img.numel() // (len(key) - 1)
        return [(k, img.data_ptr() + i * per) for i, k in enumerate(key[1:])]

    @staticmethod
    def _upload(items, device):
        parts = [pt for key, img in items for pt in WeightImages._parts(key, img)]
        descs = (L.WimgDesc * len(parts))()
        for d, (key, dst) in zip(descs, parts):
            d.W, d.img, d.ldw, d.N, d.K = key[0], dst, key[1], key[2], key[3]
        return torch.frombuffer(bytearray(bytes(descs)), dtype=torch.uint8).to(device), len(parts)

    def lookup(self, W, stack=None):
        key = (W.data_ptr(), W.stride(0), W.shape[0], W.shape[1])
        if stack is not None:
            assert W.shape == stack.shape and W.shape[0] == 128
            key = ("stack", key, (stack.data_ptr(), stack.stride(0), stack.shape[0], stack.shape[1]))
        bf = L.load().gfv_f16split_enabled() == 3
        if bf != self._bf:
            self._bf = bf
            self.invalidate()
            if self.images and not torch.cuda.is_current_stream_capturing():
                self.build()
        img = self.images.get(key)
        if img is not None:
            return img.data_ptr() if key in self.valid else 0
        blocks = key[1:] if key[0] == "stack" else (key,)
        if not all(self._is_static(k[0]) for k in blocks) or torch.cuda.is_current_stream_capturing():
            return 0
        lib = L.load()
        nbytes = sum(lib.gfv_weight_image_bytes(k[2], k[3]) for k in blocks)
        img = torch.empty((nbytes,), dtype=torch.uint8, device=self.device)
        desc, nd = self._upload([(key, img)], self.device)
        L.check(lib.gfv_weight_images(desc.data_ptr(), nd, img.numel() // 32, self.wmax.data_ptr(), L.stream_ptr()),
                "gfv_weight_images")
        self.images[key] = img
        self.valid.add(key)
        return img.data_ptr()

    def build(self):
        if not self.images:
            return
        if len(self._desc_keys) != len(self.images) and not torch.cuda.is_current_stream_capturing():
            self._desc_keys = tuple(self.images)
            self._retired.append(self._desc)
            self._desc, self._ndesc = self._upload(list(self.images.items()), self.device)
            self._max_frags = max(img.numel() for img in self.images.values()) // 32
        if self._desc is None:
            return
        L.check(L.load().gfv_weight_images(self._desc.data_ptr(), self._ndesc, self._max_frags,
                                           self.wmax.data_ptr(), L.stream_ptr()), "gfv_weight_images")
        self._bf = L.load().gfv_f16split_enabled() == 3
        self.valid = set(self._desc_keys)

    def invalidate(self):
        self.valid = set()


_WI = None


def stack_ready(Wa, Wb, rows=False):
    return (_WI is not None and L.load().gfv_f16split_enabled() and Wa.shape == Wb.shape and Wa.shape[0] == 128
            and _WI.lookup(Wa, Wb) != 0)


def set_weight_images(wi):
    global _WI
    prev, _WI = _WI, wi
    return prev


def rowtile_chain(M, segs, layers, outs, *, in_add=None, in_op=L.IN_NONE, in_gamma=None, in_beta=None, in_aux=None,
                  gadd=None, gadd_s=None, gadd_r=None, in_save=None, ln_partial=None, fin_op=L.FIN_PLAIN,
                  fin_gamma=None, fin_beta=None, fin_aux=None, fin_presave=None, res=None, out_nores=None,
                  padd=None, padd_s=None, padd_r=None, wimg=None, gscale=None, family=0, fin_stats=None, in_stats=None,
                  dw_partial=None, query_fused=False, rc=None):
    lib = L.load()
    wi = wimg if wimg is not None else _WI
    if layers[-1].stack is not None:
        ly = layers[-1]
        h = wi.lookup(ly.W, ly.stack) if (wi is not None and len(layers) == 1 and lib.gfv_f16split_enabled()) else 0
        if not h:
            assert len(layers) == 1 and len(outs) == 2 and res is None and out_nores is None
            kw = dict(in_add=in_add, in_op=in_op, in_gamma=in_gamma, in_beta=in_beta, wimg=wimg)
            rowtile_chain(M, segs, [LayerSpec(ly.W, ly.bias, ly.op)], [outs[0]], in_save=in_save, **kw)
            rowtile_chain(M, segs, [LayerSpec(ly.stack, ly.bias2, ly.op)], [outs[1]], **kw)
            return
    a = L.RowtileArgs()
    a.M = M
    a.nseg = len(segs)
    for i, s in enumerate(segs):
        s.fill(a.seg[i])
    a.in_add = _p(in_add)
    a.in_op = in_op
    a.nlayers = len(layers)
    a.in_gamma, a.in_beta, a.in_aux = _p(in_gamma), _p(in_beta), _p(in_aux)
    a.gadd, a.gadd_s, a.gadd_r = _p(gadd), _p(gadd_s), _p(gadd_r)
    a.in_save, a.ln_partial = _p(in_save), _p(ln_partial)
    for i, ly in enumerate(layers):
        cl = a.layer[i]
        stacked = ly.stack is not None or ly.stack_cols is not None
        cl.W, cl.bias, cl.bias2 = (None if stacked else _p(ly.W)), _p(ly.bias), _p(ly.bias2)
        cl.N = ly.W.shape[0] * (2 if ly.stack is not None else 1)
        cl.K = ly.W.shape[1] * (2 if ly.stack_cols is not None else 1)
        assert ly.W.stride(1) == 1
        cl.ldw = 0 if (ly.stack is not None or ly.stack_cols is not None) else ly.W.stride(0)
        cl.op = ly.op
        cl.save, cl.aux = _p(ly.save), _p(ly.aux)
    if wi is not None:
        hs = [wi.lookup(ly.W, ly.stack if ly.stack is not None else ly.stack_cols) for ly in layers]
        if all(hs):
            for i, h in enumerate(hs):
                a.layer[i].Wh = h
            a.wmax = wi.wmax.data_ptr()
    a.fin_op = fin_op
    a.fin_gamma, a.fin_beta, a.fin_aux, a.fin_presave = _p(fin_gamma), _p(fin_beta), _p(fin_aux), _p(fin_presave)
    for i, o in enumerate(outs):
        t, ld = o if isinstance(o, tuple) else (o, o.stride(0))
        a.out[i] = t.data_ptr() if torch.is_tensor(t) else t
        a.out_ld[i] = ld
    if res is not None:
        for i, o in enumerate(res):
            if o is None:
                continue
            t, ld = o if isinstance(o, tuple) else (o, o.stride(0))
            a.res[i] = t.data_ptr() if torch.is_tensor(t) else t
            a.res_ld[i] = ld
    a.out_nores = _p(out_nores)
    a.flags = family
    a.fin_stats, a.in_stats = _p(fin_stats), _p(in_stats)
    if dw_partial is not None:
        a.dw_partial, a.dw_partial_stride = dw_partial.data_ptr(), dw_partial.stride(0)
    if rc is not None:
        W2, b2, W3, b3 = rc
        h2, h3 = (wi.lookup(W2), wi.lookup(W3)) if wi is not None else (0, 0)
        if not (h2 and h3):
            if query_fused:
                return False
            raise RuntimeError("recompute form: no split-fp16 image of the forward's second / third Linear")
        a.rc_Wh[0], a.rc_Wh[1] = h2, h3
        a.rc_bias[0], a.rc_bias[1] = _p(b2), _p(b3)
    if padd is not None:
        a.padd, a.padd_s, a.padd_r, a.padd_ld = _p(padd), _p(padd_s), _p(padd_r), padd.stride(0)
    if gscale is not None:
        assert gscale.dim() == 2 and gscale.shape[0] >= 3 and gscale.shape[1] >= gscale_ld(M)
        a.gscale, a.gscale_ld = gscale.data_ptr(), gscale.stride(0)
    if query_fused:
        return bool(lib.gfv_rowtile_fuses_dw(C.byref(a)))
    rc = lib.gfv_rowtile_chain(C.byref(a), L.stream_ptr())
    L.check(rc, "gfv_rowtile_chain")
    return gscale is not None and lib.gfv_rowtile_last_path() >= 5


def trans_mlp_fwd(x, res, Wout, bout, gamma, beta, Wpre, bpre, Wpost, bpost, fx1, z, out):
    lib = L.load()
    if _WI is None or not lib.gfv_f16split_enabled():
        return False
    hs = (_WI.lookup(Wout), _WI.lookup(Wpre), _WI.lookup(Wpost))
    if not all(hs):
        return False
    a = L.TransMlp()
    a.x, a.res, a.img_out, a.img_pre, a.img_post = x.data_ptr(), res.data_ptr(), hs[0], hs[1], hs[2]
    a.b_out, a.b_pre, a.b_post = _p(bout), _p(bpre), _p(bpost)
    a.gamma, a.beta, a.wmax = gamma.data_ptr(), beta.data_ptr(), _WI.wmax.data_ptr()
    a.fx1, a.z, a.out, a.M = _p(fx1), _p(z), out.data_ptr(), x.shape[0]
    L.check(lib.gfv_trans_mlp_fwd(C.byref(a), L.stream_ptr()), "gfv_trans_mlp_fwd")
    return True


def trans_mlp_bwd(g, g_add, g_sum, z, fx1, Wpost_t, Wpre_t, Wout_t, gamma, g_z, g_fx1, g_out_x, ln_partial, gscale):
    lib = L.load()
    if _WI is None or not lib.gfv_f16split_enabled():
        return False
    hs = (_WI.lookup(Wpost_t), _WI.lookup(Wpre_t), _WI.lookup(Wout_t))
    if not all(hs):
        return False
    a = L.TransMlpBwd()
    a.g, a.g_add, a.g_sum, a.z, a.fx1 = g.data_ptr(), _p(g_add), _p(g_sum), z.data_ptr(), fx1.data_ptr()
    a.img_post_t, a.img_pre_t, a.img_out_t = hs
    a.gamma, a.wmax = gamma.data_ptr(), _WI.wmax.data_ptr()
    a.g_z, a.g_fx1, a.g_out_x = g_z.data_ptr(), g_fx1.data_ptr(), g_out_x.data_ptr()
    a.ln_partial, a.gscale, a.M = _p(ln_partial), _p(gscale), g.shape[0]
    L.check(lib.gfv_trans_mlp_bwd(C.byref(a), L.stream_ptr()), "gfv_trans_mlp_bwd")
    return True


def linear_dw(G, n_out, segs, M, *, ldg=None, in_add=None, a_op=0, a_gamma=None, a_beta=None, dW=None, db=None,
              want_db=True, accumulate=False, workspace=None, g_offset=0, gscale=None, col_scale=False):
    if col_scale:
        assert a_op == 0
        a_op = L.DW_COLSCALE
    lib = L.load()
    K = sum(s.width for s in segs)
    dev = G.device
    if dW is None:
        dW = torch.empty((n_out, K), dtype=torch.float32, device=dev)
    if db is None and want_db:
        db = torch.empty((n_out,), dtype=torch.float32, device=dev)
    need = lib.gfv_linear_dw_workspace_floats(M, n_out, K)
    if workspace is None or workspace.numel() < need:
        workspace = torch.empty((max(need, 1),), dtype=torch.float32, device=dev)
    cs = (L.Seg * 3)()
    for i, s in enumerate(segs):
        s.fill(cs[i])
    ldg = G.stride(0) if ldg is None else ldg
    rc = lib.gfv_linear_dw_gs(G.data_ptr() + 4 * g_offset, ldg, n_out, cs, len(segs), _p(in_add), a_op, _p(a_gamma),
                              _p(a_beta), M, _p(dW), _p(gscale), _p(db), _p(workspace), 1 if accumulate else 0,
                              L.stream_ptr())
    L.check(rc, "gfv_linear_dw_gs")
    return dW, db
```

### include/gfv.h

```cpp
#ifndef GFV_H_
#define GFV_H_
#include <stddef.h>
#include <stdint.h>

#ifdef __cplusplus
extern "C" {
#endif

#define GFV_ABI_VERSION 3
int gfv_abi_version(void);
int gfv_struct_size(int32_t which);

int gfv_seg_gather_sum(const float* src, const int32_t* rowptr, const int32_t* col, const float* scale,
                       const float* src_scale, float* out, int32_t n_rows, int32_t F, int32_t accumulate, void* stream);

int gfv_seg_gather_sum_nnz(const float* src, const int32_t* rowptr, const int32_t* col, const float* scale,
                           const float* src_scale, float* out, int32_t n_rows, int32_t F, int32_t accumulate,
                           int64_t nnz_hint, void* stream);

int gfv_seg_gather_sum_ex(const float* src, const int32_t* rowptr, const int32_t* col, const float* scale,
                          const float* src_scale, float* out, int32_t n_rows, int32_t F, int32_t accumulate,
                          int64_t nnz_hint, int64_t n_src_hint, void* stream);

int gfv_seg_gather_sum_ln(const float* y, const float* stats, const float* gamma, const float* beta, const int32_t* rowptr,
                          const int32_t* col, float* out, int32_t n_rows, int64_t nnz_hint, int64_t n_src_hint, void* stream);

int gfv_gather_pair(const float* a, const int32_t* s, const int32_t* r, const float* base, float* out,
                    int32_t n_edges, int32_t F, void* stream);

typedef struct {
  const float* ptr;
  const int32_t* idx;
  int32_t width;
  int32_t ld;
  const int32_t* csr_rowptr;
  const float* csr_scale;
  float* save;
} gfv_seg_t;

enum {
  GFV_OP_NONE = 0,
  GFV_OP_BIAS_GELU = 1,
  GFV_OP_MUL_DGELU = 2
};
enum { GFV_IN_NONE = 0, GFV_IN_GELU = 1, GFV_IN_LN = 2, GFV_IN_LNBWD = 3 };
enum { GFV_CHAIN_ROW_OWNER = 1,
       GFV_CHAIN_COLUMN_OWNER = 2    };
enum { GFV_FIN_PLAIN = 0, GFV_FIN_LN = 1, GFV_FIN_LNBWD = 2 };

typedef struct {
  const float* W;
  const float* bias;
  int32_t K, N;
  int32_t op;
  int32_t ldw;
  float* save;
  const float* aux;
  const void* Wh;
  const float* bias2;
} gfv_layer_t;

typedef struct {
  int32_t M;
  int32_t nseg;
  gfv_seg_t seg[3];
  const float* in_add;
  int32_t in_op;
  int32_t nlayers;
  const float* in_gamma;
  const float* in_beta;
  const float* in_aux;
  const float* gadd;
  const int32_t* gadd_s;
  const int32_t* gadd_r;
  float* in_save;
  float* ln_partial;
  gfv_layer_t layer[3];
  int32_t fin_op;
  int32_t hidden;
  const float* fin_gamma;
  const float* fin_beta;
  const float* fin_aux;
  float* fin_presave;
  const float* res[3];
  int32_t res_ld[3];
  int32_t out_ld[3];
  float* out[3];
  float* out_nores;
  const float* padd;
  const int32_t* padd_s;
  const int32_t* padd_r;
  int32_t padd_ld;
  int32_t flags;
  const float* wmax;
  float* gscale;
  int32_t gscale_ld;
  int32_t product_form;
  float* fin_stats;
  const float* in_stats;
  float* dw_partial;
  int64_t dw_partial_stride;
  const float* dw_in;
  int32_t dw_in_ld;
  int32_t reserved2_;
  const void* rc_Wh[2];
  const float* rc_bias[2];
} gfv_rowtile_args_t;
enum { GFV_DW_FUSED_FLOATS = 2 * 128 * 128 + 4 * 128 };
int gfv_rowtile_dw_partials(void);
int gfv_rowtile_dw_partials_m(int32_t M);
int gfv_rowtile_fuses_dw(const gfv_rowtile_args_t* args);

int gfv_rowtile_tiles(int32_t M);
int gfv_rowtile_ln_rows(int32_t M);
int gfv_rowtile_last_ln_rows(void);
int gfv_get_limit(int32_t which);
int gfv_set_limit(int32_t which, int32_t value);
const char* gfv_limit_name(int32_t which);
int gfv_rowtile_chain(const gfv_rowtile_args_t* args, void* stream);
int gfv_rowtile_last_path(void);

typedef struct {
  const float* W;
  void* img;
  int32_t ldw, N, K, reserved;
} gfv_wimg_desc_t;
size_t gfv_weight_image_bytes(int32_t N, int32_t K);
int gfv_f16split_enabled(void);
int gfv_set_f16split(int32_t on);
int gfv_set_f16split_thread(int32_t on);
int gfv_hidden_size(void);
int gfv_set_hidden_size(int32_t h);
int gfv_weight_absmax(const gfv_wimg_desc_t* descs_dev, int32_t n_desc, float* wmax, void* stream);
int gfv_weight_images(const gfv_wimg_desc_t* descs_dev, int32_t n_desc, int64_t max_frags, const float* wmax,
                      void* stream);
int gfv_weight_images_form(const float* wmax);

int gfv_dw_chunks(int32_t M);
int gfv_linear_dw(const float* G, int32_t ldg, int32_t n_out, const gfv_seg_t* segs, int32_t nseg,
                  const float* in_add, int32_t a_gelu, int32_t M, float* dW, float* db, float* workspace,
                  int32_t accumulate, void* stream);
int gfv_linear_dw_gs(const float* G, int32_t ldg, int32_t n_out, const gfv_seg_t* segs, int32_t nseg,
                     const float* in_add, int32_t a_op, const float* a_gamma, const float* a_beta, int32_t M,
                     float* dW, const float* gscale, float* db, float* workspace, int32_t accumulate, void* stream);
size_t gfv_linear_dw_workspace_floats(int32_t M, int32_t n_out, int32_t K);
int gfv_linear_dw_ex(const float* G, int32_t ldg, int32_t n_out, const gfv_seg_t* segs, int32_t nseg,
                     const float* in_add, int32_t a_op, const float* a_gamma, const float* a_beta, int32_t M,
                     float* dW, int32_t reserved, float* db, float* workspace, int32_t accumulate, void* stream);

typedef struct {
  const float* G;
  const float* A;
  const int32_t* idx;
  const float* in_add;
  const float* a_gamma;
  const float* a_beta;
  int32_t ldg, n_out, width, ld;
  int32_t a_op;
  int32_t ld_out;
  int64_t out_off;
  int64_t db_off;
  const float* gscale;
} gfv_dw_tile_t;
enum { GFV_DW_COLSCALE = 8 };
enum { GFV_FLAG_DW_RANGE = 1,
       GFV_FLAG_CHAIN_RANGE = 2 };
int gfv_status_flags(int32_t* flags_out);
int gfv_status_mirror(int32_t** host_word);
int gfv_status_publish(void* stream);
int gfv_dw_slabs(int32_t M, int32_t ntiles, int32_t* rows_per_slab);
size_t gfv_dw_multi_workspace_floats(int32_t M, int32_t ntiles, int64_t block_floats);
int gfv_dw_multi(const gfv_dw_tile_t* tiles, int32_t ntiles, int32_t M, int64_t block_floats, float* workspace,
                 float* grad_block, int32_t accumulate, void* stream);

int gfv_reduce_partials(const float* partial, int32_t n_chunks, int32_t n, float* out, int32_t accumulate,
                        void* stream);

int gfv_reduce_partials_2d(const float* partial, int32_t n_chunks, int64_t chunk_stride, int32_t rows, int32_t cols,
                           int32_t ld_out, float* out, void* stream);

typedef struct {
  const float* partial;
  float* out;
  int64_t chunk_stride;
  int32_t n_chunks, rows, cols, ld_in, ld_out, reserved;
} gfv_reduce_piece_t;
int gfv_reduce_multi(const gfv_reduce_piece_t* pieces, int32_t n_pieces, void* stream);

int gfv_reduce_partials_seg(const float* partial, const int32_t* seg_ptr, int32_t n_seg, int32_t n, float* out,
                            void* stream);

typedef struct {
  const float* in;
  float* out;
  int32_t rows, cols, ld_in, ld_out;
} gfv_transpose_desc_t;
int gfv_transpose_batch(const gfv_transpose_desc_t* descs, int32_t n, int32_t max_rows, int32_t max_cols, void* stream);

typedef struct {
  const void* src;
  void* dst;
  int64_t n_words;
  int32_t kind;
  int32_t add;
} gfv_concat_desc_t;
int gfv_concat_offsets(const gfv_concat_desc_t* descs, int32_t n_desc, int32_t blocks_per_desc, void* stream);

int gfv_transpose(const float* in, int32_t ld_in, float* out, int32_t rows, int32_t cols, void* stream);


int gfv_slice_softmax_fwd(const float* xmid, const float* Ws, const float* bs, const float* temp, float* w, int32_t N,
                          void* stream);
int gfv_slice_softmax_bwd_blocks(int32_t N);
int gfv_slice_softmax_bwd(const float* xmid, const float* Ws, const float* bs, const float* temp, const float* w,
                          const float* gw, float* gxmid, float* partial, int32_t N, void* stream);
int gfv_slice_token_partial(const float* w, const float* a, const int32_t* chunk_beg, const int32_t* chunk_end,
                            int32_t n_chunks, float* partial, void* stream);
int gfv_slice_attention_fwd(const float* partial, const int32_t* gchunk_ptr, int32_t B, const float* Wq, const float* Wk,
                            const float* Wv, float* token, float* norm, float* attn, float* out_token, void* stream);
int gfv_slice_attention_bwd(const float* gpartial, const int32_t* gchunk_ptr, int32_t B, const float* Wq, const float* Wk,
                            const float* Wv, const float* token, const float* norm, const float* attn, float* g_raw,
                            float* g_norm, float* dW_partial, void* stream);
int gfv_slice_softmax_token(const float* xmid, const float* Ws, const float* bs, const float* temp, const float* a,
                            const int32_t* chunk_beg, const int32_t* chunk_end, int32_t n_chunks, float* w, float* partial,
                            void* stream);
int gfv_deslice(const float* w, const float* T, const int32_t* batch, float* out, int32_t N, int32_t accumulate,
                void* stream);
int gfv_slice_gw(const float* a, const float* T, const float* add, const int32_t* batch, float* gw, int32_t N,
                 int32_t accumulate, void* stream);
int gfv_slice_post_bwd(const float* xmid, const float* Ws, const float* bs, const float* temp, const float* w,
                       const float* g_out_x, const float* out_token, const float* fx_mid, const float* g_raw,
                       const float* g_norm, const int32_t* batch, float* g_x_mid, float* g_fx_mid, float* partial,
                       int32_t N, int32_t n_graphs, void* stream);

int gfv_phi_fwd(const float* dec, const float* y, const int32_t* node_type, const float* uv_old, float* phi, int32_t N,
                int32_t mode, void* stream);
int gfv_phi_bwd(const float* gphi, const float* dec, const int32_t* node_type, float* gdec, int32_t N, int32_t mode,
                void* stream);
int gfv_wlsq_fwd(const float* phi, const int32_t* rowptr, const int32_t* outn, const float* Bp, const float* An,
                 const float* rn, float* grad, int32_t N, void* stream);
int gfv_wlsq_bwd(const float* ggrad, const float* An, const float* rn, const int32_t* rowptr_o, const int32_t* inn,
                 const float* Bo, const float* sumB, float* grhs_ws, float* gphi, int32_t N, void* stream);
int gfv_wlsq_fwd_full(const float* phi, const int32_t* rowptr, const int32_t* outn, const float* Bp, const float* An,
                      const float* rn, float* grad, float* full5, int32_t N, void* stream);
int gfv_wlsq_bwd_full(const float* g5, const float* An, const float* rn, const int32_t* rowptr_o, const int32_t* inn,
                      const float* Bo, const float* sumB, float* grhs_ws, float* gphi, int32_t N, void* stream);
int gfv_wlsq_fwd_ex(const float* phi, const int32_t* rowptr, const int32_t* outn, const float* Bp, const float* An,
                    const float* rn, float* grad, float* full, int32_t N, int32_t terms, void* stream);
int gfv_wlsq_bwd_ex(const float* ggrad, const float* gfull, const float* An, const float* rn, const int32_t* rowptr_o,
                    const int32_t* inn, const float* Bo, const float* sumB, float* grhs_ws, float* gphi, int32_t N,
                    int32_t terms, void* stream);
int gfv_face_fwd(const float* phi, const float* grad, const int32_t* es, const int32_t* er, const float* pos,
                 const float* fpos, const int32_t* ftype, const float* y, float* Ff, int32_t E, void* stream);
int gfv_cell_fwd(const float* phi, const float* grad, const float* Ff, const float* pos, const int32_t* crow,
                 const int32_t* kface, const int32_t* knode, const float* kS, const int32_t* ftype, const float* centroid,
                 const float* area, const int32_t* cbatch, const float* theta, const float* dt, const float* uvp_dim,
                 const float* sigma, float* phic, float* cres, float* uvp_cell, int32_t C, void* stream);
int gfv_cell_fwd_ex(const float* phi, const float* grad, const float* Ff, const float* pos, const int32_t* crow,
                    const int32_t* kface, const int32_t* knode, const float* kS, const int32_t* ftype,
                    const float* centroid, const float* area, const int32_t* cbatch, const float* theta, const float* dt,
                    const float* uvp_dim, const float* sigma, float* phic, float* cres, float* uvp_cell, int32_t C,
                    int32_t non_conserved, float* gradc, void* stream);
int gfv_graph_loss(const float* cres, const int32_t* gcell_ptr, const float* theta, const float* sigma, float* sums,
                   float* losses, int32_t B, void* stream);
// ... 183 lines not shown
```

Before: 284.1.

## Skip dead last-block edge output and stash bwd residual in LDS

In the last message-passing block the edge MLP's residual output is unused, so the forward chain can run with no output tensor, and the backward skips reading the zero gradient tensor and the residual. Separately, the column-chain backward kernel keeps its dy input in extra LDS so that when the residual aliases the input it is reread from LDS instead of global memory. A query-only accept entry point lets the host check whether a kernel path supports these null-pointer configurations before launching. The trade-off is more LDS per workgroup, which may lower occupancy, plus extra launch-validation logic.

```diff
diff --git a/gen-fvgn-steady_amd/csrc/cfwd.hip b/gen-fvgn-steady_amd/csrc/cfwd.hip
--- a/gen-fvgn-steady_amd/csrc/cfwd.hip
+++ b/gen-fvgn-steady_amd/csrc/cfwd.hip
@@ -308,8 +308,10 @@
                       (y[q][4 * n + 2] - mean) * rstd * ga.z + be.z, (y[q][4 * n + 3] - mean) * rstd * ga.w + be.w};
         if (live) {
           if (A.out_nores) st4(A.out_nores + (size_t)row * 128 + c0 + 16 * n, o);
-          if (A.res[0]) { o[0] += rres[q][n].x; o[1] += rres[q][n].y; o[2] += rres[q][n].z; o[3] += rres[q][n].w; }
-          st4(A.out[0] + (size_t)row * A.out_ld[0] + c0 + 16 * n, o);
+          if (A.out[0]) {
+            if (A.res[0]) { o[0] += rres[q][n].x; o[1] += rres[q][n].y; o[2] += rres[q][n].z; o[3] += rres[q][n].w; }
+            st4(A.out[0] + (size_t)row * A.out_ld[0] + c0 + 16 * n, o);
+          }
         }
       }
     }
@@ -350,7 +352,8 @@
     if (L.save && !cf_al16(L.save)) return 0;
   }
   if (a->layer[2].save) return 0;
-  if (!a->out[0] || a->out[1] || a->out[2] || (!dec && ((a->out_ld[0] & 3) || !cf_al16(a->out[0]))) || a->res[1] || a->res[2]) return 0;
+  if (!a->out[0] && (dec || !a->fin_presave || !a->fin_stats || a->res[0])) return 0;
+  if (a->out[1] || a->out[2] || (!dec && a->out[0] && ((a->out_ld[0] & 3) || !cf_al16(a->out[0]))) || a->res[1] || a->res[2]) return 0;
   if (a->res[0] && ((a->res_ld[0] & 3) || !cf_al16(a->res[0]))) return 0;
   if ((a->out_nores && !cf_al16(a->out_nores)) || (a->fin_presave && !cf_al16(a->fin_presave)) ||
       (!dec && (!cf_al16(a->fin_gamma) || !cf_al16(a->fin_beta))))
diff --git a/gen-fvgn-steady_amd/csrc/colchain.hip b/gen-fvgn-steady_amd/csrc/colchain.hip
--- a/gen-fvgn-steady_amd/csrc/colchain.hip
+++ b/gen-fvgn-steady_amd/csrc/colchain.hip
@@ -1,4 +1,5 @@
 #include "colchain_kernel.h"
+#include "gfv_limits.h"
 
 int* gfv_internal_status_ptr();
 
@@ -76,14 +77,20 @@
     int* st = gfv_internal_status_ptr();
     if (!st) return 0;
     const dim3 grid(gfv_rowtile_dw_partials_m(a->M)), blk(64 * CC_W);
+    const bool res_lds = a->res[0] && (const void*)a->res[0] == a->seg[0].ptr && a->res_ld[0] == a->seg[0].ld &&
+                         gfv_internal_limit(GFV_LIM_COLCHAIN_RES_LDS) != 0;
 #define CB_K(...) GFV_LAUNCH((colchain_bwd_kernel<__VA_ARGS__>), grid, blk, 0, stream, *a, st)
+#define CB_LAUNCH_(LOWP, RC, RL)                                                                                                 \
+  do {                                                                                                                           \
+    if (a->nlayers == 2) CB_K(LOWP, false, false, true, RC);                                                                     \
+    else if (a->layer[2].N == 192 && a->gadd) CB_K(LOWP, true, true, false, RC, RL);                                             \
+    else if (a->layer[2].N == 192) CB_K(LOWP, false, true, false, RC, RL);                                                       \
+    else if (a->gadd) CB_K(LOWP, true, false, false, RC, RL);                                                                    \
+    else CB_K(LOWP, false, false, false, RC, RL);                                                                                \
+  } while (0)
 #define CB_LAUNCH(LOWP, RC)                                                                                                      \
   do {                                                                                                                           \
-    if (a->nlayers == 2) CB_K(LOWP, false, false, true, RC);                                                                     \
-    else if (a->layer[2].N == 192 && a->gadd) CB_K(LOWP, true, true, false, RC);                                                 \
-    else if (a->layer[2].N == 192) CB_K(LOWP, false, true, false, RC);                                                           \
-    else if (a->gadd) CB_K(LOWP, true, false, false, RC);                                                                        \
-    else CB_K(LOWP, false, false, false, RC);                                                                                    \
+    if (!(RC) && res_lds) CB_LAUNCH_(LOWP, RC, (!(RC))); else CB_LAUNCH_(LOWP, RC, false);                                       \
   } while (0)
     const bool rc = a->rc_Wh[0] != nullptr;
     if (a->product_form == 2) { if (rc) CB_LAUNCH(2, true); else CB_LAUNCH(2, false); }
@@ -91,6 +98,7 @@
     else { if (rc) CB_LAUNCH(0, true); else CB_LAUNCH(0, false); }
 #undef CB_K
 #undef CB_LAUNCH
+#undef CB_LAUNCH_
     return 2;
   }
   return 0;
diff --git a/gen-fvgn-steady_amd/csrc/colchain_kernel.h b/gen-fvgn-steady_amd/csrc/colchain_kernel.h
--- a/gen-fvgn-steady_amd/csrc/colchain_kernel.h
+++ b/gen-fvgn-steady_amd/csrc/colchain_kernel.h
@@ -68,6 +68,7 @@
   static constexpr int PART = 3 * BUF;
   static constexpr int SMAX = PART + CB_TG * 16 * 8 * 8;
   static constexpr int TOTAL = SMAX + 64;
+  static constexpr int STASH = CB_TG * 512 * 16;
 };
 
 __device__ __forceinline__ void cb_tr_operand(const char* xbuf, int q0, int ct, int lane, gfv_f16x8& hi, gfv_f16x8& lo) {
@@ -233,10 +234,11 @@
   }
 }
 
-template <int LOWP, bool GADD, bool OUT2 = false, bool NOOUT = false, bool RC = false>
+template <int LOWP, bool GADD, bool OUT2 = false, bool NOOUT = false, bool RC = false, bool RESLDS = false>
 __global__ __launch_bounds__(64 * CC_W, 2) void colchain_bwd_kernel(const gfv_rowtile_args_t A, int* status) {
   constexpr int TG = CB_TG;
-  __shared__ __attribute__((aligned(16))) char lds[CbLds::TOTAL + (RC ? CbLds::BUF : 0)];
+  static_assert(!RESLDS || (!RC && !NOOUT), "the stash takes the fourth buffer's place; a two-layer launch has no residual");
+  __shared__ __attribute__((aligned(16))) char lds[CbLds::TOTAL + (RC ? CbLds::BUF : 0) + (RESLDS ? CbLds::STASH : 0)];
   char* b0 = lds + CbLds::B0;
   char* b1 = lds + CbLds::B1;
   char* b2 = lds + CbLds::B2;
@@ -247,6 +249,7 @@
   CcCtx c;
   c.w = __builtin_amdgcn_readfirstlane(threadIdx.x >> 6);
   c.lane = threadIdx.x & 63;
+  float4* stash = reinterpret_cast<float4*>(lds + CbLds::TOTAL + c.w * 1024 + c.lane * 16);
   c.j = c.lane & 15;
   c.g = c.lane >> 4;
   c.col0 = 16 * c.w + 4 * c.g;
@@ -435,6 +438,10 @@
       if (!PRE) {
         cb_load_inputs(B, c, c.row0, in);
         cb_load_gathers<GADD>(B, c, gidx, in);
+      }
+      if constexpr (RESLDS) {
+#pragma unroll
+        for (int q = 0; q < TG; ++q) stash[q * 512] = in.dy[q];
       }
       if (A.in_add) {
         const cb_rsrc ia = cb_buf(A.in_add, rows128);
@@ -616,7 +623,7 @@
       }
     }
     float4 rr[NOOUT ? 1 : TG];
-    if constexpr (!NOOUT) {
+    if constexpr (!NOOUT && !RESLDS) {
 #pragma unroll
       for (int q = 0; q < TG; ++q) rr[q] = cb_ld4(B.res, offL[q]);
     }
@@ -631,6 +638,7 @@
       for (int p = 0; p < TG / 2; ++p) {
         if (p >= np) break;
         floatx4 n0 = a0, n1 = a1;
+        if constexpr (RESLDS) { rr[2 * p] = stash[(2 * p) * 512]; rr[2 * p + 1] = stash[(2 * p + 1) * 512]; }
         if (!CB_LATE && p + 1 < TG / 2) cc_mma_pair<4, LOWP, true>(b0, p + 1, wh, wl, c.lane, n0, n1);
         const floatx4 o0 = (a0 * inv_in) * c.invw + floatx4{rr[2 * p].x, rr[2 * p].y, rr[2 * p].z, rr[2 * p].w};
         const floatx4 o1 = (a1 * inv_in) * c.invw + floatx4{rr[2 * p + 1].x, rr[2 * p + 1].y, rr[2 * p + 1].z, rr[2 * p + 1].w};
diff --git a/gen-fvgn-steady_amd/csrc/gfv_limits.h b/gen-fvgn-steady_amd/csrc/gfv_limits.h
--- a/gen-fvgn-steady_amd/csrc/gfv_limits.h
+++ b/gen-fvgn-steady_amd/csrc/gfv_limits.h
@@ -8,6 +8,8 @@
   GFV_LIM_CTRANS_MAX_M,
   GFV_LIM_LIN1S_ON,
   GFV_LIM_LIN1S_MAX_M,
+  GFV_LIM_COLCHAIN_RES_LDS,
+  GFV_LIM_LAST_EDGE_SKIP,
   GFV_LIM_COUNT
 };
 int gfv_internal_limit(int which);
diff --git a/gen-fvgn-steady_amd/csrc/rowtile.hip b/gen-fvgn-steady_amd/csrc/rowtile.hip
--- a/gen-fvgn-steady_amd/csrc/rowtile.hip
+++ b/gen-fvgn-steady_amd/csrc/rowtile.hip
@@ -53,7 +53,8 @@
 const LimitDef k_limits[GFV_LIM_COUNT] = {
     {"GFV_CBWD", 1},        {"GFV_CBWD_MAX_M", 25000},      {"GFV_CFWD", 1},          {"GFV_CFWD_MAX_M", 250000},
     {"GFV_CTRANS", 1},         {"GFV_CTRANS_MAX_M", 16384},
-    {"GFV_LIN1S", 1},       {"GFV_LIN1S_MAX_M", 16384}};
+    {"GFV_LIN1S", 1},       {"GFV_LIN1S_MAX_M", 16384},
+    {"GFV_COLCHAIN_RES_LDS", 1}, {"GFV_LAST_EDGE_SKIP", 1}};
 int g_limit[GFV_LIM_COUNT];
 bool g_limit_set[GFV_LIM_COUNT];
 std::once_flag g_limit_once;
@@ -89,6 +90,14 @@
 extern "C" int gfv_rowtile_tiles(int32_t M) { return (M + BM - 1) / BM; }
 
 static int rowtile_chain_impl(const gfv_rowtile_args_t* args, void* stream);
+static thread_local bool g_query_only = false;
+extern "C" int gfv_rowtile_chain(const gfv_rowtile_args_t* args, void* stream);
+extern "C" int gfv_rowtile_accepts(const gfv_rowtile_args_t* args) {
+  g_query_only = true;
+  const int rc = gfv_rowtile_chain(args, nullptr);
+  g_query_only = false;
+  return rc == GFV_OK ? 1 : 0;
+}
 extern "C" int gfv_rowtile_chain(const gfv_rowtile_args_t* args, void* stream) {
   if (!args) return GFV_ERR_ARG;
   if (args->product_form < 0 || args->product_form > 4 || (args->hidden != 0 && (args->hidden < 16 || args->hidden > 128 || (args->hidden & 15))))
@@ -186,6 +195,12 @@
               args->out_ld[0], args->in_op, args->fin_op);
     return GFV_ERR_ARG;
   }
+  if (!args->out[0] && !(f16 && !args->dw_partial && cfwd_try(args, f16_mode() >= 2 ? f16_mode() - 1 : 0, (hipStream_t)stream, 1)))
+    return GFV_ERR_ARG;
+  for (int i = 0; i < args->nseg; ++i)
+    if (!args->seg[i].ptr && !(i == 0 && fast_t && f16 && args->dw_partial && gfv_rowtile_fuses_dw(args))) return GFV_ERR_ARG;
+  if (args->dw_partial && !(fast_t && f16)) return GFV_ERR_ARG;
+  if (g_query_only) return GFV_OK;
   void* tok = nullptr;
   if (gfv_prof_enabled()) {
     double fl = 0, by = 0;
diff --git a/gen-fvgn-steady_amd/gfv/cmdlist.py b/gen-fvgn-steady_amd/gfv/cmdlist.py
--- a/gen-fvgn-steady_amd/gfv/cmdlist.py
+++ b/gen-fvgn-steady_amd/gfv/cmdlist.py
@@ -11,7 +11,7 @@
     "gfv_linear_dw_workspace_floats", "gfv_dw_multi_workspace_floats", "gfv_f16split_enabled", "gfv_set_f16split", "gfv_set_f16split_thread", "gfv_hidden_size",
     "gfv_weight_image_bytes", "gfv_normalizer_blocks", "gfv_slice_softmax_bwd_blocks", "gfv_profile_enable",
     "gfv_profile_collect", "gfv_profile_reset", "gfv_profile_set_sizes", "gfv_status_flags", "gfv_status_mirror", "gfv_prep_workspace_bytes", "gfv_get_limit", "gfv_set_limit", "gfv_limit_name", "gfv_rowtile_dw_partials", "gfv_rowtile_dw_partials_m",
-    "gfv_rowtile_fuses_dw", "gfv_graph_norm_workspace_bytes", "gfv_plan_create", "gfv_plan_destroy", "gfv_plan_table", "gfv_plan_sizes",
+    "gfv_rowtile_fuses_dw", "gfv_rowtile_accepts", "gfv_graph_norm_workspace_bytes", "gfv_plan_create", "gfv_plan_destroy", "gfv_plan_table", "gfv_plan_sizes",
     "gfv_record_begin", "gfv_record_count", "gfv_record_end", "gfv_record_length", "gfv_record_replay", "gfv_record_free",
     "gfv_record_delay_side", "gfv_pool_args_bytes", "gfv_pool_table_bytes", "gfv_pool_table_check"))
 
diff --git a/gen-fvgn-steady_amd/gfv/engine.py b/gen-fvgn-steady_amd/gfv/engine.py
--- a/gen-fvgn-steady_amd/gfv/engine.py
+++ b/gen-fvgn-steady_amd/gfv/engine.py
@@ -345,7 +345,7 @@
                 f"{lin}.4.bias"] + ([f"{prefix}.1.weight", f"{prefix}.1.bias"] if ln else [])
 
     def mlp3_fwd(self, P, prefix, M, segs, *, ln=True, res=None, in_add=None, want_nores=False, keep=True, w1=None,
-                 padd=None, saved_segs=None, nores_from_saved=False):
+                 padd=None, saved_segs=None, nores_from_saved=False, want_out=True):
         names = self._mlp_names(prefix, ln)
         W1, b1, W2, b2, W3, b3 = (P[n] for n in names[:6])
         if w1 is not None:
@@ -369,17 +369,18 @@
             z1 = z2 = None
             y3 = _empty(dev, M, 128) if from_saved else None
             stats = _empty(dev, M, 2) if from_saved else None
-        out = _empty(dev, M, nout)
         if want_nores and nores_from_saved and y3 is not None and stats is not None and nout == 128:
             want_nores = False
         nores = _empty(dev, M, 128) if want_nores else None
-        ops.rowtile_chain(
-            M, segs,
-            [LayerSpec(W1, b1, L.OP_BIAS_GELU, save=z1), LayerSpec(W2, b2, L.OP_BIAS_GELU, save=z2), LayerSpec(W3, b3)],
-            [out], in_add=in_add, fin_op=L.FIN_LN if ln else L.FIN_PLAIN,
-            fin_gamma=P[names[6]] if ln else None, fin_beta=P[names[7]] if ln else None, fin_presave=y3,
-            res=[res] if res is not None else None, out_nores=nores, fin_stats=stats,
-            **(dict(padd=padd[0], padd_s=padd[1], padd_r=padd[2]) if padd is not None else {}))
+        layers = [LayerSpec(W1, b1, L.OP_BIAS_GELU, save=z1), LayerSpec(W2, b2, L.OP_BIAS_GELU, save=z2), LayerSpec(W3, b3)]
+        kw = dict(in_add=in_add, fin_op=L.FIN_LN if ln else L.FIN_PLAIN, fin_gamma=P[names[6]] if ln else None,
+                  fin_beta=P[names[7]] if ln else None, fin_presave=y3, out_nores=nores, fin_stats=stats,
+                  **(dict(padd=padd[0], padd_s=padd[1], padd_r=padd[2]) if padd is not None else {}))
+        no_out = (not want_out and L.get_limit("GFV_LAST_EDGE_SKIP") and ln and nout == 128 and y3 is not None and stats is not None
+                  and nores is None and ops.rowtile_chain(M, segs, layers, [(None, 128)], query_accepts=True, **kw))
+        out = None if no_out else _empty(dev, M, nout)
+        ops.rowtile_chain(M, segs, layers, [(None, 128) if no_out else out],
+                          res=[res] if (res is not None and not no_out) else None, **kw)
         if not keep:
             return out, nores, dict(y3=y3, stats=stats)
         saved = dict(z1=z1, z2=z2, y3=y3, segs=segs if saved_segs is None else saved_segs, in_add=in_add, M=M, ln=ln,
@@ -576,7 +577,7 @@
     def _put(grads, name, value):
         cmdlist.call(grads.view(name).copy_, value.reshape(grads.shape[name]))
 
-    def gn_fwd(self, P, prefix, x, e, pl, keep=True):
+    def gn_fwd(self, P, prefix, x, e, pl, keep=True, last=False):
         N, E = pl.N, pl.E
         fuse = self.csr_fuse
         if self.factor:
@@ -591,7 +592,8 @@
                 ops.rowtile_chain(N, [Seg(nb)], [LayerSpec(W1[:, 0:128], stack=W1[:, 128:256])],
                                   [(pab, 256), (pab.data_ptr() + 512, 256)])
             e_out, e_new, sv_e = self.mlp3_fwd(P, f"{prefix}.eb_module.net", E, [Seg(e)], res=e, want_nores=True,
-                                               w1=W1[:, 256:384], padd=(pab, pl.es, pl.er), nores_from_saved=self._agg_ln, keep=keep)
+                                               w1=W1[:, 256:384], padd=(pab, pl.es, pl.er), nores_from_saved=self._agg_ln, keep=keep,
+                                               want_out=not last)
             sv_e["nb"] = nb
         else:
             nb = ops.seg_gather_sum(x, pl.n_rowptr, pl.n_col_node, N)
@@ -693,12 +695,14 @@
         layers = [LayerSpec(W3t, None, L.OP_MUL_DGELU, aux=sv["z2"]), LayerSpec(W2t, None, L.OP_MUL_DGELU, save=gz1, aux=sv["z1"]),
                   LayerSpec(W1ct)]
         gs = _empty(dev, 3, ops.gscale_ld(M))
-        kw = dict(res=[G], in_op=L.IN_LNBWD, in_gamma=P[names[6]], in_aux=sv["y3"], in_stats=sv["stats"], gadd=gadd[0], gadd_s=gadd[1],
+        dead = G is self._zero_e and bool(L.get_limit("GFV_LAST_EDGE_SKIP"))
+        gseg = Seg(None, width=128, ld=128) if dead else Seg(G)
+        kw = dict(res=None if dead else [G], in_op=L.IN_LNBWD, in_gamma=P[names[6]], in_aux=sv["y3"], in_stats=sv["stats"], gadd=gadd[0], gadd_s=gadd[1],
                   gadd_r=gadd[2], dw_partial=dwp, gscale=gs,
                   rc=(P[names[2]], P[names[3]], P[names[4]], P[names[5]]) if lean else None)
-        if not ops.rowtile_chain(M, [Seg(G)], layers, [g_e_in], query_fused=True, **kw):
+        if not ops.rowtile_chain(M, [gseg], layers, [g_e_in], query_fused=True, **kw):
             return None
-        ops.rowtile_chain(M, [Seg(G)], layers, [g_e_in], **kw)
+        ops.rowtile_chain(M, [gseg], layers, [g_e_in], **kw)
         g_nb = _empty(dev, N, 128)
         if self.csr_fuse and (self._fuse_mask & 4):
             G_s, G_r = _empty(dev, N, 128), _empty(dev, N, 128)
@@ -1195,7 +1199,7 @@
         if self.net == "EPD":
             blocks = []
             for ig in range(self.mp):
-                xn, en, sv = self.gn_fwd(P, f"{prefix}.GN_block_list.{ig}", xn, en, pl, keep=keep)
+                xn, en, sv = self.gn_fwd(P, f"{prefix}.GN_block_list.{ig}", xn, en, pl, keep=keep, last=ig == self.mp - 1)
                 blocks.append(sv)
             procs.append(dict(blocks=blocks, trans=None))
         else:
@@ -1204,7 +1208,8 @@
                 emb = xn
                 blocks = []
                 for ig in range(self.mp):
-                    xn, en, sv = self.gn_fwd(P, f"{pp}.GN_block_list.{ig}", xn, en, pl, keep=keep)
+                    xn, en, sv = self.gn_fwd(P, f"{pp}.GN_block_list.{ig}", xn, en, pl, keep=keep,
+                                             last=pp is pps[-1] and ig == self.mp - 1)
                     blocks.append(sv)
                 xn, svt = self.trans_fwd(P, f"{pp}.TransBlock", xn, emb, pl, keep=keep)
                 procs.append(dict(blocks=blocks, trans=svt))
diff --git a/gen-fvgn-steady_amd/gfv/lib.py b/gen-fvgn-steady_amd/gfv/lib.py
--- a/gen-fvgn-steady_amd/gfv/lib.py
+++ b/gen-fvgn-steady_amd/gfv/lib.py
@@ -143,6 +143,7 @@
     "gfv_rowtile_dw_partials": (C.c_int, []),
     "gfv_rowtile_dw_partials_m": (C.c_int, [C.c_int32]),
     "gfv_rowtile_fuses_dw": (C.c_int, [C.POINTER(RowtileArgs)]),
+    "gfv_rowtile_accepts": (C.c_int, [C.POINTER(RowtileArgs)]),
     "gfv_dw_chunks": (C.c_int, [C.c_int32]),
     "gfv_linear_dw_workspace_floats": (C.c_size_t, [C.c_int32, C.c_int32, C.c_int32]),
     "gfv_linear_dw": (C.c_int, [C.c_void_p, C.c_int32, C.c_int32, C.POINTER(Seg), C.c_int32, C.c_void_p, C.c_int32,
diff --git a/gen-fvgn-steady_amd/gfv/ops.py b/gen-fvgn-steady_amd/gfv/ops.py
--- a/gen-fvgn-steady_amd/gfv/ops.py
+++ b/gen-fvgn-steady_amd/gfv/ops.py
@@ -110,7 +110,7 @@
         assert csr is None or idx is None
 
     def fill(self, cs):
-        cs.ptr = self.t.data_ptr() + 4 * self.offset
+        cs.ptr = None if self.t is None else self.t.data_ptr() + 4 * self.offset
         cs.idx = _p(self.idx) if self.csr is None else self.csr[1].data_ptr()
         cs.width = self.width
         cs.ld = self.ld
@@ -226,7 +226,7 @@
                   gadd=None, gadd_s=None, gadd_r=None, in_save=None, ln_partial=None, fin_op=L.FIN_PLAIN,
                   fin_gamma=None, fin_beta=None, fin_aux=None, fin_presave=None, res=None, out_nores=None,
                   padd=None, padd_s=None, padd_r=None, wimg=None, gscale=None, family=0, fin_stats=None, in_stats=None,
-                  dw_partial=None, query_fused=False, rc=None):
+                  dw_partial=None, query_fused=False, rc=None, query_accepts=False):
     lib = L.load()
     wi = wimg if wimg is not None else _WI
     if layers[-1].stack is not None:
@@ -299,6 +299,8 @@
         a.gscale, a.gscale_ld = gscale.data_ptr(), gscale.stride(0)
     if query_fused:
         return bool(lib.gfv_rowtile_fuses_dw(C.byref(a)))
+    if query_accepts:
+        return bool(lib.gfv_rowtile_accepts(C.byref(a)))
     rc = lib.gfv_rowtile_chain(C.byref(a), L.stream_ptr())
     L.check(rc, "gfv_rowtile_chain")
     return gscale is not None and lib.gfv_rowtile_last_path() >= 5
diff --git a/include/gfv.h b/include/gfv.h
--- a/include/gfv.h
+++ b/include/gfv.h
@@ -110,6 +110,7 @@
 int gfv_rowtile_dw_partials(void);
 int gfv_rowtile_dw_partials_m(int32_t M);
 int gfv_rowtile_fuses_dw(const gfv_rowtile_args_t* args);
+int gfv_rowtile_accepts(const gfv_rowtile_args_t* args);
 
 int gfv_rowtile_tiles(int32_t M);
 int gfv_rowtile_ln_rows(int32_t M);
```

Result: no change. 286.1, median of 6 (+0.7%).
